# FEniCS/performance-test

Hardware: AMD Instinct MI355X
Metric: DoF/s for ZZZ Assemble + ZZZ Solve; CG-SpMV achieved HBM GB/s vs peak (higher is better)
Workload: dtype f64

## Files before the change

### performance-test_amd/csrc/zzz_api.hip

```cpp
#include "zzz_internal.h"
#include "zzz_sellp.h"

#include <algorithm>
#include <cstdlib>
#include <cstring>
#include <mutex>
#include <numeric>

namespace zzz
{
static std::mutex g_err_mutex;
static std::string g_err;

void set_global_error(const char* msg)
{
  std::lock_guard<std::mutex> lk(g_err_mutex);
  g_err = msg;
}

int fail(zzz_ctx* ctx, int code, const char* fmt, ...)
{
  char buf[1024];
  va_list ap;
  va_start(ap, fmt);
  vsnprintf(buf, sizeof(buf), fmt, ap);
  va_end(ap);
  if (ctx)
    ctx->err = buf;
  else
    set_global_error(buf);
  return code;
}

static int ndofs_cell(int order) { return order == 1 ? 4 : order == 2 ? 10 : order == 3 ? 20 : -1; }

template <typename T>
static int upload(zzz_ctx* ctx, DevBuf<T>& d, const T* h, size_t n, size_t pad = 0)
{
  ZZZ_HIP(ctx, d.alloc(n + pad));
  if (pad)
    ZZZ_HIP(ctx, hipMemsetAsync(d.p + n, 0, pad * sizeof(T), ctx->stream));
  if (n)
    ZZZ_HIP(ctx, hipMemcpyAsync(d.p, h, n * sizeof(T), hipMemcpyHostToDevice, ctx->stream));
  ZZZ_HIP(ctx, hipStreamSynchronize(ctx->stream));
  return ZZZ_OK;
}
int alloc_problem_vectors(zzz_ctx* ctx)
{
  const size_t nv = (size_t)ctx->nloc();
  ZZZ_HIP(ctx, ctx->bc.alloc(nv));
  ZZZ_HIP(ctx, hipMemsetAsync(ctx->bc.p, 0, nv, ctx->stream));
  DevBuf<double>* vecs[] = {&ctx->b, &ctx->u, &ctx->r, &ctx->z, &ctx->p, &ctx->w, &ctx->dinv, &ctx->coeff[0], &ctx->coeff[1]};
  for (DevBuf<double>* v : vecs)
  {
    ZZZ_HIP(ctx, v->alloc(nv));
    ZZZ_HIP(ctx, hipMemsetAsync(v->p, 0, nv * sizeof(double), ctx->stream));
  }
  ZZZ_HIP(ctx, ctx->part_a.alloc(3 * 4096));
  ZZZ_HIP(ctx, ctx->part_b.alloc(4096));
  ZZZ_HIP(ctx, hipStreamSynchronize(ctx->stream));
  return ZZZ_OK;
}
void bc_values_clear(zzz_ctx* ctx)
{
  ctx->have_bc_val = false;
  ++ctx->bc_version;
}
}

using namespace zzz;

extern "C" {

int zzz_device_count(void)
{
  int n = 0;
  if (hipGetDeviceCount(&n) != hipSuccess)
    return 0;
  return n;
}

int zzz_device_memory(int device, size_t* free_bytes, size_t* total_bytes)
{
  if (!free_bytes || !total_bytes)
    return fail(nullptr, ZZZ_ERR_ARG, "zzz_device_memory: NULL argument");
  int prev = 0;
  (void)hipGetDevice(&prev);
  if (hipSetDevice(device) != hipSuccess || hipMemGetInfo(free_bytes, total_bytes) != hipSuccess)
  {
    (void)hipGetLastError();
    (void)hipSetDevice(prev);
    return fail(nullptr, ZZZ_ERR_HIP, "hipMemGetInfo failed on device %d", device);
  }
  (void)hipSetDevice(prev);
  return ZZZ_OK;
}

int zzz_ctx_create(int device, zzz_ctx** out)
{
  if (!out)
    return fail(nullptr, ZZZ_ERR_ARG, "zzz_ctx_create: out is NULL");
  *out = nullptr;
  int n = 0;
  hipError_t e = hipGetDeviceCount(&n);
  if (e != hipSuccess || n <= 0)
    return fail(nullptr, ZZZ_ERR_NO_GPU, "no HIP device available (%s); libzzz_hip has no CPU fallback",
                e == hipSuccess ? "device count 0" : hipGetErrorString(e));
  if (device < 0 || device >= n)
    return fail(nullptr, ZZZ_ERR_ARG, "device %d out of range [0, %d)", device, n);
  e = hipSetDevice(device);
  if (e != hipSuccess)
    return fail(nullptr, ZZZ_ERR_HIP, "hipSetDevice(%d): %s", device, hipGetErrorString(e));
  zzz_ctx* ctx = new zzz_ctx();
  ctx->device = device;
  e = hipStreamCreateWithFlags(&ctx->stream, hipStreamNonBlocking);
  if (e != hipSuccess)
  {
    delete ctx;
    return fail(nullptr, ZZZ_ERR_HIP, "hipStreamCreate: %s", hipGetErrorString(e));
  }
  if (ctx->state.alloc(1) != hipSuccess || ctx->red.alloc(16) != hipSuccess
      || hipHostMalloc((void**)&ctx->h_state, 8 * sizeof(zzz::CgState), hipHostMallocDefault) != hipSuccess)
  {
    zzz_ctx_destroy(ctx);
    return fail(nullptr, ZZZ_ERR_HIP, "context allocation failed");
  }
  memset(ctx->h_state, 0, 8 * sizeof(zzz::CgState));
  {
    static bool loaded[64] = {};
    if (device < 64 && !loaded[device])
    {
      loaded[device] = true;
      zzz::preload_cubegen();
      zzz::preload_renumber();
      zzz::preload_pattern();
      zzz::preload_assemble();
      zzz::preload_sellp_pack();
      zzz::preload_sellp_dict();
      zzz::preload_sellp_pipe();
      zzz::preload_sellp_blk();
      zzz::preload_sellp_win();
      zzz::preload_sellp();
      zzz::preload_spmv();
      zzz::preload_cg();
      zzz::preload_cg_pipe();
      zzz::preload_cg_f32();
      zzz::preload_comm();
      zzz::preload_matfree();
      zzz::preload_mg();
      zzz::preload_pmg();
      zzz::preload_nullspace();
      (void)hipGetLastError();
    }
  }
  if (const char* e = getenv("ZZZ_SPMV_VARIANT"))
  {
    ctx->spmv_variant = atoi(e) & 27;
    ctx->spmv_auto = false;
  }
  if (const char* e = getenv("ZZZ_SELLP"))
  {
    const int v = atoi(e);
    ctx->sellp_mode = v >= 0 && v <= 4 ? v : 1;
    ctx->sellp_long_rows = v == 4;
    if (v == 4)
      ctx->sellp_mode = 2;
  }
  if (const char* e = getenv("ZZZ_SELLP_DROP"))
    ctx->sellp_drop = atoi(e) != 0;
  if (const char* e = getenv("ZZZ_SELLP_DICT"))
    ctx->sellp_dict = atoi(e);
  if (const char* e = getenv("ZZZ_SELLP_BWIN"))
    ctx->sellp_bwin = atoi(e);
  if (const char* e = getenv("ZZZ_SELLP_EARLY"))
    ctx->sellp_early = atoi(e) != 0;
  if (const char* e = getenv("ZZZ_ASM_NODE3"))
    ctx->asm_node3 = atoi(e) != 0;
  if (const char* e = getenv("ZZZ_SELLP_BLK"))
    ctx->sellp_blk = atoi(e);
  if (const char* e = getenv("ZZZ_SELLP_PIPE"))
    ctx->sellp_pipe = atoi(e);
  if (const char* e = getenv("ZZZ_CG_DINV_CODES"))
    ctx->cg_dinv_codes = atoi(e);
  if (const char* e = getenv("ZZZ_CG_XDEFER"))
    ctx->cg_xdefer = atoi(e);
  if (const char* e = getenv("ZZZ_CG_XDEFER_K"))
  {
    const int v = atoi(e);
    if (v == 2 || v == 4 || v == 8)
      ctx->cg_xdefer_k = v;
  }
  if (const char* e = getenv("ZZZ_SELLP_FORMS"))
  {
    const int v = atoi(e);
    if (!(v & 1))
      ctx->sellp_tail |= 2;
    ctx->sellp_align = (v & 2) != 0;
    ctx->sellp_periodic = (v & 4) != 0;
  }
  if (const char* e = getenv("ZZZ_SPMV_LPR"))
  {
    const int v = atoi(e);
    for (int sft = 0; sft <= 4; ++sft)
      if (v == (1 << sft))
        ctx->spmv_lpr_forced = sft;
  }
  if (const char* e = getenv("ZZZ_COLS16"))
  {
    const int v = atoi(e);
    ctx->cols16_enabled = v != 0;
    if (v >= 10 && v <= 13)
      ctx->cols16_offb_forced = v;
  }
  if (const char* e = getenv("ZZZ_OVERLAP"))
    ctx->overlap = atoi(e) != 0;
  if (const char* e = getenv("ZZZ_CG_PIPE_STREAM"))
    ctx->pipe_stream = atoi(e) != 0;
  *out = ctx;
  return ZZZ_OK;
}

void zzz_ctx_destroy(zzz_ctx* ctx)
{
  if (!ctx)
    return;
  (void)hipSetDevice(ctx->device);
  if (ctx->stream)
    (void)hipStreamSynchronize(ctx->stream);
  mg_destroy(ctx);
  comm_destroy(ctx);
  for (hipEvent_t ev : ctx->ev)
    (void)hipEventDestroy(ev);
  for (hipEvent_t ev : ctx->ev_halo)
    (void)hipEventDestroy(ev);
  if (ctx->sp_event)
    (void)hipEventDestroy(ctx->sp_event);
  if (ctx->h_state)
    (void)hipHostFree(ctx->h_state);
  if (ctx->adj_flag_host)
    (void)hipHostFree(ctx->adj_flag_host);
  if (ctx->stream && !ctx->stream_borrowed)
    (void)hipStreamDestroy(ctx->stream);
  for (void* q : ctx->retired)
    (void)hipFree(q);
  delete ctx;
}

const char* zzz_last_error(const zzz_ctx* ctx)
{
  if (ctx)
    return ctx->err.c_str();
  std::lock_guard<std::mutex> lk(g_err_mutex);
  static thread_local std::string copy;
  copy = g_err;
  return copy.c_str();
}

int zzz_sync(zzz_ctx* ctx)
{
  if (!ctx)
    return fail(nullptr, ZZZ_ERR_ARG, "NULL context");
  ZZZ_HIP(ctx, hipSetDevice(ctx->device));
  ZZZ_HIP(ctx, hipStreamSynchronize(ctx->stream));
  return ZZZ_OK;
}

#define ZZZ_ENTER(ctx)                                          \
  do                                                            \
  {                                                             \
    if (!(ctx))                                                 \
      return fail(nullptr, ZZZ_ERR_ARG, "NULL context");        \
    ZZZ_HIP(ctx, hipSetDevice((ctx)->device));                  \
  } while (0)

int zzz_mesh_upload(zzz_ctx* ctx, int64_t nverts, const double* x, int64_t ncells, const int32_t* cell_verts)
{
  ZZZ_ENTER(ctx);
  ctx->cube_feed = false;
  ++ctx->feed_version;
  if (nverts <= 0 || ncells <= 0 || !x || !cell_verts)
    return fail(ctx, ZZZ_ERR_ARG, "zzz_mesh_upload: empty mesh or NULL array");
  if (nverts > INT32_MAX / 4 || ncells > (INT32_MAX - 8) / 20)
    return fail(ctx, ZZZ_ERR_LIMIT, "mesh too large for int32 indexing (%lld vertices, %lld cells)", (long long)nverts,
                (long long)ncells);
  for (int64_t i = 0; i < 4 * ncells; ++i)
    if (cell_verts[i] < 0 || cell_verts[i] >= nverts)
      return fail(ctx, ZZZ_ERR_ARG, "cell_verts[%lld] = %d out of range", (long long)i, cell_verts[i]);
  ctx->nverts = nverts;
  ctx->ncells = ncells;
  ctx->h_cell_verts.assign(cell_verts, cell_verts + 4 * ncells);
  int rc = upload(ctx, ctx->x, x, (size_t)(3 * nverts));
  if (rc)
    return rc;
  rc = upload(ctx, ctx->cell_verts, cell_verts, (size_t)(4 * ncells));
  ctx->have_pattern = ctx->have_matrix = false;
  ctx->xq_valid = false;
  ctx->mf.valid = ctx->mf.failed = false;
  return rc;
}

int zzz_dofmap_upload(zzz_ctx* ctx, int order, int bs, const int32_t* cell_dofs, int64_t n_owned, int64_t n_ghost)
{
  ZZZ_ENTER(ctx);
  ctx->cube_feed = false;
  ++ctx->feed_version;
  const int nd = ndofs_cell(order);
  if (nd < 0)
    return fail(ctx, ZZZ_ERR_ARG, "order %d not supported (1..3)", order);
  if (bs != 1 && bs != 3)
    return fail(ctx, ZZZ_ERR_ARG, "block size %d not supported (1 or 3)", bs);
  if (ctx->ncells == 0)
    return fail(ctx, ZZZ_ERR_ARG, "zzz_dofmap_upload before zzz_mesh_upload");
  if (n_owned <= 0 || n_ghost < 0 || !cell_dofs)
    return fail(ctx, ZZZ_ERR_ARG, "zzz_dofmap_upload: bad sizes");
  const int64_t nloc = n_owned + n_ghost;
  if (nloc * bs > INT32_MAX - 8)
    return fail(ctx, ZZZ_ERR_LIMIT, "%lld local scalar dofs exceed int32", (long long)(nloc * bs));
  for (int64_t i = 0; i < ctx->ncells * nd; ++i)
    if (cell_dofs[i] < 0 || cell_dofs[i] >= nloc)
      return fail(ctx, ZZZ_ERR_ARG, "cell_dofs[%lld] = %d out of range", (long long)i, cell_dofs[i]);
  ctx->order = order;
  ctx->bs = bs;
  ctx->nd = nd;
  ctx->n_owned = n_owned;
  ctx->n_ghost = n_ghost;
  ctx->h_cell_dofs.assign(cell_dofs, cell_dofs + ctx->ncells * nd);
  int rc = upload(ctx, ctx->cell_dofs, cell_dofs, (size_t)(ctx->ncells * nd));
  if (rc)
    return rc;
  ZZZ_HIP(ctx, ctx->facet_mask.alloc((size_t)ctx->ncells));
  ZZZ_HIP(ctx, hipMemsetAsync(ctx->facet_mask.p, 0, (size_t)ctx->ncells, ctx->stream));
  ctx->nfacets = 0;
  rc = alloc_problem_vectors(ctx);
  if (rc)
    return rc;
  ctx->have_bc = false;
  bc_values_clear(ctx);
  ctx->have_coeff[0] = ctx->have_coeff[1] = false;
  ctx->have_pattern = ctx->have_matrix = false;
  ctx->xq_valid = false;
  ctx->mf.valid = ctx->mf.failed = false;
  ctx->near_null_ld = 0;
  rc = renumber_build(ctx);
  if (rc)
    return rc;
  ctx->adj_runs_n = -1;
  pattern_reserve(ctx);
  return ensure_p1_coords(ctx);
}

int zzz_bc_upload(zzz_ctx* ctx, int64_t nbc, const int32_t* bc_dofs)
{
  ZZZ_ENTER(ctx);
  ctx->cube_feed = false;
  ++ctx->feed_version;
  bc_values_clear(ctx);
  if (ctx->order == 0)
    return fail(ctx, ZZZ_ERR_ARG, "zzz_bc_upload before zzz_dofmap_upload");
  if (nbc < 0 || (nbc > 0 && !bc_dofs))
    return fail(ctx, ZZZ_ERR_ARG, "zzz_bc_upload: bad arguments");
  std::vector<uint8_t> m((size_t)ctx->nloc(), 0);
  for (int64_t i = 0; i < nbc; ++i)
  {
    if (bc_dofs[i] < 0 || bc_dofs[i] >= ctx->nloc())
      return fail(ctx, ZZZ_ERR_ARG, "bc_dofs[%lld] = %d out of range", (long long)i, bc_dofs[i]);
    int64_t d = bc_dofs[i];
    if (ctx->renumbered && d / ctx->bs < ctx->n_owned)
      d = (int64_t)ctx->h_iperm[(size_t)(d / ctx->bs)] * ctx->bs + d % ctx->bs;
    m[(size_t)d] = 1;
  }
  ZZZ_HIP(ctx, hipMemcpyAsync(ctx->bc.p, m.data(), m.size(), hipMemcpyHostToDevice, ctx->stream));
  ZZZ_HIP(ctx, hipStreamSynchronize(ctx->stream));
  ctx->have_bc = true;
  ctx->mf.valid = ctx->mf.failed = false;
  return ZZZ_OK;
}

int zzz_bc_values_upload(zzz_ctx* ctx, const double* values)
{
  ZZZ_ENTER(ctx);
  if (!values)
  {
    ctx->have_bc_val = false;
    return ZZZ_OK;
  }
  if (ctx->order == 0)
    return fail(ctx, ZZZ_ERR_ARG, "zzz_bc_values_upload before zzz_dofmap_upload / zzz_cube_generate: the values are indexed by local dof");
  if (!ctx->have_bc)
    return fail(ctx, ZZZ_ERR_ARG, "zzz_bc_values_upload before a Dirichlet set exists (zzz_bc_upload / zzz_cube_generate): the values "
                                  "belong to its dofs");
  const size_t nv = (size_t)ctx->nloc();
  std::vector<double> tmp;
  if (ctx->renumbered)
  {
    tmp.resize(nv);
    to_internal(ctx, values, tmp.data(), false);
    values = tmp.data();
  }
  ZZZ_HIP(ctx, ctx->bc_val.alloc(nv));
  ZZZ_HIP(ctx, hipMemcpyAsync(ctx->bc_val.p, values, nv * sizeof(double), hipMemcpyHostToDevice, ctx->stream));
  ZZZ_HIP(ctx, hipStreamSynchronize(ctx->stream));
  ctx->have_bc_val = true;
  return ZZZ_OK;
}

int zzz_facets_upload(zzz_ctx* ctx, int64_t nfacets, const int32_t* pairs)
{
  ZZZ_ENTER(ctx);
  ctx->cube_feed = false;
  ++ctx->feed_version;
  if (ctx->order == 0)
    return fail(ctx, ZZZ_ERR_ARG, "zzz_facets_upload before zzz_dofmap_upload");
  if (nfacets < 0 || (nfacets > 0 && !pairs))
    return fail(ctx, ZZZ_ERR_ARG, "zzz_facets_upload: bad arguments");
  std::vector<uint8_t> m((size_t)ctx->ncells, 0);
  for (int64_t i = 0; i < nfacets; ++i)
  {
    const int32_t c = pairs[2 * i], f = pairs[2 * i + 1];
    if (c < 0 || c >= ctx->ncells || f < 0 || f > 3)
      return fail(ctx, ZZZ_ERR_ARG, "facet %lld = (%d, %d) out of range", (long long)i, c, f);
    m[c] |= (uint8_t)(1u << f);
  }
  if (ctx->cells_renumbered)
  {
    std::vector<uint8_t> mi(m.size());
    for (size_t i = 0; i < m.size(); ++i)
      mi[i] = m[(size_t)ctx->h_cperm[i]];
    m.swap(mi);
  }
  ZZZ_HIP(ctx, hipMemcpyAsync(ctx->facet_mask.p, m.data(), m.size(), hipMemcpyHostToDevice, ctx->stream));
  ZZZ_HIP(ctx, hipStreamSynchronize(ctx->stream));
  ctx->nfacets = nfacets;
  return ZZZ_OK;
}

int zzz_coeff_upload(zzz_ctx* ctx, int which, const double* values)
{
  ZZZ_ENTER(ctx);
  if (ctx->order == 0)
    return fail(ctx, ZZZ_ERR_ARG, "zzz_coeff_upload before zzz_dofmap_upload");
  if ((which != ZZZ_COEFF_F && which != ZZZ_COEFF_G) || !values)
    return fail(ctx, ZZZ_ERR_ARG, "zzz_coeff_upload: bad arguments");
  std::vector<double> tmp;
  if (ctx->renumbered)
  {
    tmp.resize((size_t)ctx->nloc());
    to_internal(ctx, values, tmp.data(), false);
    values = tmp.data();
  }
  ZZZ_HIP(ctx, hipMemcpyAsync(ctx->coeff[which].p, values, (size_t)ctx->nloc() * sizeof(double), hipMemcpyHostToDevice,
                              ctx->stream));
  ZZZ_HIP(ctx, hipStreamSynchronize(ctx->stream));
  ctx->have_coeff[which] = true;
  return ZZZ_OK;
}

static int pattern_build_host(zzz_ctx* ctx);

int zzz_csr_pattern_build(zzz_ctx* ctx)
{
  ZZZ_ENTER(ctx);
  if (ctx->order == 0)
    return fail(ctx, ZZZ_ERR_ARG, "zzz_csr_pattern_build before zzz_dofmap_upload");
  ctx->have_pattern = ctx->have_matrix = false;
  ++ctx->pattern_version;
  ctx->bw_on = false;
  ctx->have_adj_li = false;
  ctx->have_asm_pos = false;
  ++ctx->mat_version;
  const char* mode = getenv("ZZZ_PATTERN");
  int rc;
  if (mode && strcmp(mode, "host") == 0)
    rc = pattern_build_host(ctx);
  else
  {
    bool fallback = false;
    rc = pattern_build_device(ctx, &fallback);
    if (rc && fallback)
      rc = pattern_build_host(ctx);
  }
  if (rc)
    return rc;
  rc = build_adjT(ctx);
  if (!rc)
// ... 358 lines not shown
    ctx->spmv_variant = variant & 27;
    ctx->spmv_auto = false;
  }
  hipEvent_t e0, e1;
  ZZZ_HIP(ctx, hipEventCreate(&e0));
  ZZZ_HIP(ctx, hipEventCreate(&e1));
  ZZZ_HIP(ctx, hipMemsetAsync(ctx->state.p, 0, sizeof(zzz::CgState), ctx->stream));
  int np = 0;
  int rc = launch_spmv(ctx, ctx->p.p, ctx->w.p, ctx->part_a.p, &np);
  ZZZ_HIP(ctx, hipEventRecord(e0, ctx->stream));
  for (int i = 0; i < reps && !rc; ++i)
    rc = launch_spmv(ctx, ctx->p.p, ctx->w.p, ctx->part_a.p, &np);
  ZZZ_HIP(ctx, hipEventRecord(e1, ctx->stream));
  ZZZ_HIP(ctx, hipEventSynchronize(e1));
  float ms = 0;
  ZZZ_HIP(ctx, hipEventElapsedTime(&ms, e0, e1));
  (void)hipEventDestroy(e0);
  (void)hipEventDestroy(e1);
  ctx->spmv_variant = saved;
  ctx->spmv_auto = saved_auto;
  *avg_ms = ms / reps;
  return rc;
}

int zzz_action(zzz_ctx* ctx, const double* x, double* y)
{
  ZZZ_ENTER(ctx);
  if (ctx->order == 0 || !x || !y)
    return fail(ctx, ZZZ_ERR_ARG, "zzz_action: no dofmap or NULL vector");
  const size_t n = (size_t)(ctx->n_owned * ctx->bs);
  std::vector<double> xin;
  if (ctx->renumbered)
  {
    xin.resize(n);
    to_internal(ctx, x, xin.data(), true);
    x = xin.data();
  }
  ZZZ_HIP(ctx, hipMemsetAsync(ctx->p.p, 0, ctx->p.n * sizeof(double), ctx->stream));
  ZZZ_HIP(ctx, hipMemcpyAsync(ctx->p.p, x, n * sizeof(double), hipMemcpyHostToDevice, ctx->stream));
  ZZZ_HIP(ctx, hipStreamSynchronize(ctx->stream));
  if (ctx->comm)
  {
    int rc = comm_halo_forward(ctx, ctx->p.p);
    if (rc)
      return rc;
  }
  int rc = launch_matfree_action(ctx, ctx->p.p, ctx->w.p, nullptr, nullptr);
  if (rc)
    return rc;
  if (ctx->renumbered)
  {
    ZZZ_HIP(ctx, hipMemcpyAsync(xin.data(), ctx->w.p, n * sizeof(double), hipMemcpyDeviceToHost, ctx->stream));
    ZZZ_HIP(ctx, hipStreamSynchronize(ctx->stream));
    to_caller(ctx, xin.data(), y, true);
    return ctx->comm ? comm_p2p_check(ctx) : ZZZ_OK;
  }
  ZZZ_HIP(ctx, hipMemcpyAsync(y, ctx->w.p, n * sizeof(double), hipMemcpyDeviceToHost, ctx->stream));
  ZZZ_HIP(ctx, hipStreamSynchronize(ctx->stream));
  return ctx->comm ? comm_p2p_check(ctx) : ZZZ_OK;
}

int zzz_matfree_setup(zzz_ctx* ctx)
{
  ZZZ_ENTER(ctx);
  return mf_plan_build(ctx);
}

int zzz_matfree_diagonal(zzz_ctx* ctx, double* diag)
{
  ZZZ_ENTER(ctx);
  if (ctx->order == 0 || !diag)
    return fail(ctx, ZZZ_ERR_ARG, "zzz_matfree_diagonal: no dofmap or NULL vector");
  if (int rc = launch_matfree_diagonal(ctx, ctx->w.p))
    return rc;
  const size_t n = (size_t)(ctx->n_owned * ctx->bs);
  std::vector<double> tmp(ctx->renumbered ? n : 0);
  double* dst = ctx->renumbered ? tmp.data() : diag;
  ZZZ_HIP(ctx, hipMemcpyAsync(dst, ctx->w.p, n * sizeof(double), hipMemcpyDeviceToHost, ctx->stream));
  ZZZ_HIP(ctx, hipStreamSynchronize(ctx->stream));
  if (ctx->renumbered)
    to_caller(ctx, tmp.data(), diag, true);
  return ZZZ_OK;
}

int zzz_matfree_info(zzz_ctx* ctx, int64_t info[8])
{
  if (!ctx || !info)
    return fail(ctx, ZZZ_ERR_ARG, "zzz_matfree_info: bad arguments");
  const zzz::MfPlan& M = ctx->mf;
  info[0] = M.valid ? 1 : 0;
  info[1] = M.nblocks;
  info[2] = M.nc;
  info[3] = M.threads;
  info[4] = M.nloc_max;
  info[5] = M.nshared;
  info[6] = M.nslots;
  info[7] = M.bytes_per_action;
  return ZZZ_OK;
}

int zzz_action_time(zzz_ctx* ctx, int reps, double* avg_ms)
{
  ZZZ_ENTER(ctx);
  if (reps <= 0 || !avg_ms || ctx->order == 0)
    return fail(ctx, ZZZ_ERR_ARG, "zzz_action_time: bad arguments");
  hipEvent_t e0, e1;
  ZZZ_HIP(ctx, hipEventCreate(&e0));
  ZZZ_HIP(ctx, hipEventCreate(&e1));
  ZZZ_HIP(ctx, hipMemsetAsync(ctx->state.p, 0, sizeof(zzz::CgState), ctx->stream));
  int np = 0;
  int rc = launch_matfree_action(ctx, ctx->p.p, ctx->w.p, ctx->part_a.p, &np);
  ZZZ_HIP(ctx, hipEventRecord(e0, ctx->stream));
  for (int i = 0; i < reps && !rc; ++i)
    rc = launch_matfree_action(ctx, ctx->p.p, ctx->w.p, ctx->part_a.p, &np);
  ZZZ_HIP(ctx, hipEventRecord(e1, ctx->stream));
  ZZZ_HIP(ctx, hipEventSynchronize(e1));
  float ms = 0;
  ZZZ_HIP(ctx, hipEventElapsedTime(&ms, e0, e1));
  (void)hipEventDestroy(e0);
  (void)hipEventDestroy(e1);
  *avg_ms = ms / reps;
  return rc;
}

int zzz_cg_solve(zzz_ctx* ctx, const zzz_solver_opts* o, int* iters, double* rnorm)
{
  ZZZ_ENTER(ctx);
  if (!o)
    return fail(ctx, ZZZ_ERR_ARG, "zzz_cg_solve: NULL options");
  if (o->op == ZZZ_OP_CSR && !ctx->have_matrix)
    return fail(ctx, ZZZ_ERR_ARG, "zzz_cg_solve: matrix not assembled");
  if (o->op != ZZZ_OP_CSR && o->op != ZZZ_OP_MATFREE)
    return fail(ctx, ZZZ_ERR_ARG, "unknown operator kind %d", o->op);
  if (o->variant != ZZZ_CG_PETSC && o->variant != ZZZ_CG_CGH && o->variant != ZZZ_CG_PIPE)
    return fail(ctx, ZZZ_ERR_ARG, "unknown CG variant %d", o->variant);
  if (o->variant == ZZZ_CG_PIPE && (o->op != ZZZ_OP_CSR || o->single_reduction || (o->pc != ZZZ_PC_NONE && o->pc != ZZZ_PC_JACOBI)))
    return fail(ctx, ZZZ_ERR_ARG, "-ksp_type pipecg applies to the assembled operator with -pc_type jacobi or none, and not with "
                                  "-ksp_cg_single_reduction");
  if (o->variant == ZZZ_CG_CGH && o->pc != ZZZ_PC_NONE)
    return fail(ctx, ZZZ_ERR_ARG, "src/cg.h has no preconditioner: use pc = ZZZ_PC_NONE");
  if (o->pc != ZZZ_PC_NONE && o->pc != ZZZ_PC_JACOBI && o->pc != ZZZ_PC_CHEBYSHEV_JACOBI && o->pc != ZZZ_PC_MG && o->pc != ZZZ_PC_PMG)
    return fail(ctx, ZZZ_ERR_ARG, "unsupported preconditioner %d (none, jacobi, chebyshev-jacobi, mg, pmg)", o->pc);
  if (o->pc == ZZZ_PC_MG || o->pc == ZZZ_PC_PMG)
    if (int rc = mg_check(ctx, o))
      return rc;
  if (o->pc == ZZZ_PC_CHEBYSHEV_JACOBI && o->op != ZZZ_OP_CSR)
    return fail(ctx, ZZZ_ERR_ARG, "the Chebyshev-Jacobi preconditioner needs the assembled operator");
  if (o->pc == ZZZ_PC_CHEBYSHEV_JACOBI && (o->variant != ZZZ_CG_PETSC || o->pc_degree < 0 || o->pc_degree > 64 || o->pc_esteig_its > 64))
    return fail(ctx, ZZZ_ERR_ARG, "the Chebyshev-Jacobi preconditioner applies to KSPCG (either form), degree 1..64, estimate <= 64 steps");
  if (o->norm < 0 || o->norm > 2)
    return fail(ctx, ZZZ_ERR_ARG, "unknown norm type %d", o->norm);
  if (o->single_reduction && (o->variant != ZZZ_CG_PETSC || o->op != ZZZ_OP_CSR))
    return fail(ctx, ZZZ_ERR_ARG, "-ksp_cg_single_reduction applies to KSPCG on the assembled operator only");
  if (o->max_it < 0 || o->max_it > (1 << 24))
    return fail(ctx, ZZZ_ERR_ARG, "max_it %d out of range", o->max_it);
  return cg_solve(ctx, o, iters, rnorm);
}

static const char* f32_declined(const zzz_ctx* ctx)
{
  if (ctx->order == 0)
    return "no dofmap";
  if (ctx->bs != 1)
    return "block size 3: the float32 path exists for the Poisson form M only (src/Poisson.py:33), not for elasticity";
  if (ctx->comm)
    return "a communicator is attached: the float32 path has no halo exchange or all-reduce yet (one rank only)";
  return nullptr;
}

int zzz_action_f32(zzz_ctx* ctx, const float* x, float* y)
{
  ZZZ_ENTER(ctx);
  if (!x || !y)
    return fail(ctx, ZZZ_ERR_ARG, "zzz_action_f32: NULL vector");
  if (const char* why = f32_declined(ctx))
    return fail(ctx, ZZZ_ERR_ARG, "zzz_action_f32: %s", why);
  const size_t n = (size_t)ctx->n_owned, nl = (size_t)ctx->nloc();
  std::vector<float> tmp;
  if (ctx->renumbered)
  {
    tmp.resize(n);
    for (size_t i = 0; i < n; ++i)
      tmp[i] = x[ctx->h_perm[i]];
    x = tmp.data();
  }
  ZZZ_HIP(ctx, ctx->f32_p.reserve(nl));
  ZZZ_HIP(ctx, ctx->f32_y.reserve(nl));
  ZZZ_HIP(ctx, hipMemsetAsync(ctx->f32_p.p, 0, nl * sizeof(float), ctx->stream));
  ZZZ_HIP(ctx, hipMemcpyAsync(ctx->f32_p.p, x, n * sizeof(float), hipMemcpyHostToDevice, ctx->stream));
  ZZZ_HIP(ctx, hipStreamSynchronize(ctx->stream));
  if (int rc = mf_action_f32(ctx, ctx->f32_p.p, ctx->f32_y.p, nullptr, nullptr))
    return rc;
  float* dst = ctx->renumbered ? tmp.data() : y;
  ZZZ_HIP(ctx, hipMemcpyAsync(dst, ctx->f32_y.p, n * sizeof(float), hipMemcpyDeviceToHost, ctx->stream));
  ZZZ_HIP(ctx, hipStreamSynchronize(ctx->stream));
  if (ctx->renumbered)
    for (size_t i = 0; i < n; ++i)
      y[ctx->h_perm[i]] = tmp[i];
  return ZZZ_OK;
}

int zzz_action_time_f32(zzz_ctx* ctx, int reps, double* avg_ms)
{
  ZZZ_ENTER(ctx);
  if (reps <= 0 || !avg_ms)
    return fail(ctx, ZZZ_ERR_ARG, "zzz_action_time_f32: bad arguments");
  if (const char* why = f32_declined(ctx))
    return fail(ctx, ZZZ_ERR_ARG, "zzz_action_time_f32: %s", why);
  const size_t nl = (size_t)ctx->nloc();
  const float* before = ctx->f32_p.p;
  ZZZ_HIP(ctx, ctx->f32_p.reserve(nl));
  ZZZ_HIP(ctx, ctx->f32_y.reserve(nl));
  if (ctx->f32_p.p != before)
    ZZZ_HIP(ctx, hipMemsetAsync(ctx->f32_p.p, 0, nl * sizeof(float), ctx->stream));
  hipEvent_t e0, e1;
  ZZZ_HIP(ctx, hipEventCreate(&e0));
  ZZZ_HIP(ctx, hipEventCreate(&e1));
  ZZZ_HIP(ctx, hipMemsetAsync(ctx->state.p, 0, sizeof(zzz::CgState), ctx->stream));
  int np = 0;
  int rc = mf_action_f32(ctx, ctx->f32_p.p, ctx->f32_y.p, ctx->part_a.p, &np);
  ZZZ_HIP(ctx, hipEventRecord(e0, ctx->stream));
  for (int i = 0; i < reps && !rc; ++i)
    rc = mf_action_f32(ctx, ctx->f32_p.p, ctx->f32_y.p, ctx->part_a.p, &np);
  ZZZ_HIP(ctx, hipEventRecord(e1, ctx->stream));
  ZZZ_HIP(ctx, hipEventSynchronize(e1));
  float ms = 0;
  ZZZ_HIP(ctx, hipEventElapsedTime(&ms, e0, e1));
  (void)hipEventDestroy(e0);
  (void)hipEventDestroy(e1);
  *avg_ms = ms / reps;
  return rc;
}

int zzz_matfree_info_f32(zzz_ctx* ctx, int64_t info[4])
{
  if (!ctx || !info)
    return fail(ctx, ZZZ_ERR_ARG, "zzz_matfree_info_f32: bad arguments");
  return mf_f32_info(ctx, info);
}

int zzz_cg_solve_f32(zzz_ctx* ctx, const zzz_solver_opts* o, int* iters, double* rnorm)
{
  ZZZ_ENTER(ctx);
  if (!o)
    return fail(ctx, ZZZ_ERR_ARG, "zzz_cg_solve_f32: NULL options");
  if (o->variant != ZZZ_CG_CGH)
    return fail(ctx, ZZZ_ERR_ARG, "zzz_cg_solve_f32: variant %d: float32 runs linalg::cg (src/cg.h, ZZZ_CG_CGH) only", o->variant);
  if (o->pc != ZZZ_PC_NONE)
    return fail(ctx, ZZZ_ERR_ARG, "zzz_cg_solve_f32: preconditioner %d: src/cg.h has none, use pc = ZZZ_PC_NONE", o->pc);
  if (o->op != ZZZ_OP_MATFREE)
    return fail(ctx, ZZZ_ERR_ARG, "zzz_cg_solve_f32: operator %d: float32 exists for the matrix-free operator (ZZZ_OP_MATFREE) only", o->op);
  if (o->single_reduction)
    return fail(ctx, ZZZ_ERR_ARG, "zzz_cg_solve_f32: -ksp_cg_single_reduction (single_reduction) applies to KSPCG on the assembled operator only");
  if (const char* why = f32_declined(ctx))
    return fail(ctx, ZZZ_ERR_ARG, "zzz_cg_solve_f32: %s", why);
  if (ctx->have_bc_val)
    return fail(ctx, ZZZ_ERR_ARG, "zzz_cg_solve_f32: Dirichlet values were uploaded (zzz_bc_values_upload): the lifted right-hand side is "
                                  "not formed in float32 yet");
  if (o->max_it < 0 || o->max_it > (1 << 24))
    return fail(ctx, ZZZ_ERR_ARG, "max_it %d out of range", o->max_it);
  if (ctx->b.n < (size_t)ctx->nloc() || ctx->u.n < (size_t)ctx->nloc())
    return fail(ctx, ZZZ_ERR_ARG, "zzz_cg_solve_f32: no problem vectors");
  return cg_solve_f32(ctx, o, iters, rnorm);
}

int zzz_cg_history(zzz_ctx* ctx, int n, double* out)
{
  if (!ctx || !out || n < 0)
    return fail(ctx, ZZZ_ERR_ARG, "zzz_cg_history: bad arguments");
  const size_t m = std::min((size_t)n, ctx->history.size());
  std::copy(ctx->history.begin(), ctx->history.begin() + (long)m, out);
  return ZZZ_OK;
}

int zzz_spmv_info(zzz_ctx* ctx, int64_t info[8])
{
  ZZZ_ENTER(ctx);
  if (!info || !ctx->have_pattern)
    return fail(ctx, ZZZ_ERR_ARG, "zzz_spmv_info: no pattern");
  if (!sellp_active(ctx))
    if (int rc = ensure_cols16(ctx))
      return rc;
  info[0] = ctx->have_cols16 ? 1 : 0;
  info[1] = ctx->cols16_offb;
  info[2] = ctx->have_cols16 ? ctx->cols16_fallback_tiles : ctx->ntiles;
  info[3] = ctx->ntiles;
  if (sellp_active(ctx) && ctx->sp_win_max > 0)
  {
    info[2] = ctx->sp_win_bytes;
    info[3] = -(int64_t)ctx->sp_win_max;
  }
  info[4] = sellp_active(ctx) ? 1 : (int64_t)1 << ctx->spmv_lpr_shift;
  info[5] = sellp_active(ctx) ? (ctx->sp_sorted ? 2 : 1) : 0;
  info[6] = sellp_active(ctx) ? sellp_stream_bytes(ctx) : 0;
  info[7] = sellp_active(ctx) ? ctx->sp_chunks * 512 : 0;
  return ZZZ_OK;
}

int zzz_spmv_values_info2(zzz_ctx* ctx, int n, int64_t* out)
{
  ZZZ_ENTER(ctx);
  if (!out || n < 0 || !ctx->have_pattern)
    return fail(ctx, ZZZ_ERR_ARG, "zzz_spmv_values_info: no pattern");
  int64_t info[10] = {0, 0, 0, 0, 0, 0, 0, 0, 0, 0};
  if (sellp_active(ctx))
  {
    const bool blk = zzz::sellp_blk_serves(ctx);
    info[4] = !blk && zzz::sellp_pipe_wgs(ctx, false) ? 1 : 0;
    info[5] = blk ? 1 : (info[4] ? zzz::sellp_pipe_wgs(ctx, false) : 8);
    info[0] = ctx->sp_sd_on ? 3 : (ctx->sp_dict_on ? (ctx->sp_dict_n <= zzz::SP_DICT_LDS_ENTRIES ? 2 : 1) : 0);
    info[1] = ctx->sp_dict_on ? ctx->sp_dict_n : 0;
    info[2] = sellp_stream_bytes(ctx);
    info[3] = ctx->sp_bytes + ctx->nslices * 8;
    const bool win = zzz::sellp_win_serves(ctx);
    info[6] = blk ? 1 : (win ? 2 : 0);
    info[7] = blk ? ctx->bk_entries : (win ? ctx->bw_window_entries : 0);
    info[8] = blk ? ctx->bk_chunks : (win ? ctx->bw_chunks : 0);
    info[9] = blk ? ctx->bk_form : (win ? ctx->bw_nblk : 0);
    if (win)
      info[4] = 0, info[5] = 1;
  }
  for (int i = 0; i < std::min(n, 10); ++i)
    out[i] = info[i];
  return ZZZ_OK;
}

int zzz_spmv_values_info(zzz_ctx* ctx, int64_t info[4]) { return zzz_spmv_values_info2(ctx, 4, info); }

int zzz_abi_version(void) { return ZZZ_ABI_VERSION; }

int zzz_internal_order_download(zzz_ctx* ctx, int32_t* perm, int32_t* kind)
{
  if (!ctx || ctx->order == 0)
    return fail(ctx, ZZZ_ERR_ARG, "zzz_internal_order_download: no dofmap yet");
  if (perm)
    for (int64_t i = 0; i < ctx->n_owned; ++i)
      perm[i] = ctx->renumbered ? ctx->h_perm[(size_t)i] : (int32_t)i;
  if (kind)
    *kind = (ctx->renumbered ? ctx->renumber_kind : 0) | (ctx->cells_renumbered ? 16 : 0);
  return ZZZ_OK;
}

int zzz_cg_info(zzz_ctx* ctx, int64_t info[4])
{
  if (!ctx || !info)
    return fail(ctx, ZZZ_ERR_ARG, "zzz_cg_info: bad arguments");
  info[0] = (ctx->last_solve_dinv_codes > 0 ? 2 : 0) | (ctx->last_solve_red_overlapped ? 4 : 0) | (ctx->last_solve_xdefer_k > 1 ? 8 : 0) |
            ((int64_t)(ctx->last_solve_xdefer_k & 15) << 4) | ((int64_t)ctx->last_solve_dinv_codes << 8);
  info[1] = ctx->last_iters;
  info[2] = ctx->last_reason;
  info[3] = (int64_t)(ctx->last_pc_bound * 1.0e6);
  return ZZZ_OK;
}

int zzz_profile_get(zzz_ctx* ctx, double* spmv_avg_ms, int64_t* spmv_count)
{
  if (!ctx)
    return fail(nullptr, ZZZ_ERR_ARG, "NULL context");
  if (spmv_avg_ms)
    *spmv_avg_ms = ctx->prof_spmv_ms;
  if (spmv_count)
    *spmv_count = ctx->prof_spmv_n;
  return ZZZ_OK;
}

}
```

### performance-test_amd/csrc/zzz_cg.hip

```cpp
#include "zzz_device.h"
#include "zzz_internal.h"
#include "zzz_cg.h"

#include <cmath>
#include <cstdlib>

namespace zzz
{
__device__ inline double reduce_parts_bcast(const double* __restrict__ parts, int np, double* sh)
{
  double s = 0;
  for (int i = threadIdx.x; i < np; i += blockDim.x)
    s += parts[i];
  const double t = block_reduce_sum(s, sh);
  __shared__ double bc;
  __syncthreads();
  if (threadIdx.x == 0)
    bc = t;
  __syncthreads();
  return bc;
}

struct DirScalars
{
// ... 493 lines not shown
  const double alpha = beta_it / pw;
  if (variant != ZZZ_CG_CGH && !isfinite(alpha))
  {
    if (blockIdx.x == 0 && threadIdx.x == 0)
    {
      st->iters = it;
      st->converged = 2;
      __atomic_store_n(&st->conv_it1, it + 1, __ATOMIC_RELAXED);
    }
    return;
  }
  if (blockIdx.x == 0 && threadIdx.x == 0)
    alpha_hist[it] = alpha;
  double sa = 0, sb = 0;
  for (int64_t i = i0; i < n2; i += stride)
  {
    dbl2 wi, di, ri, zi;
    if (i == i0)
    {
      wi = wi0;
      di = di0;
      ri = ri0;
    }
    else
    {
      wi = vload<NT>(w2 + i);
      if (!DZ)
        di = vload<NT>(d2 + i);
      ri = vload<NT>(r2 + i);
    }
    if (DZ)
    {
      const uint32_t dc = i == i0 ? dc0 : dz.codes[i];
      di.x = dtab[dc & 0xffffu];
      di.y = dtab[dc >> 16];
    }
    ri.x = -alpha * wi.x + ri.x;
    ri.y = -alpha * wi.y + ri.y;
    zi.x = di.x * ri.x;
    zi.y = di.y * ri.y;
    if (DZ)
      r2[i] = ri;
    else
    {
      vstore<NT>(ri, r2 + i);
      z2[i] = zi;
    }
    sa += ri.x * zi.x;
    sa += ri.y * zi.y;
    if (norm == ZZZ_NORM_UNPRECONDITIONED)
    {
      sb += ri.x * ri.x;
      sb += ri.y * ri.y;
    }
    else
    {
      sb += zi.x * zi.x;
      sb += zi.y * zi.y;
    }
  }
  if ((n & 1) && blockIdx.x == 0 && threadIdx.x == 0)
  {
    const int64_t i = n - 1;
    const double ri = -alpha * w[i] + r[i];
    const double zi = (DZ ? dtab[reinterpret_cast<const uint16_t*>(dz.codes)[i]] : dinv[i]) * ri;
    r[i] = ri;
    if (!DZ)
      z[i] = zi;
    sa += ri * zi;
    sb += (norm == ZZZ_NORM_UNPRECONDITIONED) ? ri * ri : zi * zi;
  }
  const double ta = block_reduce_sum(sa, sh);
  const double tb = block_reduce_sum(sb, sh);
  if (threadIdx.x == 0)
  {
    pa[blockIdx.x] = ta;
    pb[blockIdx.x] = tb;
  }
}

template <bool NT, bool CHEB = false, bool DZ = false>
__global__ __launch_bounds__(VB) void k_sr_update(CgState* __restrict__ st, double* __restrict__ beta_hist,
                                                  double* __restrict__ dpi_hist, double* __restrict__ dp_hist, int it,
                                                  CgParams P, const double* __restrict__ pa, const double* __restrict__ pb,
                                                  const double* __restrict__ pc, int np, const double* __restrict__ dinv,
                                                  const double* __restrict__ s, double* __restrict__ z, double* __restrict__ p,
                                                  double* __restrict__ w, double* __restrict__ x, double* __restrict__ r,
                                                  int64_t n, int scalars_only, double theta = 0.0, double* __restrict__ chg = nullptr,
                                                  double* __restrict__ chd = nullptr, DinvCodes dz = DinvCodes())
{
  static_assert(!(CHEB && DZ), "the polynomial's first term is not D^-1 r alone");
  __shared__ double dtab[DZ ? DZ_MAX : 1];
  if (DZ)
  {
    for (int k = threadIdx.x; k < dz.ndict; k += VB)
      dtab[k] = dz.dict[k];
    __syncthreads();
  }
  const int64_t n2 = n >> 1, stride = (int64_t)gridDim.x * VB;
  const int64_t i0 = blockIdx.x * (int64_t)VB + threadIdx.x;
  const dbl2* __restrict__ s2 = reinterpret_cast<const dbl2*>(s);
  const dbl2* __restrict__ d2 = reinterpret_cast<const dbl2*>(dinv);
  dbl2 *__restrict__ z2 = reinterpret_cast<dbl2*>(z), *__restrict__ p2 = reinterpret_cast<dbl2*>(p),
                     *__restrict__ w2 = reinterpret_cast<dbl2*>(w), *__restrict__ x2 = reinterpret_cast<dbl2*>(x),
                     *__restrict__ r2 = reinterpret_cast<dbl2*>(r);
  const int64_t c0 = (i0 < n2) ? i0 : 0;
  dbl2 zi0 = {0, 0}, si0 = {0, 0}, di0 = {0, 0}, xi0 = {0, 0}, ri0 = {0, 0}, po0 = {0, 0}, wo0 = {0, 0};
  uint32_t dc0 = 0;
  if (n2 > 0 && !scalars_only)
  {
    if (DZ)
      dc0 = dz.codes[c0];
    else
    {
      zi0 = z2[c0];
      di0 = vload<NT>(d2 + c0);
    }
    si0 = vload<NT>(s2 + c0);
    xi0 = vload<NT>(x2 + c0);
    ri0 = vload<NT>(r2 + c0);
    po0 = vload<NT>(p2 + c0);
    wo0 = vload<NT>(w2 + c0);
  }
  const int f0 = st->converged;
  const double ttol_st = st->ttol, dp0_st = st->dp0;
  const double bo_h = it > 0 ? beta_hist[it - 1] : 1.0, dpi_h = it > 0 ? dpi_hist[it - 1] : 0.0;
  double rz = pa[0], nn = pb[0], zs = pc[0];
  if (np == 1)
  {
    if (f0)
      return;
  }
  else
  {
    if (block_flag(f0))
      return;
    reduce_parts3_bcast(pa, pb, pc, np, rz, nn, zs);
  }
  const double dp = (P.norm == ZZZ_NORM_NATURAL) ? sqrt(fabs(rz)) : sqrt(nn);
  double ttol = ttol_st;
  if (it == 0)
    ttol = fmax(P.rtol * dp, P.atol);
  int conv = 0;
  if (!isfinite(dp))
    conv = 2;
  else if (dp <= ttol)
    conv = 1;
  else if (dp >= P.dtol * (it == 0 ? dp : dp0_st))
    conv = 3;
  double b = 0.0, dpi = zs;
  if (it > 0)
  {
    const double bo = bo_h;
    b = rz / bo;
    dpi = zs - rz * rz * dpi_h / (bo * bo);
  }
  const double a = rz / dpi;
  if (!conv && !scalars_only && !isfinite(a))
    conv = 2;
  if (blockIdx.x == 0 && threadIdx.x == 0)
  {
    beta_hist[it] = rz;
    dpi_hist[it] = dpi;
    dp_hist[it] = dp;
    st->dp = dp;
    if (it == 0)
    {
      st->dp0 = dp;
      st->ttol = ttol;
    }
    if (conv)
    {
      st->iters = it;
      st->converged = conv;
    }
  }
  if (conv || scalars_only)
    return;
  auto one = [&](int64_t i) {
    const double dv = DZ ? dtab[reinterpret_cast<const uint16_t*>(dz.codes)[i]] : dinv[i];
    const double zo = DZ ? dv * r[i] : z[i];
    const double pn = (it == 0) ? zo : b * p[i] + zo;
    const double wn = (it == 0) ? s[i] : b * w[i] + s[i];
    p[i] = pn;
    w[i] = wn;
    x[i] = a * pn + x[i];
    const double ri = -a * wn + r[i];
    r[i] = ri;
    const double zi = dv * ri;
    if (CHEB)
    {
      chg[i] = zi;
      chd[i] = zi / theta;
      z[i] = zi / theta;
    }
    else
      z[i] = zi;
  };
  for (int64_t i = i0; i < n2; i += stride)
  {
    dbl2 zi, si, di, xi, ri, po, wo;
    uint32_t dc = dc0;
    if (i == i0)
    {
      zi = zi0, si = si0, di = di0, xi = xi0, ri = ri0, po = po0, wo = wo0;
    }
    else
    {
      if (DZ)
        dc = dz.codes[i];
      else
        zi = z2[i], di = vload<NT>(d2 + i);
      si = vload<NT>(s2 + i), xi = vload<NT>(x2 + i), ri = vload<NT>(r2 + i);
      if (it != 0)
        po = vload<NT>(p2 + i), wo = vload<NT>(w2 + i);
    }
    if (DZ)
    {
      di.x = dtab[dc & 0xffffu];
      di.y = dtab[dc >> 16];
      zi.x = di.x * ri.x;
      zi.y = di.y * ri.y;
    }
    dbl2 pn = zi, wn = si, zn;
    if (it != 0)
    {
      pn.x = b * po.x + zi.x;
      pn.y = b * po.y + zi.y;
      wn.x = b * wo.x + si.x;
      wn.y = b * wo.y + si.y;
    }
    xi.x = a * pn.x + xi.x;
    xi.y = a * pn.y + xi.y;
    ri.x = -a * wn.x + ri.x;
    ri.y = -a * wn.y + ri.y;
    zn.x = di.x * ri.x;
    zn.y = di.y * ri.y;
    vstore<NT>(pn, p2 + i);
    vstore<NT>(wn, w2 + i);
    vstore<NT>(xi, x2 + i);
    vstore<NT>(ri, r2 + i);
    if (CHEB)
    {
      dbl2 dn;
      dn.x = zn.x / theta;
      dn.y = zn.y / theta;
      reinterpret_cast<dbl2*>(chg)[i] = zn;
      reinterpret_cast<dbl2*>(chd)[i] = dn;
      z2[i] = dn;
    }
    else
      z2[i] = zn;
  }
  if ((n & 1) && blockIdx.x == 0 && threadIdx.x == 0)
    one(n - 1);
}

__device__ inline double reduce_parts(const double* __restrict__ parts, int np, double* sh)
{
  double s = 0;
  for (int i = threadIdx.x; i < np; i += blockDim.x)
    s += parts[i];
  return block_reduce_sum(s, sh);
}

__global__ __launch_bounds__(VB) void k_sqnorm(const double* __restrict__ v, int64_t n, double* __restrict__ parts)
{
  __shared__ double sh[VB / 64];
  double s = 0;
  for (int64_t i = blockIdx.x * (int64_t)VB + threadIdx.x; i < n; i += (int64_t)gridDim.x * VB)
    s += v[i] * v[i];
  const double t = block_reduce_sum(s, sh);
  if (threadIdx.x == 0)
    parts[blockIdx.x] = t;
}
__global__ __launch_bounds__(1024) void k_reduce_plain(const double* __restrict__ parts, int np, double* out)
{
  __shared__ double sh[16];
  const double s = reduce_parts(parts, np, sh);
  if (threadIdx.x == 0)
    out[0] = s;
}

int dinv_codes_build(zzz_ctx* ctx, int64_t n, DinvCodes& dzc)
{
  hipStream_t s = ctx->stream;
  const int64_t npad = (n + 1) & ~(int64_t)1;
  ValSet<DD_BITS, 0>& vs = ctx->dd_set;
  ZZZ_HIP(ctx, vs.begin(DZ_MAX, s, ctx->retired));
  ZZZ_HIP(ctx, ctx->dd_codes.reserve((size_t)npad));
  const unsigned gd = (unsigned)std::min<int64_t>((n + 255) / 256, 4096);
  hipLaunchKernelGGL(k_dd_insert, dim3(gd), dim3(256), 0, s, ctx->dinv.p, n, vs.table.p, vs.info.p, DZ_MAX);
  vs.number(s);
  hipLaunchKernelGGL(k_dd_encode, dim3(gd), dim3(256), 0, s, ctx->dinv.p, n, npad, vs.table.p, vs.slot.p, ctx->dd_codes.p, vs.info.p);
  int nd = 0;
  ZZZ_HIP(ctx, vs.finish(s, nd));
  if (nd)
    dzc = DinvCodes{reinterpret_cast<const uint32_t*>(ctx->dd_codes.p), vs.dict.p, ctx->r.p, nd};
  return ZZZ_OK;
}

bool loop_exceeds_cache(zzz_ctx* ctx, int nvec)
{
  const double op = sellp_active(ctx) ? (double)sellp_stream_bytes(ctx) : 10.0 * (double)ctx->nnz;
  return op + 8.0 * nvec * (double)ctx->nloc() > 200.0e6;
}

int vgrid(int64_t n)
{
  constexpr int per = 8;
  int64_t g = (n + VB * per - 1) / (VB * per);
  if (g > VGRID_MAX)
    g = VGRID_MAX;
  if (g < 1)
    g = 1;
  return (int)g;
}

void cg_launch_extract_dinv(zzz_ctx* ctx, int64_t n, int jacobi)
{
  hipLaunchKernelGGL(k_extract_dinv, dim3(vgrid(n)), dim3(VB), 0, ctx->stream, ctx->rowptr.p, ctx->cols.p, ctx->vals.p, ctx->dinv.p, n,
                     jacobi);
}
void cg_launch_init_residual(zzz_ctx* ctx, double* z, int64_t n, int norm, double* pa, double* pb)
{
  hipLaunchKernelGGL(k_init_residual, dim3(vgrid(n)), dim3(VB), 0, ctx->stream, ctx->b.p, (const double*)nullptr, ctx->dinv.p, ctx->r.p,
                     z, n, norm, pa, pb);
}

int vec_norm_local(zzz_ctx* ctx, const double* v, int64_t n, double* out)
{
  const int g = vgrid(n);
  hipLaunchKernelGGL(k_sqnorm, dim3(g), dim3(VB), 0, ctx->stream, v, n, ctx->part_b.p);
  if (ctx->comm)
  {
    int rc = comm_reduce_allreduce(ctx, nullptr, ctx->part_b.p, nullptr, nullptr, g, 1, ctx->red.p);
    if (rc)
      return rc;
  }
  else
    hipLaunchKernelGGL(k_reduce_plain, dim3(1), dim3(1024), 0, ctx->stream, ctx->part_b.p, g, ctx->red.p);
  ZZZ_HIP(ctx, hipGetLastError());
  double s = 0;
  ZZZ_HIP(ctx, hipMemcpyAsync(&s, ctx->red.p, sizeof(double), hipMemcpyDeviceToHost, ctx->stream));
  ZZZ_HIP(ctx, hipStreamSynchronize(ctx->stream));
  *out = std::sqrt(s);
  return comm_p2p_check(ctx);
}

static int cg_solve_single_reduction(zzz_ctx* ctx, const zzz_solver_opts* o, int* iters, double* rnorm);

static int finish_reason(zzz_ctx* ctx, const zzz_solver_opts* o, const CgState& fin, int its)
{
  int reason;
  if (fin.converged == 1)
    reason = (o->variant != ZZZ_CG_CGH && fin.dp < o->atol) ? 3  : 2 ;
  else if (fin.converged == 2)
    reason = -9;
  else if (fin.converged == 3)
    reason = -4;
  else
    reason = -3;
  ctx->last_reason = reason;
  if (o->error_if_not_converged && reason < 0)
  {
    if (reason == -9)
      return fail(ctx, ZZZ_ERR_DIVERGED, "KSP_DIVERGED_NANORINF: CG broke down, non-finite scalar at iteration %d", its);
    if (reason == -4)
      return fail(ctx, ZZZ_ERR_DIVERGED, "KSP_DIVERGED_DTOL: norm %g >= divtol x initial norm %g at iteration %d", fin.dp,
                  fin.dp0, its);
    return fail(ctx, ZZZ_ERR_DIVERGED, "KSP_DIVERGED_ITS: %d iterations without reaching the tolerance (norm %g)", its, fin.dp);
  }
  return ZZZ_OK;
}

void cg_report_reset(zzz_ctx* ctx)
{
  ctx->last_pc_bound = 0.0;
  ctx->last_solve_red_overlapped = false;
  ctx->last_solve_xdefer_k = 1;
  ctx->last_solve_dinv_codes = 0;
}

int CgSolve::begin(zzz_ctx* c, const zzz_solver_opts* opts, int prof_stride)
{
  ctx = c;
  o = opts;
  stride = prof_stride;
  ZZZ_HIP(ctx, ctx->beta_hist.reserve((size_t)o->max_it + 2));
  ZZZ_HIP(ctx, ctx->dp_hist.reserve((size_t)o->max_it + 2));
  ZZZ_HIP(ctx, hipMemsetAsync(ctx->state.p, 0, sizeof(CgState), ctx->stream));
  max_prof = o->profile ? 512 : 0;
  if ((int)ctx->ev.size() < 2 * max_prof)
  {
    size_t old = ctx->ev.size();
    ctx->ev.resize(2 * max_prof);
    for (size_t i = old; i < ctx->ev.size(); ++i)
      ZZZ_HIP(ctx, hipEventCreate(&ctx->ev[i]));
  }
  ctx->prof_halo_n = 0;
  ctx->prof_halo_wait_ms = 0.0;
  ZZZ_HIP(ctx, chk_ev.create());
  return ZZZ_OK;
}

void CgSolve::product_begin(int it)
{
  timed = nprof < max_prof && it % stride == 0;
  ctx->prof_now = timed;
  if (timed)
    (void)hipEventRecord(ctx->ev[2 * nprof], ctx->stream);
}

int CgSolve::product_end(int rc)
{
  ctx->prof_now = false;
  if (rc)
    return rc;
  if (timed)
  {
    (void)hipEventRecord(ctx->ev[2 * nprof + 1], ctx->stream);
    ++nprof;
  }
  return ZZZ_OK;
}

int CgSolve::poll(int done)
{
  if (done % CHECK != 0)
    return ZZZ_OK;
  const int slot = nchk % NSLOT;
  if (nchk >= NSLOT - 1)
  {
    const int old = (nchk - (NSLOT - 1)) % NSLOT;
    ZZZ_HIP(ctx, hipEventSynchronize(chk_ev[old]));
    if (ctx->h_state[old].converged)
      stop = true;
  }
  ZZZ_HIP(ctx, hipMemcpyAsync(&ctx->h_state[slot], ctx->state.p, sizeof(CgState), hipMemcpyDeviceToHost, ctx->stream));
  ZZZ_HIP(ctx, hipEventRecord(chk_ev[slot], ctx->stream));
  ++nchk;
  return ZZZ_OK;
}

int CgSolve::finish(int* iters, double* rnorm)
{
  hipStream_t s = ctx->stream;
  ZZZ_HIP(ctx, hipGetLastError());
  CgState fin;
  ZZZ_HIP(ctx, hipMemcpyAsync(&fin, ctx->state.p, sizeof(CgState), hipMemcpyDeviceToHost, s));
  ZZZ_HIP(ctx, hipStreamSynchronize(s));
  if (int rc = comm_p2p_check(ctx))
    return rc;

  const int its = fin.converged ? fin.iters : o->max_it;
  ctx->last_iters = its;
  if (iters)
    *iters = its;
  if (rnorm)
  {
    rnorm[0] = fin.dp;
    rnorm[1] = fin.dp0;
  }
  ctx->history.resize((size_t)its + 1);
  ZZZ_HIP(ctx, hipMemcpy(ctx->history.data(), ctx->dp_hist.p, sizeof(double) * ((size_t)its + 1), hipMemcpyDeviceToHost));

  ctx->prof_spmv_ms = 0.0;
  ctx->prof_spmv_n = 0;
  const int used = std::min(nprof, (its + stride - 1) / stride);
  for (int i = 0; i < used; ++i)
  {
    float ms = 0;
    if (hipEventElapsedTime(&ms, ctx->ev[2 * i], ctx->ev[2 * i + 1]) == hipSuccess)
    {
      ctx->prof_spmv_ms += ms;
      ctx->prof_spmv_n++;
    }
  }
  if (ctx->prof_spmv_n)
    ctx->prof_spmv_ms /= (double)ctx->prof_spmv_n;
  int cnt = 0;
  for (int i = 0; i < ctx->prof_halo_n; ++i)
  {
    float ms = 0;
    if (hipEventElapsedTime(&ms, ctx->ev_halo[(size_t)(2 * i)], ctx->ev_halo[(size_t)(2 * i + 1)]) == hipSuccess)
    {
      ctx->prof_halo_wait_ms += ms;
      ++cnt;
    }
  }
  if (cnt)
    ctx->prof_halo_wait_ms /= cnt;
  (void)hipGetLastError();
  return finish_reason(ctx, o, fin, its);
}

static int cg_solve_chebyshev(zzz_ctx* ctx, const zzz_solver_opts* o, int* iters, double* rnorm);

int cg_solve(zzz_ctx* ctx, const zzz_solver_opts* o, int* iters, double* rnorm)
{
  cg_report_reset(ctx);
  if (o->variant == ZZZ_CG_PIPE)
    return cg_solve_pipe(ctx, o, iters, rnorm);
  if (o->pc == ZZZ_PC_CHEBYSHEV_JACOBI && !o->single_reduction)
    return cg_solve_chebyshev(ctx, o, iters, rnorm);
  if (o->pc == ZZZ_PC_MG || o->pc == ZZZ_PC_PMG)
    return cg_solve_mg(ctx, o, iters, rnorm);
  if (o->single_reduction)
    return cg_solve_single_reduction(ctx, o, iters, rnorm);
  const int64_t n = ctx->n_owned * ctx->bs;
  const int max_it = o->max_it;
  CgParams P{o->variant, o->pc, o->norm, o->rtol, o->atol, o->dtol > 0.0 ? o->dtol : 1.0e4};
  const bool multi = ctx->comm != nullptr;
  const int g = vgrid(n);
  hipStream_t s = ctx->stream;
  const bool nt = loop_exceeds_cache(ctx, 6);
  auto pick_update_p = [&](bool dzf) { return dzf ? (nt ? k_update_p<true, true> : k_update_p<false, true>) : (nt ? k_update_p<true, false> : k_update_p<false, false>); };
  auto pick_update_xr = [&](bool dzf) { return dzf ? (nt ? k_update_xr<true, true> : k_update_xr<false, true>) : (nt ? k_update_xr<true, false> : k_update_xr<false, false>); };

  CgSolve S;
  if (int rc = S.begin(ctx, o))
    return rc;
  ZZZ_HIP(ctx, ctx->alpha_hist.reserve((size_t)max_it + 2));
  ZZZ_HIP(ctx, hipMemsetAsync(ctx->p.p, 0, sizeof(double) * ctx->p.n, s));

  if (o->op == ZZZ_OP_CSR)
    hipLaunchKernelGGL(k_extract_dinv, dim3(g), dim3(VB), 0, s, ctx->rowptr.p, ctx->cols.p, ctx->vals.p, ctx->dinv.p, n,
                       o->pc == ZZZ_PC_JACOBI ? 1 : 0);
  else if (o->pc == ZZZ_PC_JACOBI)
  {
    if (int rc = launch_matfree_diagonal(ctx, ctx->dinv.p))
      return rc;
    hipLaunchKernelGGL(k_invert, dim3(g), dim3(VB), 0, s, ctx->dinv.p, n);
  }
  else
    hipLaunchKernelGGL(k_extract_dinv, dim3(g), dim3(VB), 0, s, (const rp_t*)nullptr, (const int32_t*)nullptr,
                       (const double*)nullptr, ctx->dinv.p, n, 0);

  DinvCodes dzc{nullptr, nullptr, nullptr, 0};
  if (o->variant == ZZZ_CG_PETSC && o->pc == ZZZ_PC_JACOBI && ctx->cg_dinv_codes != 0 && (ctx->cg_dinv_codes == 2 || nt))
    if (int rc = dinv_codes_build(ctx, n, dzc))
      return rc;
  ctx->last_solve_dinv_codes = dzc.codes ? dzc.ndict : 0;
  const bool dz = dzc.codes != nullptr;
  auto kern_update_p = pick_update_p(dz);
  auto kern_update_xr = pick_update_xr(dz);

  int K = (ctx->cg_xdefer != 0 && (ctx->cg_xdefer == 2 || nt)) ? ctx->cg_xdefer_k : 1;
  PRing ring{};
  ring.slot[0] = ctx->p.p;
  for (int j = 1; j < K; ++j)
  {
    DevBuf<double>& rb = ctx->p_ring[j - 1];
    const double* before = rb.p;
    if (rb.reserve(ctx->p.n) != hipSuccess)
    {
      (void)hipGetLastError();
      for (DevBuf<double>& b : ctx->p_ring)
        b.release();
      fprintf(stderr, "zzz: no memory for %d more direction vectors of %zu entries: CG updates the solution in every iteration (K = 1)\n",
              K - 1, ctx->p.n);
      K = 1;
      break;
    }
    if (rb.p != before)
      ZZZ_HIP(ctx, hipMemsetAsync(rb.p, 0, sizeof(double) * rb.cap, s));
    else if (ctx->p.n > (size_t)n)
      ZZZ_HIP(ctx, hipMemsetAsync(rb.p + n, 0, sizeof(double) * (ctx->p.n - (size_t)n), s));
    ring.slot[j] = rb.p;
  }
  ctx->last_solve_xdefer_k = K;
  update_p_ring_fn kern_light = nullptr, kern_flush = nullptr;
  if (K > 1)
  {
    kern_light = dz ? (nt ? k_update_p_light<true, true> : k_update_p_light<false, true>)
                    : (nt ? k_update_p_light<true, false> : k_update_p_light<false, false>);
    kern_flush = dz ? (nt ? pick_update_p_flush<true, true>(K) : pick_update_p_flush<false, true>(K))
                    : (nt ? pick_update_p_flush<true, false>(K) : pick_update_p_flush<false, false>(K));
  }
  auto dir_of = [&](int k) { return ring.slot[k % K]; };
  auto launch_update_p = [&](int k, int update_dir, const double* rz_src, const double* nn_src, int n_rz) {
    if (K == 1)
      hipLaunchKernelGGL(kern_update_p, dim3(g), dim3(VB), 0, s, ctx->state.p, ctx->beta_hist.p, ctx->dp_hist.p, ctx->alpha_hist.p, k,
                         P, rz_src, nn_src, n_rz, ctx->z.p, ctx->p.p, ctx->u.p, n, update_dir, dzc);
    else
      hipLaunchKernelGGL((k > 0 && k % K == 0) ? kern_flush : kern_light, dim3(g), dim3(VB), 0, s, ctx->state.p, ctx->beta_hist.p,
                         ctx->dp_hist.p, ctx->alpha_hist.p, k, P, rz_src, nn_src, n_rz, ctx->z.p, (const double*)dir_of(k + K - 1),
                         dir_of(k), ring, ctx->u.p, n, update_dir, dzc);
  };

  auto apply = [&](double* x, double* y, double* parts, int* np) -> int {
    if (o->op == ZZZ_OP_CSR)
      return launch_product(ctx, x, y, parts, np);
    if (multi)
      if (int rc = comm_halo_forward(ctx, x))
        return rc;
    return launch_matfree_action(ctx, x, y, parts, np);
  };

  const double* w0 = nullptr;
  if (o->variant == ZZZ_CG_CGH)
  {
    int rc = apply(ctx->u.p, ctx->w.p, nullptr, nullptr);
    if (rc)
      return rc;
    w0 = ctx->w.p;
  }
// ... 678 lines not shown
```

### performance-test_amd/csrc/zzz_internal.h

```cpp
#pragma once

#include <hip/hip_runtime.h>

#include <cstdarg>
#include <cstdint>
#include <cstdio>
#include <string>
#include <vector>

#include "../../include/zzz_abi.h"

struct ChebEpi
{
  const double* dinv = nullptr;
  double* g = nullptr;
  double* z = nullptr;
  const double* r = nullptr;
  double c1 = 0.0, c2 = 0.0;
};

namespace zzz
{
template <typename T>
struct DevBuf
{
  T* p = nullptr;
  size_t n = 0;
  size_t cap = 0;
  DevBuf() = default;
  DevBuf(const DevBuf&) = delete;
  DevBuf& operator=(const DevBuf&) = delete;
  ~DevBuf() { release(); }
  void release()
  {
    if (p)
      (void)hipFree(p);
    p = nullptr;
    n = cap = 0;
  }
  hipError_t reserve(size_t count)
  {
    if (p && cap >= count)
    {
      n = count ? count : 1;
      return hipSuccess;
    }
    return alloc(count);
  }
  hipError_t grow_keep(size_t count, std::vector<void*>& retired)
  {
    if (count == 0)
      count = 1;
    if (p && cap >= count)
    {
      n = count;
      return hipSuccess;
    }
    if (p)
      retired.push_back(p);
    p = nullptr;
    n = cap = 0;
    hipError_t e = hipMalloc((void**)&p, count * sizeof(T));
    if (e == hipSuccess)
      n = cap = count;
    return e;
  }
  hipError_t alloc(size_t count)
  {
    if (count == 0)
      count = 1;
    if (p && cap >= count && cap <= 2 * count + 1024)
    {
      n = count;
      return hipSuccess;
    }
    release();
    hipError_t e = hipMalloc((void**)&p, count * sizeof(T));
    if (e == hipSuccess)
      n = cap = count;
    return e;
  }
};

struct Comm;
struct MgHier;

typedef int64_t rp_t;

constexpr int SPMV_PSTRIDE = 4096;
constexpr int SPMV_TILE_NNZ = 2048;

struct CgState
{
  int converged;
  int iters;
  double dp0;
  double ttol;
  double dp;
  int conv_it1;
  int pad;
};

struct CgParams
{
  int variant, pc, norm;
  double rtol, atol, dtol;
};

struct MfPlan
{
  bool valid = false, failed = false;
  int nd = 0, nc = 0, threads = 0, nsb = 0;
  int ndw = 0, nrw = 0;
  int64_t nblocks = 0, nshared = 0, nslots = 0;
  int nloc_max = 0;
  int64_t bytes_per_action = 0;
  DevBuf<int32_t> hdr;
  DevBuf<int32_t> dof_ids;
  DevBuf<uint8_t> dof_flag;
  DevBuf<double> xyz;
  DevBuf<uint32_t> idxw, rnkw;
  DevBuf<uint8_t> rmax;
  DevBuf<double> geom;
  DevBuf<int32_t> gid;
  DevBuf<double> dtab;
  DevBuf<double> ypart;
  DevBuf<int32_t> sh_dof, sh_off, sh_slot;
  DevBuf<uint8_t> sh_flag;
  DevBuf<int32_t> mf_cell;
  bool f32_built = false;
  int64_t nu = 0;
  int64_t bytes_per_action_f32 = 0;
  DevBuf<float> xyz32;
  DevBuf<float> geom32, dtab32;
  DevBuf<float> ypart32;
};
}

#include "zzz_valset.h"

struct zzz_ctx
{
  int device = 0;
  hipStream_t stream = nullptr;
  std::string err;

  int64_t nverts = 0, ncells = 0;
  zzz::DevBuf<double> x;
  zzz::DevBuf<double> xdof;
  const double* xq = nullptr;
  bool xq_valid = false;
  zzz::DevBuf<int32_t> cell_verts;
  std::vector<int32_t> h_cell_verts;

  int order = 0, bs = 0, nd = 0;
  int64_t n_owned = 0, n_ghost = 0;
  zzz::DevBuf<int32_t> cell_dofs;
  std::vector<int32_t> h_cell_dofs;
  std::vector<int64_t> h_dof_global, h_vert_global;
  int64_t owned_cells = 0;
  bool renumbered = false;
  int renumber_kind = 0;
  zzz::DevBuf<int32_t> perm, iperm;
  std::vector<int32_t> h_perm, h_iperm;
  std::vector<uint16_t> csr_slot;
  bool cells_renumbered = false;
  std::vector<int32_t> h_cperm;

  zzz::DevBuf<uint8_t> bc;
  bool have_bc = false;
  zzz::DevBuf<double> bc_val;
  bool have_bc_val = false;
  uint64_t bc_version = 0;
  zzz::DevBuf<int32_t> lift_rows;
  zzz::DevBuf<uint8_t> lift_flag;
  int64_t n_lift_rows = 0;
  uint64_t lift_pattern_version = ~0ull, lift_bc_version = ~0ull;
  zzz::DevBuf<double> b_masked;

  zzz::DevBuf<uint8_t> facet_mask;
  int64_t nfacets = 0;

  zzz::DevBuf<double> tables;
  int tables_order = 0;
  unsigned lds_attr_set = 0;

  zzz::DevBuf<double> coeff[2];
  bool have_coeff[2] = {false, false};

  int64_t nrows = 0, ncols = 0, nnz = 0;
  zzz::DevBuf<zzz::rp_t> rowptr;
  zzz::DevBuf<int32_t> cols;
  zzz::DevBuf<double> vals;
  zzz::DevBuf<int32_t> scr_keys_out, scr_vals_in, scr_cnt, scr_stage;
  int64_t scr_cell_of_n = -1;
  int scr_cell_of_nd = 0;
  zzz::DevBuf<int64_t> scr_bptr;
  zzz::DevBuf<int32_t> adj_runs, adj_run_lo, adj_win_base;
  int adj_runs_n = -1;
  int32_t* adj_flag_host = nullptr;
  zzz::DevBuf<unsigned char> scr_tmp;
  std::vector<void*> retired;
  zzz::DevBuf<int32_t> adj_off, adj_cells;
  zzz::DevBuf<int32_t> adjT_off, adjT_cells;
  zzz::DevBuf<uint8_t> adj_li;
  zzz::DevBuf<double> cell_w;
  bool have_adj_li = false;
  zzz::DevBuf<uint16_t> asm_pos;
  bool have_asm_pos = false;
  zzz::DevBuf<double> cell_geom;
  int max_row_nnz = 0;
  zzz::DevBuf<double> alpha_hist;
  zzz::DevBuf<int32_t> tile_row;
  zzz::DevBuf<uint16_t> cols16;
  zzz::DevBuf<int32_t> tile_base;
  zzz::DevBuf<int32_t> scr_c16;
  bool have_cols16 = false, cols16_enabled = true, cols16_pending = false;
  int cols16_offb = 12, cols16_offb_forced = 0;
  int64_t cols16_fallback_tiles = 0;
  int64_t ntiles = 0;
  zzz::DevBuf<int32_t> tiles_interior, tiles_boundary;
  int64_t n_tiles_interior = 0, n_tiles_boundary = 0;
  bool have_tile_split = false;
  int spmv_lpr_shift = 0, spmv_lpr_forced = -1;
  bool spmv_auto = true;
  int spmv_variant = 1;
  zzz::DevBuf<int32_t> sp_rownnz, sp_nch, sp_chunk_off, sp_perm, sp_codes32, sp_meta, sp_desc, sp_counter;
  zzz::DevBuf<int64_t> sp_crow;
  zzz::DevBuf<double> sp_cvals;
  zzz::DevBuf<int32_t> sp_ccols;
  zzz::DevBuf<uint8_t> sp_gflag;
  hipEvent_t sp_event = nullptr;
  bool sp_pending = false, sp_forced = false, sp_bounds_ok = false, sp_lds_attr = false;
  bool sp_rownnz_fresh = false;
  bool sp_compact_fresh = false;
  bool sp_crow_is_cap = false;
  int sp_max_range = 0;
  int64_t sp_chunk_bound = 0;
  zzz::DevBuf<uint16_t> sp_codes16;
  zzz::DevBuf<double> sp_vals;
  zzz::DevBuf<unsigned long long> sp_smode;
  bool sp_pipe_ok = false;
  bool sp_one_chunk = false;
  zzz::DevBuf<uint8_t> sp_pairs;
  bool sp_pairs_ok = false;
  int sellp_pipe = 1;
  int64_t nslices = 0, sp_chunks = 0, sp_kept = 0, sp_bytes = 0;
  zzz::DevBuf<uint8_t> sp_wlast;
  zzz::DevBuf<uint16_t> sp_vcode;
  zzz::ValSet<18, 1> sp_dset;
  zzz::DevBuf<int32_t> sp_dict_info;
  zzz::DevBuf<uint16_t> sp_vcode8;
  zzz::DevBuf<double> sp_sd_vals;
  zzz::DevBuf<int32_t> sp_sd_info;
  zzz::DevBuf<int64_t> sp_sd_off;
  bool sp_sd_on = false;
  bool sp_sd_all = false;
  int64_t sp_sd_bytes = 0;
  bool sp_dict_done = false, sp_dict_on = false;
  bool sp_generic = false;
  bool sp_special_tried = false;
  bool sellp_early = true;
  int sellp_dict = 1;
  zzz::ValSet<14, 0> dd_set;
  zzz::DevBuf<uint16_t> dd_codes;
  int cg_dinv_codes = 1;
  int last_solve_dinv_codes = 0;
  zzz::DevBuf<double> p_ring[7];
  int cg_xdefer = 1;
  int cg_xdefer_k = 4;
  int last_solve_xdefer_k = 1;
  int sp_dict_n = 0;
  int64_t sp_dict_bytes = 0;
  bool sp_sorted = false;
  int sellp_mode = 1;
  bool sellp_long_rows = false;
  bool sellp_align = true;
  bool sellp_periodic = true;
  int sellp_tail = 1;
  bool sellp_drop = true;
  bool have_sell = false;
  bool sell_current = false;
  zzz::DevBuf<int32_t> groups_interior, groups_boundary;
  zzz::DevBuf<int32_t> bw_order, bw_perm, bw_desc, bw_wlist, bw_blk_chunks, bw_blk_wn, bw_dnum, bw_info, bw_list_interior, bw_list_boundary;
  zzz::DevBuf<int64_t> bw_chunk0, bw_woff;
  zzz::DevBuf<uint16_t> bw_ccode, bw_vcode, bw_hcode;
  zzz::DevBuf<uint32_t> bw_cpack, bw_vpack;
  zzz::DevBuf<uint8_t> bw_cflag, bw_vflag;
  int64_t bw_packed_planes = 0;
  zzz::DevBuf<uint32_t> bw_key, bw_key2, bw_skey;
  zzz::DevBuf<int32_t> bw_val, bw_hid, bw_first;
  zzz::DevBuf<double> bw_dofx, bw_bbox;
  zzz::DevBuf<double> bw_dict;
  zzz::DevBuf<uint8_t> bw_gflag;
  bool bw_on = false, bw_struct_ok = false, bw_have_split = false, bw_lds_attr = false;
  int sellp_bwin = 1;
  bool asm_node3 = true;
  int32_t bw_nblk = 0;
  int64_t bw_chunks = 0, bw_window_entries = 0, bw_dict_entries = 0, bw_bytes = 0, bw_n_interior = 0, bw_n_boundary = 0;
  uint64_t pattern_version = 0, bw_struct_version = ~0ull;
  zzz::DevBuf<int32_t> bk_desc, bk_meta, bk_flags, bk_nch, bk_c0, bk_slot_code, bk_info, bk_list_interior, bk_list_boundary;
  zzz::DevBuf<uint16_t> bk_code, bk_ccode, bk_rows16;
  zzz::ValSet<13, 1> bk_vset;
  int bk_form = 1, bk_ndict = 0;
  zzz::DevBuf<double> bk_tab;
  zzz::DevBuf<unsigned long long> bk_hash_tag, bk_hash_tag2, bk_hash_owner;
  zzz::DevBuf<int32_t> bk_park;
  zzz::DevBuf<uint8_t> bk_gflag;
  bool bk_on = false, bk_have_split = false, bk_lds_attr = false;
  int sellp_blk = 1;
  int bk_entries = 0;
  int64_t bk_chunks = 0, bk_slices = 0, bk_bytes = 0, bk_n_interior = 0, bk_n_boundary = 0;
  int64_t n_groups_interior = 0, n_groups_boundary = 0;
  bool have_group_split = false;
  zzz::DevBuf<int32_t> asm_tile;
  int64_t n_asm_tiles = 0;
  bool have_pattern = false, have_matrix = false;
  bool tiles_ok = true;

  zzz::DevBuf<double> b, u, r, z, p, w, dinv;
  zzz::DevBuf<double> part_a, part_b, red;
  zzz::DevBuf<double> beta_hist, dp_hist, dpi_hist;
  zzz::DevBuf<double> sr_s;
  zzz::DevBuf<double> pipe_m, pipe_n, pipe_parts;
  zzz::DevBuf<double> cheb_d, cheb_d2, cheb_g;
  zzz::DevBuf<double> cheb_noise;
  zzz::DevBuf<zzz::CgState> state;
  zzz::CgState* h_state = nullptr;
  std::vector<double> history;
  int last_iters = 0;
  int last_reason = 0;
  zzz::DevBuf<int32_t> sp_win_info;
  zzz::DevBuf<int32_t> sp_win_seg;
  int sp_win_max = 0;
  int64_t sp_win_bytes = 0;
  bool halo_pending = false;
  zzz::MfPlan mf;
  zzz::DevBuf<float> f32_x, f32_r, f32_p, f32_y;
  zzz::DevBuf<double> near_null;
  int64_t near_null_ld = 0;
  uint64_t mat_version = 0, cheb_version = ~0ull;
  int cheb_est_its = 0;
  double cheb_hi = 0.0;
  double last_pc_bound = 0.0;

  std::vector<hipEvent_t> ev;
  double prof_spmv_ms = 0.0;
  int64_t prof_spmv_n = 0;
  std::vector<hipEvent_t> ev_halo;
  bool prof_now = false;
  int prof_halo_n = 0;
  double prof_halo_wait_ms = 0.0;

  zzz::Comm* comm = nullptr;
  int nneigh = 0;
  std::vector<int32_t> neigh_rank;
  std::vector<int64_t> send_off, recv_cnt;
  zzz::DevBuf<int32_t> send_idx;
  zzz::DevBuf<double> send_buf;
  std::vector<int64_t> send_contig;
  hipStream_t comm_stream = nullptr;
  hipEvent_t ev_x_ready = nullptr, ev_halo_done = nullptr;
  hipStream_t red_stream = nullptr;
  hipEvent_t ev_parts_ready = nullptr, ev_red_done = nullptr;
  bool red_pending = false;
  bool pipe_stream = true;
  bool last_solve_red_overlapped = false;
  bool overlap = true;

  bool cube_feed = false;
  int cube_problem = 0, cube_nparts = 0;
  int64_t cube_n[3] = {0, 0, 0};
  uint64_t feed_version = 0;
  zzz::MgHier* mg = nullptr;
  bool stream_borrowed = false;

  int64_t nloc() const { return (n_owned + n_ghost) * bs; }
};

namespace zzz
{
int fail(zzz_ctx* ctx, int code, const char* fmt, ...);
void set_global_error(const char* msg);

#define ZZZ_HIP(ctx, call)                                                                                            \
  do                                                                                                                  \
  {                                                                                                                   \
    hipError_t e_ = (call);                                                                                           \
    if (e_ != hipSuccess)                                                                                             \
      return zzz::fail(ctx, ZZZ_ERR_HIP, "%s failed: %s (%s:%d)", #call, hipGetErrorString(e_), __FILE__, __LINE__); \
  } while (0)

#define ZZZ_PRELOAD_TU(name)                                                                                          \
  __global__ void k_preload_##name() {}                                                                               \
  void preload_##name()                                                                                               \
  {                                                                                                                   \
    hipFuncAttributes a;                                                                                              \
    (void)hipFuncGetAttributes(&a, reinterpret_cast<const void*>(&k_preload_##name));                                 \
  }
void preload_assemble();
void preload_cg();
void preload_cg_pipe();
void preload_cg_f32();
void preload_comm();
void preload_cubegen();
void preload_matfree();
void preload_mg();
void preload_nullspace();
void preload_pmg();
void preload_pattern();
void preload_renumber();
void preload_sellp();
void preload_sellp_dict();
void preload_sellp_pack();
void preload_sellp_pipe();
void preload_sellp_blk();
void preload_sellp_win();
void preload_spmv();

int alloc_problem_vectors(zzz_ctx* ctx);
int pattern_build_device(zzz_ctx* ctx, bool* fallback);
void pattern_reserve(zzz_ctx* ctx);
int build_tiles_device(zzz_ctx* ctx, int max_block_cols);
int ensure_cols16(zzz_ctx* ctx);
int asm_tile_nnz(const zzz_ctx* ctx);
int build_adjT(zzz_ctx* ctx);
int dof_coords_device(zzz_ctx* ctx, DevBuf<double>& dofx, DevBuf<int32_t>& first);
int build_adjT_offsets(zzz_ctx* ctx);
int ensure_tables(zzz_ctx* ctx);
int ensure_p1_coords(zzz_ctx* ctx);
int renumber_build(zzz_ctx* ctx);
void renumber_clear(zzz_ctx* ctx);
void to_internal(const zzz_ctx* ctx, const double* in, double* out, bool owned_only);
void to_caller(const zzz_ctx* ctx, const double* in, double* out, bool owned_only);
int csr_to_caller(zzz_ctx* ctx, std::vector<zzz::rp_t>& rowptr_c, int32_t* cols_c, double* vals_c, bool need_cols);
int csr_values_to_internal(zzz_ctx* ctx, const double* vals_c, std::vector<double>& vals_i);
enum ProductMode { PM_DOT_SR, PM_DOT, PM_PLAIN, PM_CHEB_DOT, PM_CHEB, PM_COUNT };
enum ProductLoad { LOAD_NT, LOAD_PLAIN };
struct ProductCall
{
  const double* x = nullptr;
  double* y = nullptr;
  double* partials = nullptr;
  const int* stop = nullptr;
  const int32_t* list = nullptr;
  int64_t nlist = 0;
  const double* rvec = nullptr;
  int nn_is_rr = 0;
  const ChebEpi* epi = nullptr;
  ProductMode mode = PM_PLAIN;
  ProductLoad load = LOAD_PLAIN;
  int special = 0;
};
inline ProductCall product_call(const zzz_ctx* ctx, const double* x, double* y, double* partials, const double* rvec, int nn_is_rr,
                                const ChebEpi* epi)
{
  ProductCall c;
  c.x = x;
  c.y = y;
  c.epi = epi;
  if (partials)
  {
    c.partials = partials;
    c.stop = reinterpret_cast<const int*>(ctx->state.p);
    c.rvec = rvec;
    c.nn_is_rr = nn_is_rr;
  }
  c.mode = epi ? (partials ? PM_CHEB_DOT : PM_CHEB) : partials ? (rvec ? PM_DOT_SR : PM_DOT) : PM_PLAIN;
  return c;
}
typedef void (*ProductLauncher)(zzz_ctx* ctx, int grid, const ProductCall& c);
struct ProductPart
{
  int64_t n;
  const int32_t* list;
  int grid;
};
int launch_spmv(zzz_ctx* ctx, const double* x, double* y, double* partials, int* npartials, const double* rvec = nullptr,
                int nn_is_rr = 0, const ChebEpi* epi = nullptr);
int launch_product(zzz_ctx* ctx, double* x, double* y, double* partials, int* npartials, const double* rvec = nullptr,
                   int nn_is_rr = 0, const ChebEpi* epi = nullptr);
int launch_overlapped(zzz_ctx* ctx, double* x, ProductCall c, const ProductPart& in, const ProductPart& bd, ProductLauncher launch,
                      int* npartials);
int sell_update(zzz_ctx* ctx, bool structure);
bool sellp_active(zzz_ctx* ctx);
int sellp_resolve(zzz_ctx* ctx);
int sellp_pattern_bounds(zzz_ctx* ctx);
int sellp_capacity_rows(zzz_ctx* ctx);
int64_t sellp_stream_bytes(const zzz_ctx* ctx);
constexpr int SP_DICT_LDS_ENTRIES = 2048;
int launch_sellp(zzz_ctx* ctx, ProductCall c, int* npartials);
int launch_sellp_overlapped(zzz_ctx* ctx, double* x, ProductCall c, int* npartials);

int launch_assemble_matrix(zzz_ctx* ctx, int form);
int launch_assemble_vector(zzz_ctx* ctx, int form);
int launch_lift(zzz_ctx* ctx);
void bc_values_clear(zzz_ctx* ctx);
int launch_matfree_action(zzz_ctx* ctx, const double* x, double* y, double* partials, int* npartials);
int launch_matfree_legacy(zzz_ctx* ctx, const double* x, double* y, double* partials, int* npartials);
int launch_matfree_diagonal(zzz_ctx* ctx, double* d);
int mf_plan_build(zzz_ctx* ctx);
int mf_action(zzz_ctx* ctx, const double* x, double* y, double* partials, int* npartials);
int mf_diagonal(zzz_ctx* ctx, double* y);
int mf_action_f32(zzz_ctx* ctx, const float* x, float* y, double* partials, int* npartials);
int mf_f32_prepare(zzz_ctx* ctx);
int mf_f32_info(zzz_ctx* ctx, int64_t info[4]);
int cg_solve_f32(zzz_ctx* ctx, const zzz_solver_opts* o, int* iters, double* rnorm);

int cg_solve(zzz_ctx* ctx, const zzz_solver_opts* o, int* iters, double* rnorm);
int vec_norm_local(zzz_ctx* ctx, const double* v, int64_t n, double* out);

int mg_check(zzz_ctx* ctx, const zzz_solver_opts* o);
int mg_setup(zzz_ctx* ctx, const zzz_solver_opts* o);
int mg_vcycle(zzz_ctx* ctx, const double* r, double* z, bool timed);
void mg_profile_begin(zzz_ctx* ctx);
void mg_profile_end(zzz_ctx* ctx, int cycles);
int mg_level0_products(const zzz_ctx* ctx);
double mg_level0_bound(const zzz_ctx* ctx);
void mg_destroy(zzz_ctx* ctx);
int pmg_prolong(zzz_ctx* ctx, const int* stop, int order, int bs, const int64_t n[3], const uint8_t* bcf, const uint8_t* bcc,
                const double* ec, double* xf, int accumulate);
int pmg_restrict(zzz_ctx* ctx, const int* stop, int order, int bs, const int64_t n[3], const uint8_t* bcf, const uint8_t* bcc,
                 const double* rf, const double* sub, double* rc);
int chebyshev_bound(zzz_ctx* ctx, const zzz_solver_opts* o, double* hi);
int cg_solve_mg(zzz_ctx* ctx, const zzz_solver_opts* o, int* iters, double* rnorm);

int comm_allreduce_sum(zzz_ctx* ctx, double* dev, int n);
int comm_reduce_allreduce(zzz_ctx* ctx, const int* stop, const double* pa, const double* pb, const double* pc, int np, int nv,
                          double* out, hipStream_t st = nullptr);
int comm_reduce_begin(zzz_ctx* ctx, const int* stop, const double* pa, const double* pb, const double* pc, int np, int nv,
                      double* out);
int comm_reduce_end(zzz_ctx* ctx);
bool comm_p2p_enabled(const zzz_ctx* ctx);
int comm_p2p_check(zzz_ctx* ctx);
int comm_halo_forward(zzz_ctx* ctx, double* vec);
int comm_halo_begin(zzz_ctx* ctx, double* vec);
int comm_halo_end(zzz_ctx* ctx);
int build_tile_split(zzz_ctx* ctx);
void comm_destroy(zzz_ctx* ctx);
}
```

### performance-test_amd/csrc/zzz_sellp.hip

```cpp
#include <climits>
#include <cstring>
#include <cstdlib>
#include <vector>

#include "zzz_sellp.h"

namespace zzz
{
template <bool NT, typename T>
__device__ inline T sp_load(const T* p)
{
  return NT ? __builtin_nontemporal_load(p) : *p;
}

template <bool NT, bool FULL, int DICT = 0, bool FOLD = false>
__device__ inline void read_chunk(int c, int w, int lane, const double* __restrict__ svals, const uint16_t* __restrict__ c16,
                                  const int32_t* __restrict__ c32, const int32_t* __restrict__ meta, dbl2 (&v)[4], int (&cl)[8],
                                  const uint16_t* __restrict__ vcode = nullptr, const double* __restrict__ dict = nullptr,
                                  int* __restrict__ loff = nullptr)
{
  if (FOLD)
    *loff = 0;
  const double* __restrict__ sp = svals + (size_t)c * 512;
  if (DICT == 1 || DICT == 2 || (DICT == 3 && dict != nullptr))
// ... 74 lines not shown
    cl[2] = mp[2] + (int)((q.x >> 16) & 0xffu);
    cl[3] = mp[3] + (int)(q.x >> 24);
    cl[4] = mp[4] + (int)(q.y & 0xffu);
    cl[5] = mp[5] + (int)((q.y >> 8) & 0xffu);
    cl[6] = mp[6] + (int)((q.y >> 16) & 0xffu);
    cl[7] = mp[7] + (int)(q.y >> 24);
  }
  else
  {
    const uint4v q = sp_load<NT>(reinterpret_cast<const uint4v*>(c16 + (size_t)c * 512) + lane);
    cl[0] = m0 + (int)(q.x & 0xffffu);
    cl[1] = mp[1] + (int)(q.x >> 16);
    cl[2] = mp[2] + (int)(q.y & 0xffffu);
    cl[3] = mp[3] + (int)(q.y >> 16);
    cl[4] = mp[4] + (int)(q.z & 0xffffu);
    cl[5] = mp[5] + (int)(q.z >> 16);
    cl[6] = mp[6] + (int)(q.w & 0xffffu);
    cl[7] = mp[7] + (int)(q.w >> 16);
  }
}

template <bool NT, bool FULL, bool LDS = false, int DICT = 0>
__device__ inline void chunk_product(int c, int w, int lane, const double* __restrict__ svals, const uint16_t* __restrict__ c16,
                                     const int32_t* __restrict__ c32, const int32_t* __restrict__ meta,
                                     const double* __restrict__ x, double& sum, const uint16_t* __restrict__ vcode = nullptr,
                                     const double* __restrict__ dict = nullptr)
{
  dbl2 v[4];
  int cl[8];
  int loff = 0;
  read_chunk<NT, FULL, DICT, LDS>(c, w, lane, svals, c16, c32, meta, v, cl, vcode, dict, &loff);
  const double* __restrict__ xl = LDS ? x + loff : x;
  double xv[8];
#pragma unroll
  for (int e = 0; e < 8; ++e)
    xv[e] = (FULL || e < w) ? (LDS ? xl[cl[e]] : gather(x, cl[e])) : 0.0;
#pragma unroll
  for (int e = 0; e < 8; ++e)
    if (FULL || e < w)
      sum += ((e & 1) ? v[e >> 1].y : v[e >> 1].x) * xv[e];
}

template <bool DOT, bool NT, bool PERM, bool CHEB = false, bool WIN = false, int DICT = 0>
__global__ __launch_bounds__(SP_BLOCK, 8) void spmv_sellp_kernel(const int2* __restrict__ desc,
                                                              const double* __restrict__ svals,
                                                              const uint16_t* __restrict__ c16,
                                                              const int32_t* __restrict__ c32,
                                                              const int32_t* __restrict__ meta,
                                                              const int32_t* __restrict__ perm,
                                                              const double* __restrict__ x, double* __restrict__ y,
                                                              int nrows, int64_t nslices, double* __restrict__ partials,
                                                              const int* __restrict__ stop_flag,
                                                              const int32_t* __restrict__ group_list, int64_t nlist,
                                                              const double* __restrict__ rvec, int pstride, int nn_is_rr,
                                                              ChebEpi epi, const int2* __restrict__ win_info,
                                                              const int2* __restrict__ win_seg, const uint16_t* __restrict__ vcode,
                                                              const double* __restrict__ dict_g, int dict_n,
                                                              const int32_t* __restrict__ sd_info,
                                                              const int64_t* __restrict__ sd_off)
{
  extern __shared__ __attribute__((aligned(16))) double sp_lds[];
  double* const xwin = sp_lds + (DICT == 2 ? ((dict_n + 1) & ~1) : 0);
  double* const sdl = sp_lds + (threadIdx.x >> 6) * SD_MAX;
  const double* dict = DICT == 2 ? sp_lds : dict_g;
  __shared__ double red[SP_BLOCK / 64];
  const int lane = threadIdx.x & 63, wv = threadIdx.x >> 6;
  const int64_t ngroups = group_list ? nlist : (nslices + 3) / 4;
  double dot = 0.0, dot_rx = 0.0, dot_nn = 0.0;
  auto next_slice = [&](int i, int& s_out, int2& ds_out) -> int {
    const int64_t gi = sp_xcd_item(ngroups, blockIdx.x, gridDim.x, i);
    if (gi < 0)
      return -1;
    const int64_t g = group_list ? group_list[gi] : gi;
    const int s = __builtin_amdgcn_readfirstlane((int)(4 * g + wv));
    s_out = s;
    if (s >= nslices)
      return 0;
    ds_out = desc[s];
    return 1;
  };
  int s_n = 0;
  int2 ds_n = make_int2(0, 0);
  int st_n = next_slice(0, s_n, ds_n);
  if (stop_flag && *stop_flag)
    return;
  if (DICT == 2)
  {
    double t[SP_DICT_LDS_ENTRIES / SP_BLOCK];
#pragma unroll
    for (int i = 0; i < SP_DICT_LDS_ENTRIES / SP_BLOCK; ++i)
    {
      const int k = (int)threadIdx.x + i * SP_BLOCK;
      t[i] = k < dict_n ? dict_g[k] : 0.0;
    }
#pragma unroll
    for (int i = 0; i < SP_DICT_LDS_ENTRIES / SP_BLOCK; ++i)
    {
      const int k = (int)threadIdx.x + i * SP_BLOCK;
      if (k < dict_n)
        sp_lds[k] = t[i];
    }
    __syncthreads();
  }
  for (int i = 0; st_n >= 0; ++i)
  {
    const int st = st_n, s = s_n;
    const int2 ds = ds_n;
    st_n = next_slice(i + 1, s_n, ds_n);
    int nwin = 0;
    if (WIN)
    {
      const int2 wi = win_info[s >> 2];
      nwin = __builtin_amdgcn_readfirstlane(wi.x);
      if (nwin > 0)
      {
        const int2* __restrict__ sg = win_seg + (int64_t)(s >> 2) * SP_WIN_NSEG;
        __syncthreads();
        constexpr int WIN_BLOCKS = 12;
        int q = 0, seg_first = 0, off = 0;
        int2 sq = sg[0];
        int c0s = __builtin_amdgcn_readfirstlane(sq.x), len = __builtin_amdgcn_readfirstlane(sq.y);
        for (int b0 = 0; q < nwin; b0 += WIN_BLOCKS)
        {
          double t[WIN_BLOCKS];
          int at[WIN_BLOCKS];
#pragma unroll
          for (int i = 0; i < WIN_BLOCKS; ++i)
          {
            at[i] = -1;
            t[i] = 0.0;
            while (q < nwin && (b0 + i - seg_first) * SP_BLOCK >= len)
            {
              off += len;
              seg_first = b0 + i;
              ++q;
              if (q < nwin)
              {
                sq = sg[q];
                c0s = __builtin_amdgcn_readfirstlane(sq.x);
                len = __builtin_amdgcn_readfirstlane(sq.y);
              }
            }
            if (q < nwin)
            {
              const int k = (b0 + i - seg_first) * SP_BLOCK + (int)threadIdx.x;
              if (k < len)
              {
                t[i] = x[c0s + k];
                at[i] = off + k;
              }
            }
          }
#pragma unroll
          for (int i = 0; i < WIN_BLOCKS; ++i)
            if (at[i] >= 0)
              xwin[at[i]] = t[i];
        }
        __syncthreads();
      }
    }
    if (st == 0)
      continue;
    if (DICT == 3)
    {
      const int n_sd = __builtin_amdgcn_readfirstlane(sd_info[s]);
      const int64_t sd_tab = sd_off[s];
      if (n_sd > 0)
      {
        __builtin_amdgcn_wave_barrier();
        const dbl2* __restrict__ tsrc = reinterpret_cast<const dbl2*>(dict_g + sd_tab);
        const int n2 = (n_sd + 1) >> 1;
        for (int b0 = 0; b0 * 64 < n2; b0 += 4)
        {
          dbl2 t[4];
#pragma unroll
          for (int i = 0; i < 4; ++i)
            t[i] = lane + 64 * (b0 + i) < n2 ? tsrc[lane + 64 * (b0 + i)] : dbl2{0.0, 0.0};
#pragma unroll
          for (int i = 0; i < 4; ++i)
            if (lane + 64 * (b0 + i) < n2)
              reinterpret_cast<dbl2*>(sdl)[lane + 64 * (b0 + i)] = t[i];
        }
        __builtin_amdgcn_wave_barrier();
        dict = sdl;
      }
      else
        dict = nullptr;
    }
    const int c0 = ds.x, nch = ds.y & 0xffffff, wl = ds.y >> 24;
    int r = PERM ? perm[(int64_t)s * 64 + lane] : s * 64 + lane;
    if (!PERM && r >= nrows)
      r = -1;
    const double xr = ((DOT || CHEB) && r >= 0) ? x[r] : 0.0;
    double sum = 0.0;
    if (WIN && nwin > 0)
    {
      for (int j = 0; j + 1 < nch; ++j)
        chunk_product<NT, true, true, DICT>(c0 + j, 8, lane, svals, c16, c32, meta, xwin, sum, vcode, dict);
      if (nch)
      {
        if (wl == 8)
          chunk_product<NT, true, true, DICT>(c0 + nch - 1, 8, lane, svals, c16, c32, meta, xwin, sum, vcode, dict);
        else
          chunk_product<NT, false, true, DICT>(c0 + nch - 1, wl, lane, svals, c16, c32, meta, xwin, sum, vcode, dict);
      }
    }
    else
    {
      for (int j = 0; j + 1 < nch; ++j)
        chunk_product<NT, true, false, DICT>(c0 + j, 8, lane, svals, c16, c32, meta, x, sum, vcode, dict);
      if (nch)
      {
        if (wl == 8)
          chunk_product<NT, true, false, DICT>(c0 + nch - 1, 8, lane, svals, c16, c32, meta, x, sum, vcode, dict);
        else
          chunk_product<NT, false, false, DICT>(c0 + nch - 1, wl, lane, svals, c16, c32, meta, x, sum, vcode, dict);
      }
    }
    if (CHEB)
    {
      if (r >= 0)
      {
        const double gi = -1.0 * (epi.dinv[r] * sum) + epi.g[r];
        const double dn = epi.c1 * xr + epi.c2 * gi;
        const double zi = epi.z[r] + dn;
        epi.z[r] = zi;
        if (DOT)
        {
          const double ri = epi.r[r];
          dot_rx += ri * zi;
          dot_nn += nn_is_rr ? ri * ri : zi * zi;
        }
        else
        {
          epi.g[r] = gi;
          y[r] = dn;
        }
      }
    }
    else if (r >= 0)
    {
      y[r] = sum;
      if (DOT)
      {
        dot += sum * xr;
        if (rvec)
        {
          const double rr_ = rvec[r];
          dot_rx += rr_ * xr;
          dot_nn += nn_is_rr ? rr_ * rr_ : xr * xr;
        }
      }
    }
  }
  if (DOT)
  {
    const double sres = CHEB ? 0.0 : block_reduce_sum(dot, red);
    double s1 = 0.0, s2 = 0.0;
    if (rvec || CHEB)
    {
      s1 = block_reduce_sum(dot_rx, red);
      s2 = block_reduce_sum(dot_nn, red);
    }
    if (threadIdx.x == 0)
    {
      if (!CHEB)
        partials[blockIdx.x] = sres;
      if (rvec || CHEB)
      {
        partials[pstride + blockIdx.x] = s1;
        partials[2 * pstride + blockIdx.x] = s2;
      }
    }
  }
}


bool sellp_special_build(zzz_ctx* ctx)
{
  if (sellp_blk_build(ctx) != ZZZ_OK)
  {
    ctx->bk_on = false;
    (void)hipGetLastError();
  }
  if (sellp_win_build(ctx) != ZZZ_OK)
  {
    ctx->bw_on = false;
    (void)hipGetLastError();
  }
  return sellp_blk_serves(ctx) || sellp_win_serves(ctx);
}

bool sellp_active(zzz_ctx* ctx)
{
  if (ctx->sp_pending)
    (void)sellp_resolve(ctx);
  if (!ctx->have_sell || !ctx->sell_current)
    return false;
  if (!(ctx->spmv_auto || (ctx->spmv_variant & 8) != 0))
    return false;
  if (!ctx->sp_dict_done)
  {
    ctx->sp_dict_done = true;
    ctx->sp_dict_on = ctx->sp_sd_on = ctx->sp_sd_all = false;
    ctx->sp_dict_n = 0;
    if (!ctx->sp_special_tried)
    {
      (void)sellp_special_build(ctx);
      ctx->sp_special_tried = true;
    }
    if (!sellp_blk_serves(ctx) && !sellp_win_serves(ctx))
    {
      if (sp_dict_build(ctx) != ZZZ_OK)
      {
        ctx->sp_dict_on = false;
        (void)hipGetLastError();
        ctx->sp_vcode.release();
      }
      if (sp_sd_build(ctx) != ZZZ_OK)
      {
        ctx->sp_sd_on = ctx->sp_sd_all = false;
        (void)hipGetLastError();
        ctx->sp_vcode8.release();
        ctx->sp_sd_vals.release();
        ctx->sp_sd_info.release();
        ctx->sp_sd_off.release();
      }
    }
    ctx->sp_pairs_ok = false;
    if (ctx->sp_one_chunk && ctx->sp_dict_on && ctx->bs == 1 && !ctx->sp_sorted)
      ctx->sp_pairs_ok = sellp_pairs_build(ctx) == ZZZ_OK;
  }
  return true;
}

int64_t sellp_stream_bytes(const zzz_ctx* ctx)
{
  if (sellp_blk_serves(ctx))
    return ctx->bk_bytes;
  if (sellp_win_serves(ctx))
    return ctx->bw_bytes;
  return (ctx->sp_sd_on ? ctx->sp_sd_bytes : (ctx->sp_dict_on ? ctx->sp_dict_bytes : ctx->sp_bytes)) + ctx->nslices * 8;
}

static bool sp_stream_nt(const zzz_ctx* ctx)
{
  return (double)sellp_stream_bytes(ctx) + 48.0 * (double)(ctx->n_owned + ctx->n_ghost) * ctx->bs > 200.0e6;
}

static int sp_grid(const zzz_ctx* ctx, int64_t ngroups, bool sr, bool plain)
{
  const int pw = plain ? sellp_pipe_wgs(ctx, sr) : 0;
  int64_t gs = 256 * (pw ? pw : 8);
  const int64_t need = (ngroups + 7) / 8 * 8;
  if (gs > need)
    gs = need;
  if (gs < 8)
    gs = 8;
  return (int)gs;
}

enum SpLayout { SP_PLAIN, SP_SORTED, SP_WINDOWED, SP_LAYOUTS };
using SpKernel = decltype(&spmv_sellp_kernel<false, false, false>);
struct SpVariants
{
  SpKernel k[SP_LAYOUTS][4];
};
template <bool DOT, bool CHEB, bool NT>
constexpr SpVariants sp_variants()
{
  return {{{spmv_sellp_kernel<DOT, NT, false, CHEB, false, 0>, spmv_sellp_kernel<DOT, NT, false, CHEB, false, 1>,
            spmv_sellp_kernel<DOT, NT, false, CHEB, false, 2>, spmv_sellp_kernel<DOT, NT, false, CHEB, false, 3>},
           {spmv_sellp_kernel<DOT, NT, true, CHEB, false, 0>, spmv_sellp_kernel<DOT, NT, true, CHEB, false, 1>,
            spmv_sellp_kernel<DOT, NT, true, CHEB, false, 2>, spmv_sellp_kernel<DOT, NT, true, CHEB, false, 3>},
           {spmv_sellp_kernel<DOT, NT, false, CHEB, true, 0>, spmv_sellp_kernel<DOT, NT, false, CHEB, true, 1>,
            spmv_sellp_kernel<DOT, NT, false, CHEB, true, 2>, nullptr}}};
}
static const SpVariants sp_kernels[PM_COUNT][2] = {{sp_variants<true, false, true>(), sp_variants<true, false, false>()},
                                                   {sp_variants<true, false, true>(), sp_variants<true, false, false>()},
                                                   {sp_variants<false, false, true>(), sp_variants<false, false, false>()},
                                                   {sp_variants<true, true, true>(), sp_variants<true, true, false>()},
                                                   {sp_variants<false, true, true>(), sp_variants<false, true, false>()}};

static void launch_one(zzz_ctx* ctx, int grid, const ProductCall& c)
{
  if (c.special == 1 && launch_sellp_blk(ctx, grid, c))
    return;
  if (c.special == 2 && launch_sellp_win(ctx, grid, c))
    return;
  if (launch_sellp_pipe(ctx, grid, c))
    return;
  const SpLayout layout = ctx->sp_sorted ? SP_SORTED : ctx->sp_win_max > 0 ? SP_WINDOWED : SP_PLAIN;
  size_t lds = layout == SP_WINDOWED ? (size_t)ctx->sp_win_max * sizeof(double) : 0;
  int dict = 0;
  if (ctx->sp_sd_on && layout != SP_WINDOWED)
  {
    dict = 3;
    lds = (size_t)4 * SD_MAX * sizeof(double);
  }
  else if (ctx->sp_dict_on && ctx->sp_dict_n <= SP_DICT_LDS_ENTRIES)
  {
    dict = 2;
    lds += (size_t)((ctx->sp_dict_n + 1) & ~1) * sizeof(double);
  }
  else if (ctx->sp_dict_on)
    dict = 1;
  hipLaunchKernelGGL(sp_kernels[c.mode][c.load].k[layout][dict], dim3(grid), dim3(SP_BLOCK), lds, ctx->stream,
                     reinterpret_cast<const int2*>(ctx->sp_desc.p), ctx->sp_vals.p, ctx->sp_codes16.p, ctx->sp_codes32.p,
                     ctx->sp_meta.p, ctx->sp_perm.p, c.x, c.y, (int)ctx->nrows, ctx->nslices, c.partials, c.stop, c.list, c.nlist,
                     c.rvec, SPMV_PSTRIDE, c.nn_is_rr, c.epi ? *c.epi : ChebEpi(), reinterpret_cast<const int2*>(ctx->sp_win_info.p),
                     reinterpret_cast<const int2*>(ctx->sp_win_seg.p), dict == 3 ? ctx->sp_vcode8.p : ctx->sp_vcode.p,
                     dict == 3 ? ctx->sp_sd_vals.p : ctx->sp_dset.dict.p, ctx->sp_dict_n, ctx->sp_sd_info.p, ctx->sp_sd_off.p);
}

static int sp_prepare(zzz_ctx* ctx, ProductCall& c, bool split)
{
  c.special = (sellp_blk_serves(ctx) && (!split || ctx->bk_have_split)) ? 1
              : (sellp_win_serves(ctx) && (!split || ctx->bw_have_split)) ? 2 : 0;
  bool nt = sp_stream_nt(ctx);
  if (!ctx->spmv_auto)
    nt = (ctx->spmv_variant & 1) != 0;
  c.load = nt ? LOAD_NT : LOAD_PLAIN;
  return c.special ? ZZZ_OK : sellp_need_generic(ctx);
}

int launch_sellp(zzz_ctx* ctx, ProductCall c, int* npartials)
{
  if (int rc = sp_prepare(ctx, c, false))
    return rc;
  const int gs = c.special == 1 ? sellp_blk_grid(ctx, ctx->bk_slices) : c.special == 2 ? sellp_win_grid(ctx, ctx->bw_nblk)
                 : sp_grid(ctx, (ctx->nslices + 3) / 4, c.mode == PM_DOT_SR, !c.epi);
  launch_one(ctx, gs, c);
  if (c.partials && npartials)
    *npartials = gs;
  ZZZ_HIP(ctx, hipGetLastError());
  return ZZZ_OK;
}

int launch_sellp_overlapped(zzz_ctx* ctx, double* x, ProductCall c, int* npartials)
{
  if (int rc = sp_prepare(ctx, c, true))
    return rc;
  const int blk = c.special;
  const bool plain = !c.epi, sr = c.mode == PM_DOT_SR;
  const int64_t gi = blk == 1 ? ctx->bk_n_interior : blk == 2 ? ctx->bw_n_interior : ctx->n_groups_interior;
  const int64_t gb = blk == 1 ? ctx->bk_n_boundary : blk == 2 ? ctx->bw_n_boundary : ctx->n_groups_boundary;
  const int32_t* list_in = blk == 1 ? ctx->bk_list_interior.p : blk == 2 ? ctx->bw_list_interior.p : ctx->groups_interior.p;
  const int32_t* list_bd = blk == 1 ? ctx->bk_list_boundary.p : blk == 2 ? ctx->bw_list_boundary.p : ctx->groups_boundary.p;
  auto grid = [&](int64_t items) {
    return !items ? 0 : blk == 1 ? sellp_blk_grid(ctx, items) : blk == 2 ? sellp_win_grid(ctx, items) : sp_grid(ctx, items, sr, plain);
  };
  int g_in = grid(gi);
  const int pw = plain ? sellp_pipe_wgs(ctx, sr) : 0;
  const int room = 256 * ((pw ? pw : 8) - 1);
  if (!blk && g_in > room && ctx->nneigh > 0)
    g_in = room;
  const int g_bd = grid(gb);
  if (c.partials && (size_t)(g_in + g_bd) > (size_t)SPMV_PSTRIDE)
    return fail(ctx, ZZZ_ERR_ARG, "partials buffer too small");
  return launch_overlapped(ctx, x, c, {gi, list_in, g_in}, {gb, list_bd, g_bd}, launch_one, npartials);
}
ZZZ_PRELOAD_TU(sellp)
}
```

### performance-test_amd/csrc/zzz_sellp_dict.hip

```cpp
#include <climits>
#include <cstring>
#include <cstdlib>

#include "zzz_sellp.h"

#include <rocprim/rocprim.hpp>

namespace zzz
{
struct Even2
{
  __host__ __device__ int64_t operator()(int32_t n) const { return ((int64_t)n + 1) & ~(int64_t)1; }
};
constexpr int SP_DICT_BITS = decltype(zzz_ctx::sp_dset)::bits;
constexpr int SP_DICT_MAX = 65535;

__device__ inline unsigned long long sp_value_bits(const double* __restrict__ svals, int64_t c, int w, int lane, int e)
{
  const int64_t at = ((w & 1) && e == w - 1) ? 128 * (e >> 1) + lane : 128 * (e >> 1) + 2 * lane + (e & 1);
  return reinterpret_cast<const unsigned long long*>(svals)[c * 512 + at];
}

template <bool PERM>
__global__ __launch_bounds__(256) void k_sp_dict_insert(const int2* __restrict__ desc, const int32_t* __restrict__ perm,
                                                         const double* __restrict__ svals, int nrows, int64_t nslices,
                                                         unsigned long long* __restrict__ table, int* __restrict__ info, int limit)
{
  const int lane = threadIdx.x & 63;
  for (int64_t s = blockIdx.x * 4ll + (threadIdx.x >> 6); s < nslices; s += gridDim.x * 4ll)
  {
    const int r = PERM ? perm[s * 64 + lane] : (int)(s * 64 + lane);
    const bool row = r >= 0 && r < nrows;
    const int2 ds = desc[s];
    const int c0 = ds.x, nch = ds.y & 0xffffff, wl = ds.y >> 24;
    unsigned long long last = 0ull;
    for (int j = 0; j < nch; ++j)
    {
      const int w = j + 1 < nch ? 8 : wl;
      for (int e = 0; e < w; ++e)
      {
        const unsigned long long b = row ? sp_value_bits(svals, c0 + j, w, lane, e) : 0ull;
        const bool need = b != last && b != 0ull;
        last = b;
        if (!valset_insert_wave<SP_DICT_BITS>(table, info, limit, b, need))
          return;
      }
    }
  }
}

template <bool PERM>
__global__ __launch_bounds__(256) void k_sp_dict_encode(const int2* __restrict__ desc, const int32_t* __restrict__ perm,
                                                         const double* __restrict__ svals, const int32_t* __restrict__ meta,
                                                         int nrows, int64_t nslices, const unsigned long long* __restrict__ table,
                                                         const int32_t* __restrict__ slot_code, const int* __restrict__ info,
                                                         uint16_t* __restrict__ vcode, unsigned long long* __restrict__ bytes_out)
{
  if (info[1])
    return;
  const int lane = threadIdx.x & 63;
  unsigned long long bytes = 0;
  for (int64_t s = blockIdx.x * 4ll + (threadIdx.x >> 6); s < nslices; s += gridDim.x * 4ll)
  {
    const int r = PERM ? perm[s * 64 + lane] : (int)(s * 64 + lane);
    const bool row = r >= 0 && r < nrows;
    const int2 ds = desc[s];
    const int c0 = ds.x, nch = ds.y & 0xffffff, wl = ds.y >> 24;
    unsigned long long last = 0ull;
    unsigned last_code = 0;
    for (int j = 0; j < nch; ++j)
    {
      const int w = j + 1 < nch ? 8 : wl;
      unsigned code[8];
#pragma unroll
      for (int e = 0; e < 8; ++e)
      {
        code[e] = 0;
        if (row && e < w)
        {
          const unsigned long long b = sp_value_bits(svals, c0 + j, w, lane, e);
          if (b == 0ull)
            continue;
          if (b != last)
          {
            last = b;
            last_code = (unsigned)valset_find<SP_DICT_BITS>(table, slot_code, b);
          }
          code[e] = last_code;
        }
      }
      uint4v q;
      q.x = code[0] | (code[1] << 16);
      q.y = code[2] | (code[3] << 16);
      q.z = code[4] | (code[5] << 16);
      q.w = code[6] | (code[7] << 16);
      reinterpret_cast<uint4v*>(vcode + (size_t)(c0 + j) * 512)[lane] = q;
      if (lane == 0)
      {
        const int m0 = meta[(size_t)(c0 + j) * 8];
        unsigned cb = 0;
        if (m0 < 0 && (m0 & 0x40000000))
          cb = 100;
        else if (m0 < 0)
          cb = 2048;
        else if ((m0 & 0x60000000) == 0x20000000)
          cb = 0;
        else if (m0 & 0x40000000)
          cb = 512;
        else
          cb = 1024;
        bytes += 1024 + 32 + cb;
      }
    }
  }
  if (lane == 0 && bytes)
    atomicAdd(bytes_out, bytes);
}

template <bool PERM, bool COUNT>
__global__ __launch_bounds__(128) void k_sp_sd_build(const int2* __restrict__ desc, const int32_t* __restrict__ perm,
                                                      const double* __restrict__ svals, const int32_t* __restrict__ meta,
                                                      int nrows, int64_t nslices, uint16_t* __restrict__ vcode8,
                                                      double* __restrict__ sd_vals, const int64_t* __restrict__ sd_off,
                                                      int32_t* __restrict__ sd_info, unsigned long long* __restrict__ bytes_out)
{
  __shared__ unsigned long long keys_s[2][SD_SLOTS];
  __shared__ uint16_t code_s[2][SD_SLOTS];
  __shared__ int cnt_s[2];
  const int lane = threadIdx.x & 63, wv = threadIdx.x >> 6;
  unsigned long long* const keys = keys_s[wv];
  uint16_t* const codes = code_s[wv];
  unsigned long long bytes = 0;
  for (int64_t s = blockIdx.x * 2ll + wv; s < nslices; s += gridDim.x * 2ll)
  {
    for (int k = lane; k < SD_SLOTS; k += 64)
      keys[k] = ~0ull;
    if (lane == 0)
      cnt_s[wv] = 1;
    __builtin_amdgcn_wave_barrier();
    const int r = PERM ? perm[s * 64 + lane] : (int)(s * 64 + lane);
    const bool row = r >= 0 && r < nrows;
    const int2 ds = desc[s];
    const int c0 = ds.x, nch = ds.y & 0xffffff, wl = ds.y >> 24;
    if (!COUNT && sd_info[s] == 0)
    {
      if (lane == 0)
      {
        for (int j = 0; j < nch; ++j)
        {
          const int w = j + 1 < nch ? 8 : wl;
          const int m0 = meta[(size_t)(c0 + j) * 8];
          const unsigned cb = (m0 < 0 && (m0 & 0x40000000)) ? 100u : (m0 < 0 ? 2048u : ((m0 & 0x60000000) == 0x20000000 ? 0u : ((m0 & 0x40000000) ? 512u : 1024u)));
          bytes += 32 + cb + (unsigned)((w >> 1) * 1024 + (w & 1) * 512);
        }
        bytes += 4;
        atomicAdd(reinterpret_cast<int*>(bytes_out) + 2, 1);
      }
      continue;
    }
    double* const tab = COUNT ? nullptr : sd_vals + sd_off[s];
    if (!COUNT && lane == 0)
      tab[0] = 0.0;
    unsigned long long last = 0ull;
    for (int j = 0; j < nch; ++j)
    {
      if (cnt_s[wv] > SD_MAX)
        break;
      const int w = j + 1 < nch ? 8 : wl;
      for (int e = 0; e < w; ++e)
      {
        const unsigned long long b = row ? sp_value_bits(svals, c0 + j, w, lane, e) : 0ull;
        if (b != 0ull && b != last && b != ~0ull)
        {
          unsigned h = valset_hash<SD_BITS>(b);
          for (int probe = 0; probe < SD_SLOTS; ++probe)
          {
            const unsigned long long cur = keys[h];
            if (cur == b)
              break;
            if (cur == ~0ull)
            {
              const unsigned long long old = atomicCAS(&keys[h], ~0ull, b);
              if (old == ~0ull)
              {
                const int c = atomicAdd(&cnt_s[wv], 1);
                codes[h] = (uint16_t)c;
                if (!COUNT && c < SD_MAX)
                  tab[c] = __longlong_as_double((long long)b);
                break;
              }
              if (old == b)
                break;
            }
            h = (h + 1) & (SD_SLOTS - 1);
            if (cnt_s[wv] > SD_MAX)
              break;
          }
        }
        if (b == ~0ull)
          cnt_s[wv] = SD_MAX + 1;
        last = b;
      }
    }
    __builtin_amdgcn_wave_barrier();
    const int n = cnt_s[wv];
    const bool ok = n <= SD_MAX;
    if (COUNT)
    {
      if (lane == 0)
        sd_info[s] = ok ? n : 0;
      __builtin_amdgcn_wave_barrier();
      continue;
    }
    if (ok)
    {
      last = 0ull;
      unsigned last_code = 0;
      for (int j = 0; j < nch; ++j)
      {
        const int w = j + 1 < nch ? 8 : wl;
        unsigned code[8];
#pragma unroll
        for (int e = 0; e < 8; ++e)
        {
          code[e] = 0;
          if (row && e < w)
          {
            const unsigned long long b = sp_value_bits(svals, c0 + j, w, lane, e);
            if (b == 0ull)
              continue;
            if (b != last)
            {
              unsigned h = valset_hash<SD_BITS>(b);
              while (keys[h] != b)
                h = (h + 1) & (SD_SLOTS - 1);
              last = b;
              last_code = codes[h];
            }
            code[e] = last_code;
          }
        }
        uint4v q;
        q.x = code[0] | (code[1] << 16);
        q.y = code[2] | (code[3] << 16);
        q.z = code[4] | (code[5] << 16);
        q.w = code[6] | (code[7] << 16);
        reinterpret_cast<uint4v*>(vcode8 + (size_t)(c0 + j) * 512)[lane] = q;
      }
    }
    if (lane == 0)
    {
      for (int j = 0; j < nch; ++j)
      {
        const int w = j + 1 < nch ? 8 : wl;
        const int m0 = meta[(size_t)(c0 + j) * 8];
        unsigned cb = 0;
        if (m0 < 0 && (m0 & 0x40000000))
          cb = 100;
        else if (m0 < 0)
          cb = 2048;
        else if ((m0 & 0x60000000) == 0x20000000)
          cb = 0;
        else if (m0 & 0x40000000)
          cb = 512;
        else
          cb = 1024;
        bytes += 32 + cb + (ok ? 1024 : (unsigned)((w >> 1) * 1024 + (w & 1) * 512));
      }
      bytes += ok ? (unsigned)n * 8 + 4 : 4;
    }
    __builtin_amdgcn_wave_barrier();
  }
  if (lane == 0 && bytes)
    atomicAdd(bytes_out, bytes);
}

int sp_dict_build(zzz_ctx* ctx)
{
  ctx->sp_dict_done = true;
  ctx->sp_dict_on = false;
  ctx->sp_dict_n = 0;
  if (!ctx->sellp_dict || ctx->sp_chunks <= 0 || (ctx->sellp_dict == 1 && ctx->sp_bytes < 48ll << 20))
    return ZZZ_OK;
  hipStream_t s = ctx->stream;
  const int64_t nsl = ctx->nslices;
  ValSet<SP_DICT_BITS, 1>& vs = ctx->sp_dset;
  ZZZ_HIP(ctx, vs.begin(SP_DICT_MAX + 1, s, ctx->retired));
  ZZZ_HIP(ctx, ctx->sp_vcode.alloc((size_t)ctx->sp_chunks * 512));
  ZZZ_HIP(ctx, ctx->sp_dict_info.reserve(4));
  ZZZ_HIP(ctx, hipMemsetAsync(ctx->sp_dict_info.p, 0, 4 * sizeof(int32_t), s));
  unsigned long long* bytes = reinterpret_cast<unsigned long long*>(ctx->sp_dict_info.p);
  const int2* desc = reinterpret_cast<const int2*>(ctx->sp_desc.p);
  const unsigned grid = (unsigned)std::min<int64_t>((nsl + 3) / 4, 256 * 16);
  const int limit = ctx->sellp_dict == 2 ? SP_DICT_MAX - 1 : SP_DICT_LDS_ENTRIES - 2;
  if (ctx->sp_sorted)
    hipLaunchKernelGGL(k_sp_dict_insert<true>, dim3(grid), dim3(256), 0, s, desc, ctx->sp_perm.p, ctx->sp_vals.p, (int)ctx->nrows, nsl,
                       vs.table.p, vs.info.p, limit);
  else
    hipLaunchKernelGGL(k_sp_dict_insert<false>, dim3(grid), dim3(256), 0, s, desc, (const int32_t*)nullptr, ctx->sp_vals.p,
                       (int)ctx->nrows, nsl, vs.table.p, vs.info.p, limit);
  vs.number(s);
  if (ctx->sp_sorted)
    hipLaunchKernelGGL(k_sp_dict_encode<true>, dim3(grid), dim3(256), 0, s, desc, ctx->sp_perm.p, ctx->sp_vals.p, ctx->sp_meta.p,
                       (int)ctx->nrows, nsl, vs.table.p, vs.slot.p, vs.info.p, ctx->sp_vcode.p, bytes);
  else
    hipLaunchKernelGGL(k_sp_dict_encode<false>, dim3(grid), dim3(256), 0, s, desc, (const int32_t*)nullptr, ctx->sp_vals.p,
                       ctx->sp_meta.p, (int)ctx->nrows, nsl, vs.table.p, vs.slot.p, vs.info.p, ctx->sp_vcode.p, bytes);
  unsigned long long hb = 0;
  ZZZ_HIP(ctx, hipMemcpyAsync(&hb, bytes, sizeof(hb), hipMemcpyDeviceToHost, s));
  int n = 0;
  ZZZ_HIP(ctx, vs.finish(s, n));
  if (!n)
    return ZZZ_OK;
  ctx->sp_dict_n = n;
  ctx->sp_dict_bytes = (int64_t)hb + (int64_t)n * 8;
  ctx->sp_dict_on = true;
  return ZZZ_OK;
}

int sp_sd_build(zzz_ctx* ctx)
{
  ctx->sp_sd_on = ctx->sp_sd_all = false;
  if (!ctx->sellp_dict || ctx->sp_dict_on || ctx->sp_chunks <= 0 || ctx->sp_win_max > 0)
    return ZZZ_OK;
  if (ctx->sellp_dict != 3 && (ctx->sp_bytes < 48ll << 20 || ctx->sp_chunks < 4 * ctx->nslices))
    return ZZZ_OK;
  hipStream_t s = ctx->stream;
  const int64_t nsl = ctx->nslices;
  ZZZ_HIP(ctx, ctx->sp_vcode8.alloc((size_t)ctx->sp_chunks * 512));
  ZZZ_HIP(ctx, ctx->sp_sd_info.alloc((size_t)nsl + 1));
  ZZZ_HIP(ctx, ctx->sp_sd_off.alloc((size_t)nsl + 1));
  ZZZ_HIP(ctx, ctx->sp_dict_info.reserve(4));
  ZZZ_HIP(ctx, hipMemsetAsync(ctx->sp_dict_info.p, 0, 4 * sizeof(int32_t), s));
  ZZZ_HIP(ctx, hipMemsetAsync(ctx->sp_sd_info.p + nsl, 0, sizeof(int32_t), s));
  const int2* desc = reinterpret_cast<const int2*>(ctx->sp_desc.p);
  const unsigned grid = (unsigned)std::min<int64_t>((nsl + 1) / 2, 256 * 8);
  unsigned long long* bytes = reinterpret_cast<unsigned long long*>(ctx->sp_dict_info.p);
  if (ctx->sp_sorted)
    hipLaunchKernelGGL((k_sp_sd_build<true, true>), dim3(grid), dim3(128), 0, s, desc, ctx->sp_perm.p, ctx->sp_vals.p, ctx->sp_meta.p,
                       (int)ctx->nrows, nsl, (uint16_t*)nullptr, (double*)nullptr, (const int64_t*)nullptr, ctx->sp_sd_info.p, bytes);
  else
    hipLaunchKernelGGL((k_sp_sd_build<false, true>), dim3(grid), dim3(128), 0, s, desc, (const int32_t*)nullptr, ctx->sp_vals.p,
                       ctx->sp_meta.p, (int)ctx->nrows, nsl, (uint16_t*)nullptr, (double*)nullptr, (const int64_t*)nullptr,
                       ctx->sp_sd_info.p, bytes);
  {
    const auto even = rocprim::make_transform_iterator(ctx->sp_sd_info.p, Even2{});
    size_t tb = 0;
    ZZZ_HIP(ctx, rocprim::exclusive_scan(nullptr, tb, even, ctx->sp_sd_off.p, (int64_t)0, (size_t)nsl + 1, rocprim::plus<int64_t>(), s));
    ZZZ_HIP(ctx, ctx->scr_tmp.grow_keep(tb, ctx->retired));
    ZZZ_HIP(ctx, rocprim::exclusive_scan(ctx->scr_tmp.p, tb, even, ctx->sp_sd_off.p, (int64_t)0, (size_t)nsl + 1, rocprim::plus<int64_t>(), s));
  }
  int64_t total = 0;
  ZZZ_HIP(ctx, hipMemcpyAsync(&total, ctx->sp_sd_off.p + nsl, sizeof(total), hipMemcpyDeviceToHost, s));
  ZZZ_HIP(ctx, hipStreamSynchronize(s));
  ZZZ_HIP(ctx, ctx->sp_sd_vals.alloc((size_t)total + 2));
  if (ctx->sp_sorted)
    hipLaunchKernelGGL((k_sp_sd_build<true, false>), dim3(grid), dim3(128), 0, s, desc, ctx->sp_perm.p, ctx->sp_vals.p, ctx->sp_meta.p,
                       (int)ctx->nrows, nsl, ctx->sp_vcode8.p, ctx->sp_sd_vals.p, ctx->sp_sd_off.p, ctx->sp_sd_info.p, bytes);
  else
    hipLaunchKernelGGL((k_sp_sd_build<false, false>), dim3(grid), dim3(128), 0, s, desc, (const int32_t*)nullptr, ctx->sp_vals.p,
                       ctx->sp_meta.p, (int)ctx->nrows, nsl, ctx->sp_vcode8.p, ctx->sp_sd_vals.p, ctx->sp_sd_off.p, ctx->sp_sd_info.p,
                       bytes);
  ZZZ_HIP(ctx, hipGetLastError());
  int32_t h[4];
  ZZZ_HIP(ctx, hipMemcpyAsync(h, ctx->sp_dict_info.p, sizeof(h), hipMemcpyDeviceToHost, s));
  ZZZ_HIP(ctx, hipStreamSynchronize(s));
  unsigned long long b = 0;
  memcpy(&b, h, sizeof(b));
  if (ctx->sellp_dict != 3 && (double)b > 0.6 * (double)ctx->sp_bytes)
    return ZZZ_OK;
  if ((int64_t)h[2] >= nsl)
    return ZZZ_OK;
  ctx->sp_sd_bytes = (int64_t)b;
  ctx->sp_sd_on = true;
  ctx->sp_sd_all = h[2] == 0;
  return ZZZ_OK;
}
ZZZ_PRELOAD_TU(sellp_dict)
}
```

### performance-test_amd/csrc/zzz_sellp_pipe.hip

```cpp
#include <algorithm>
#include <cstdlib>
#include <type_traits>

#include "zzz_sellp.h"

namespace zzz
{
struct PipeArgs
{
  int dict_n;
  int nrows;
  int nslices;
  double* partials;
  const int* stop_flag;
  int64_t nlist;
  int pstride, nn_is_rr;
};

template <bool NT, typename T>
__device__ inline T pipe_load(const T* p)
{
  return NT ? __builtin_nontemporal_load(p) : *p;
}

typedef double dbl2u __attribute__((ext_vector_type(2), aligned(8)));

__global__ __launch_bounds__(256) void k_sp_pairs(const int2* __restrict__ desc, const unsigned long long* __restrict__ smode,
                                                  const int32_t* __restrict__ meta, int64_t nslices, uint8_t* __restrict__ pairs)
{
  const int64_t npairs = (nslices + 1) / 2;
  for (int64_t p = blockIdx.x * (int64_t)blockDim.x + threadIdx.x; p < npairs; p += (int64_t)gridDim.x * blockDim.x)
  {
    bool ok = 2 * p + 1 < nslices;
    if (ok)
    {
      const int2 da = desc[2 * p], db = desc[2 * p + 1];
      ok = (da.y & 0xffffff) == 1 && (db.y & 0xffffff) == 1 && (da.y >> 24) == (db.y >> 24) && (smode[2 * p] & 3ull) == 0ull
           && (smode[2 * p + 1] & 3ull) == 0ull;
      if (ok)
      {
        const int32_t* ma = meta + (int64_t)da.x * 8;
        const int32_t* mb = meta + (int64_t)db.x * 8;
        const int w = da.y >> 24;
        ok = ma[0] >= 0 && mb[0] >= 0 && (ma[0] & 0x60000000) == 0x20000000 && (mb[0] & 0x60000000) == 0x20000000;
        for (int e = 0; e < w && ok; ++e)
        {
          const int ba = e ? ma[e] : (ma[0] & 0x1fffffff), bb = e ? mb[e] : (mb[0] & 0x1fffffff);
          ok = bb - ba == 64;
        }
      }
    }
    pairs[p] = ok ? 1 : 0;
  }
}

template <bool DOT, bool SR, bool NT>
__global__ __launch_bounds__(SP_BLOCK, SR ? SP_ONE_WGS_SR : SP_ONE_WGS) void spmv_one_kernel(
    const int2* __restrict__ p_desc, const unsigned long long* __restrict__ p_smode, const uint8_t* __restrict__ p_pairs,
    const double* __restrict__ p_svals, const uint16_t* __restrict__ p_c16, const int32_t* __restrict__ p_meta,
    const uint16_t* __restrict__ p_vcode, const double* __restrict__ p_dict, const double* __restrict__ p_x, double* __restrict__ p_y,
    const double* __restrict__ p_rvec, const int32_t* __restrict__ p_list, PipeArgs a)
{
  extern __shared__ __attribute__((aligned(16))) double pp_lds[];
  __shared__ double red[SP_BLOCK / 64];
  const int lane = threadIdx.x & 63;
  const int wv = __builtin_amdgcn_readfirstlane((int)(threadIdx.x >> 6));
  const double* dict = pp_lds;

  const int64_t ngroups = p_list ? a.nlist : ((int64_t)a.nslices + 3) / 4;
  const int64_t nitems = (ngroups + 1) / 2;
  const int xcd = blockIdx.x & 7;
  const int64_t lo = nitems * xcd / 8, hi = nitems * (xcd + 1) / 8;
  const int n_in_xcd = ((int)gridDim.x + 7 - xcd) >> 3;
  const int64_t first_item = lo + (blockIdx.x >> 3);
  const int n_steps = first_item < hi ? (int)((hi - first_item + n_in_xcd - 1) / n_in_xcd) : 0;

  int r_ia = 0, r_ib = 0, r_s = 0;
  auto load_regs = [&](int base) {
    const int i = base + lane;
    const bool valid = i < n_steps;
    const int64_t t = first_item + (int64_t)(valid ? i : 0) * n_in_xcd;
    const int64_t gi = 2 * t + (wv >> 1);
    const bool have = valid && gi < ngroups;
    const int64_t g = (have && p_list) ? p_list[gi] : gi;
    const int64_t sa = 4 * g + 2 * (wv & 1);
    auto slice_info = [&](int64_t s64) -> int {
      if (!(have && s64 < a.nslices))
        return 0;
      const int2 d = p_desc[s64];
      const unsigned sm = (unsigned)p_smode[s64];
      const int nch = d.y & 0xffffff;
      return (nch ? d.x : 0) | ((nch ? (int)((unsigned)d.y >> 24) : 0) << 25) | ((nch ? (int)(sm & 3u) : 0) << 29) | (int)0x80000000;
    };
    r_ia = slice_info(sa);
    r_ib = slice_info(sa + 1);
    const bool pr = have && sa + 1 < a.nslices && p_pairs[sa >> 1] != 0;
    r_s = have ? ((int)sa | (pr ? 0x40000000 : 0)) : 0;
  };
  load_regs(0);
  if (a.stop_flag && *a.stop_flag)
    return;
  {
    double t[SP_DICT_LDS_ENTRIES / SP_BLOCK];
#pragma unroll
    for (int i = 0; i < SP_DICT_LDS_ENTRIES / SP_BLOCK; ++i)
    {
      const int k = (int)threadIdx.x + i * SP_BLOCK;
      t[i] = k < a.dict_n ? p_dict[k] : 0.0;
    }
#pragma unroll
    for (int i = 0; i < SP_DICT_LDS_ENTRIES / SP_BLOCK; ++i)
    {
      const int k = (int)threadIdx.x + i * SP_BLOCK;
      if (k < a.dict_n)
        pp_lds[k] = t[i];
    }
  }
  __syncthreads();

  const int nb8 = a.nrows * 8;
  const __amdgpu_buffer_rsrc_t rs_vq = __builtin_amdgcn_make_buffer_rsrc(const_cast<uint16_t*>(p_vcode), 0, a.nslices * 1024, 0x00020000);
  const __amdgpu_buffer_rsrc_t rs_x = __builtin_amdgcn_make_buffer_rsrc(const_cast<double*>(p_x), 0, nb8, 0x00020000);
  const __amdgpu_buffer_rsrc_t rs_y = __builtin_amdgcn_make_buffer_rsrc(p_y, 0, nb8, 0x00020000);
  const __amdgpu_buffer_rsrc_t rs_r = __builtin_amdgcn_make_buffer_rsrc(const_cast<double*>(SR ? p_rvec : p_x), 0, nb8, 0x00020000);
  const int lane8 = lane * 8, lane16 = lane * 16;
  const int aux = NT ? 2 : 0;

  struct Two
  {
    int ba[8];
    uint4v c0, c1;
  };
  auto prefetch = [&](Two& S, int ia, int ib, int sw) {
    const int ca = ia & 0x1ffffff, cb = ib & 0x1ffffff;
    const int32_t* __restrict__ ma = p_meta + (int64_t)ca * 8;
#pragma unroll
    for (int e = 0; e < 8; ++e)
      S.ba[e] = ma[e];
    int off0, off1;
    if (sw & 0x40000000)
    {
      off0 = ((lane < 32 ? ca : cb) << 10) + ((lane & 31) << 5);
      off1 = off0 + 16;
    }
    else
    {
      off0 = (ca << 10) + lane16;
      off1 = (cb << 10) + lane16;
    }
    const auto q0 = __builtin_amdgcn_raw_buffer_load_b128(rs_vq, off0, 0, aux);
    const auto q1 = __builtin_amdgcn_raw_buffer_load_b128(rs_vq, off1, 0, aux);
    S.c0.x = q0[0], S.c0.y = q0[1], S.c0.z = q0[2], S.c0.w = q0[3];
    S.c1.x = q1[0], S.c1.y = q1[1], S.c1.z = q1[2], S.c1.w = q1[3];
  };
  auto load_codes = [&](int info) -> uint4v {
    const int c = info & 0x1ffffff, cls = (info >> 29) & 3;
    uint4v q = {0u, 0u, 0u, 0u};
    if (cls == SP_CLS_C16)
      q = pipe_load<NT>(reinterpret_cast<const uint4v*>(p_c16 + (int64_t)c * 512) + lane);
    else if (cls != SP_CLS_NONE)
    {
      const char* cbase = cls == SP_CLS_C8T ? reinterpret_cast<const char*>(p_svals) + ((int64_t)c * 4096 + 3584)
                                            : reinterpret_cast<const char*>(p_c16) + (int64_t)c * 1024;
      const uint2v t = pipe_load<NT>(reinterpret_cast<const uint2v*>(cbase) + lane);
      q.x = t.x, q.y = t.y;
    }
    return q;
  };

  double dot = 0.0, dot_rx = 0.0, dot_nn = 0.0;
  int regs_base = 0;
  auto step_scalars = [&](int i, int& ia, int& ib, int& sw) {
    if (i >= n_steps)
    {
      ia = ib = sw = 0;
      return;
    }
    if (i - regs_base >= 64)
    {
      regs_base = i;
      load_regs(regs_base);
      __builtin_amdgcn_s_waitcnt(0x0F70);
    }
    ia = __builtin_amdgcn_readlane(r_ia, i - regs_base);
    ib = __builtin_amdgcn_readlane(r_ib, i - regs_base);
    sw = __builtin_amdgcn_readlane(r_s, i - regs_base);
  };

  auto slice = [&](auto wtag, const int (&b)[8], const uint4v vq, int info, int s, auto&& between) {
    constexpr int W = decltype(wtag)::value;
    const int w = (info >> 25) & 15, cls = (info >> 29) & 3;
    const uint4v cq = load_codes(info);
    unsigned cc[8];
    if (cls == SP_CLS_C16)
    {
      cc[0] = cq.x & 0xffffu, cc[1] = cq.x >> 16, cc[2] = cq.y & 0xffffu, cc[3] = cq.y >> 16;
      cc[4] = cq.z & 0xffffu, cc[5] = cq.z >> 16, cc[6] = cq.w & 0xffffu, cc[7] = cq.w >> 16;
    }
    else if (cls != SP_CLS_NONE)
    {
      cc[0] = cq.x & 0xffu, cc[1] = (cq.x >> 8) & 0xffu, cc[2] = (cq.x >> 16) & 0xffu, cc[3] = cq.x >> 24;
      cc[4] = cq.y & 0xffu, cc[5] = (cq.y >> 8) & 0xffu, cc[6] = (cq.y >> 16) & 0xffu, cc[7] = cq.y >> 24;
    }
    else
    {
#pragma unroll
      for (int e = 0; e < 8; ++e)
        cc[e] = lane;
    }
    const unsigned vc[8] = {vq.x & 0xffffu, vq.x >> 16, vq.y & 0xffffu, vq.y >> 16, vq.z & 0xffffu, vq.z >> 16, vq.w & 0xffffu, vq.w >> 16};
    double xv[W > 0 ? W : 1], v[W > 0 ? W : 1];
#pragma unroll
    for (int e = 0; e < W; ++e)
    {
      const unsigned base = e == 0 ? (unsigned)(b[0] & 0x1fffffff) : (unsigned)b[e];
      xv[e] = *reinterpret_cast<const double*>(reinterpret_cast<const char*>(p_x) + ((base + ((W == 8 && e >= w) ? 0u : cc[e])) << 3));
    }
    double xr = 0.0, rr = 0.0;
    if (DOT)
    {
      const auto u = __builtin_amdgcn_raw_buffer_load_b64(rs_x, lane8, s << 9, 0);
      xr = __hiloint2double((int)u[1], (int)u[0]);
      if (SR)
      {
        const auto t = __builtin_amdgcn_raw_buffer_load_b64(rs_r, lane8, s << 9, 0);
        rr = __hiloint2double((int)t[1], (int)t[0]);
      }
    }
#pragma unroll
    for (int e = 0; e < W; ++e)
      v[e] = dict[vc[e]];
    between();
    double sum = 0.0;
#pragma unroll
    for (int e = 0; e < W; ++e)
      if (W < 8 || e < w)
        sum += v[e] * xv[e];
    __builtin_amdgcn_raw_buffer_store_b64(__builtin_bit_cast(uint2v, sum), rs_y, lane8, s << 9, 0);
    if (DOT && (s << 6) + lane < a.nrows)
    {
      dot += sum * xr;
      if (SR)
      {
        dot_rx += rr * xr;
        dot_nn += a.nn_is_rr ? rr * rr : xr * xr;
      }
    }
  };
  auto slice_w = [&](const int (&b)[8], const uint4v vq, int info, int s, auto&& between) {
    if (info >= 0)
    {
      between();
      return;
    }
    const int w = (info >> 25) & 15;
    if (w == 7)
      slice(std::integral_constant<int, 7>(), b, vq, info, s, between);
    else
      slice(std::integral_constant<int, 8>(), b, vq, info, s, between);
  };

  auto body = [&](Two& S, int ia, int ib, int sw, Two& N, int ia_n, int ib_n, int sw_n) {
    const int sa = sw & 0x3fffffff;
    auto request_next = [&]() {
      __builtin_amdgcn_sched_barrier(0);
      __builtin_amdgcn_s_waitcnt(0xC07F);
      prefetch(N, ia_n, ib_n, sw_n);
      __builtin_amdgcn_sched_barrier(0);
    };
    if (sw & 0x40000000)
    {
      const int w = (ia >> 25) & 15;
      auto pair = [&](auto wtag, auto dtag) {
        constexpr int W = decltype(wtag)::value;
        constexpr int D = decltype(dtag)::value;
        dbl2u xq[W];
#pragma unroll
        for (int e = 0; e < W; ++e)
        {
          if (e == D)
            continue;
          const unsigned base = e == 0 ? (unsigned)(S.ba[0] & 0x1fffffff) : ((W == 8 && e >= w) ? 0u : (unsigned)S.ba[e]);
          xq[e] = *reinterpret_cast<const dbl2u*>(reinterpret_cast<const char*>(p_x) + ((base << 3) + lane16));
        }
        if (D >= 1)
        {
          xq[D >= 1 ? D : 1].x = xq[D >= 1 ? D - 1 : 0].y;
          xq[D >= 1 ? D : 1].y = xq[D >= 1 ? D + 1 : 2].x;
        }
        double xr0 = 0.0, xr1 = 0.0, rr0 = 0.0, rr1 = 0.0;
        if (DOT)
        {
          if (D >= 1)
          {
            xr0 = xq[D >= 1 ? D : 1].x;
            xr1 = xq[D >= 1 ? D : 1].y;
          }
          else
          {
            const auto u = __builtin_amdgcn_raw_buffer_load_b128(rs_x, lane16, sa << 9, 0);
            xr0 = __hiloint2double((int)u[1], (int)u[0]);
            xr1 = __hiloint2double((int)u[3], (int)u[2]);
          }
          if (SR)
          {
            const auto t = __builtin_amdgcn_raw_buffer_load_b128(rs_r, lane16, sa << 9, 0);
            rr0 = __hiloint2double((int)t[1], (int)t[0]);
            rr1 = __hiloint2double((int)t[3], (int)t[2]);
          }
        }
        const uint4v c0 = S.c0, c1 = S.c1;
        __builtin_amdgcn_sched_barrier(0);
        prefetch(N, ia_n, ib_n, sw_n);
        __builtin_amdgcn_sched_barrier(0);
        auto code = [](const uint4v& c, int e) -> unsigned {
          const unsigned wd = e < 2 ? c.x : (e < 4 ? c.y : (e < 6 ? c.z : c.w));
          return (e & 1) ? wd >> 16 : wd & 0xffffu;
        };
        double s0 = 0.0, s1 = 0.0;
#pragma unroll
        for (int e = 0; e < W; ++e)
          if (W < 8 || e < w)
          {
            s0 += dict[code(c0, e)] * xq[e].x;
            s1 += dict[code(c1, e)] * xq[e].y;
          }
        uint4v out;
        out.x = (unsigned)__double2loint(s0), out.y = (unsigned)__double2hiint(s0);
        out.z = (unsigned)__double2loint(s1), out.w = (unsigned)__double2hiint(s1);
        __builtin_amdgcn_raw_buffer_store_b128(out, rs_y, lane16, sa << 9, 0);
        if (DOT)
        {
          const int r0 = (sa << 6) + 2 * lane;
          if (r0 < a.nrows)
          {
            dot += s0 * xr0;
            if (SR)
            {
              dot_rx += rr0 * xr0;
              dot_nn += a.nn_is_rr ? rr0 * rr0 : xr0 * xr0;
            }
          }
          if (r0 + 1 < a.nrows)
          {
            dot += s1 * xr1;
            if (SR)
            {
              dot_rx += rr1 * xr1;
              dot_nn += a.nn_is_rr ? rr1 * rr1 : xr1 * xr1;
            }
          }
        }
      };
      const unsigned rb = (unsigned)sa << 6;
      auto tri = [&](int d) {
        const unsigned bl = d - 1 == 0 ? (unsigned)(S.ba[0] & 0x1fffffff) : (unsigned)S.ba[d - 1];
        return d + 1 < w && (unsigned)S.ba[d] == rb && bl + 1u == rb && (unsigned)S.ba[d + 1] == rb + 1u;
      };
      const int dsel = tri(3) ? 3 : (tri(4) ? 4 : -1);
      if (w == 7)
      {
        if (dsel == 3)
          pair(std::integral_constant<int, 7>(), std::integral_constant<int, 3>());
        else if (dsel == 4)
          pair(std::integral_constant<int, 7>(), std::integral_constant<int, 4>());
        else
          pair(std::integral_constant<int, 7>(), std::integral_constant<int, -1>());
      }
      else
      {
        if (dsel == 3)
          pair(std::integral_constant<int, 8>(), std::integral_constant<int, 3>());
        else if (dsel == 4)
          pair(std::integral_constant<int, 8>(), std::integral_constant<int, 4>());
        else
          pair(std::integral_constant<int, 8>(), std::integral_constant<int, -1>());
      }
    }
    else
    {
      slice_w(S.ba, S.c0, ia, sa, request_next);
      int bb[8];
      const int32_t* __restrict__ mb = p_meta + (int64_t)(ib & 0x1ffffff) * 8;
#pragma unroll
      for (int e = 0; e < 8; ++e)
        bb[e] = mb[e];
      slice_w(bb, S.c1, ib, sa + 1, []() {});
    }
  };

  Two A, B;
  int ia_a, ib_a, sw_a, ia_b, ib_b, sw_b;
  step_scalars(0, ia_a, ib_a, sw_a);
  prefetch(A, ia_a, ib_a, sw_a);
  for (int i = 0; i < n_steps;)
  {
    step_scalars(i + 1, ia_b, ib_b, sw_b);
    body(A, ia_a, ib_a, sw_a, B, ia_b, ib_b, sw_b);
    if (++i >= n_steps)
      break;
    step_scalars(i + 1, ia_a, ib_a, sw_a);
    body(B, ia_b, ib_b, sw_b, A, ia_a, ib_a, sw_a);
    ++i;
  }

  if (DOT)
  {
    const double sres = block_reduce_sum(dot, red);
    double s1 = 0.0, s2 = 0.0;
    if (SR)
    {
      s1 = block_reduce_sum(dot_rx, red);
      s2 = block_reduce_sum(dot_nn, red);
    }
    if (threadIdx.x == 0)
    {
      a.partials[blockIdx.x] = sres;
      if (SR)
      {
        a.partials[a.pstride + blockIdx.x] = s1;
        a.partials[2 * a.pstride + blockIdx.x] = s2;
      }
    }
  }
}

int sellp_pairs_build(zzz_ctx* ctx)
{
  const int64_t npairs = (ctx->nslices + 1) / 2;
  ZZZ_HIP(ctx, ctx->sp_pairs.alloc((size_t)npairs + 1));
  hipLaunchKernelGGL(k_sp_pairs, dim3((unsigned)std::min<int64_t>((npairs + 255) / 256, 4096)), dim3(256), 0, ctx->stream,
                     reinterpret_cast<const int2*>(ctx->sp_desc.p), ctx->sp_smode.p, ctx->sp_meta.p, ctx->nslices, ctx->sp_pairs.p);
  ZZZ_HIP(ctx, hipGetLastError());
  return ZZZ_OK;
}

int sellp_pipe_wgs(const zzz_ctx* ctx, bool sr)
{
  if (!ctx->sellp_pipe || !ctx->sp_pipe_ok || ctx->sp_sorted || ctx->sp_chunks <= 0)
    return 0;
  if (!(ctx->sp_dict_on && ctx->sp_dict_n <= SP_DICT_LDS_ENTRIES && !ctx->sp_sd_on))
    return 0;
  if (!(ctx->sp_one_chunk && ctx->sp_pairs_ok && ctx->bs == 1 && ctx->sp_win_max == 0 && ctx->nslices < (1 << 21)))
    return 0;
  return sr ? SP_ONE_WGS_SR : SP_ONE_WGS;
}

using OneKernel = decltype(&spmv_one_kernel<false, false, false>);
static const OneKernel one_kernels[PM_PLAIN + 1][2] = {{spmv_one_kernel<true, true, true>, spmv_one_kernel<true, true, false>},
                                                       {spmv_one_kernel<true, false, true>, spmv_one_kernel<true, false, false>},
                                                       {spmv_one_kernel<false, false, true>, spmv_one_kernel<false, false, false>}};

bool launch_sellp_pipe(zzz_ctx* ctx, int grid, const ProductCall& c)
{
  if (c.epi || !sellp_pipe_wgs(ctx, c.mode == PM_DOT_SR))
    return false;
  PipeArgs a;
  a.dict_n = ctx->sp_dict_n;
  a.nrows = (int)ctx->nrows;
  a.nslices = (int)ctx->nslices;
  product_args_tail(a, c);
  const size_t lds = (size_t)((ctx->sp_dict_n + 1) & ~1) * sizeof(double);
  hipLaunchKernelGGL(one_kernels[c.mode][c.load], dim3(grid), dim3(SP_BLOCK), lds, ctx->stream,
                     reinterpret_cast<const int2*>(ctx->sp_desc.p), ctx->sp_smode.p, ctx->sp_pairs.p, ctx->sp_vals.p, ctx->sp_codes16.p,
                     ctx->sp_meta.p, ctx->sp_vcode.p, ctx->sp_dset.dict.p, c.x, c.y, c.rvec, c.list, a);
  return true;
}
ZZZ_PRELOAD_TU(sellp_pipe)
}
```

### performance-test_amd/zzz/__init__.py

```python
import ctypes as C
import os
import subprocess

import numpy as np

PKG = os.path.dirname(os.path.dirname(os.path.abspath(__file__)))
ROOT = os.path.dirname(PKG)

FORM_POISSON, FORM_ELASTICITY = 0, 1
COEFF_F, COEFF_G = 0, 1
VEC_B, VEC_U = 0, 1
PC_NONE, PC_JACOBI, PC_CHEBYSHEV_JACOBI, PC_MG, PC_PMG = 0, 1, 2, 3, 4
NORM_PRECONDITIONED, NORM_UNPRECONDITIONED, NORM_NATURAL = 0, 1, 2
CG_PETSC, CG_CGH, CG_PIPE = 0, 1, 2
OP_CSR, OP_MATFREE = 0, 1
ERR_NO_GPU = 4

ABI_SYMBOLS = [
    "zzz_device_count", "zzz_device_memory", "zzz_ctx_create", "zzz_ctx_destroy", "zzz_last_error", "zzz_sync", "zzz_mesh_upload",
    "zzz_dofmap_upload", "zzz_bc_upload", "zzz_bc_values_upload", "zzz_facets_upload", "zzz_coeff_upload", "zzz_cube_generate",
    "zzz_csr_pattern_build",
    "zzz_csr_sizes", "zzz_csr_download", "zzz_csr_rowptr64_download", "zzz_csr_upload_values", "zzz_assemble_matrix", "zzz_assemble_vector",
    "zzz_vec_download", "zzz_vec_upload", "zzz_vec_norm", "zzz_spmv", "zzz_spmv_time", "zzz_spmv_values_info", "zzz_spmv_values_info2", "zzz_abi_version", "zzz_action", "zzz_matfree_setup", "zzz_matfree_info", "zzz_matfree_diagonal", "zzz_action_time", "zzz_near_nullspace_build", "zzz_near_nullspace_download", "zzz_cg_solve", "zzz_cg_history",
    "zzz_profile_get", "zzz_cg_info", "zzz_internal_order_download", "zzz_global_ids_upload", "zzz_global_ids_download", "zzz_ghost_layer_build", "zzz_local_sizes", "zzz_spmv_info", "zzz_comm_load", "zzz_comm_library_path", "zzz_comm_info", "zzz_comm_unique_id", "zzz_comm_init", "zzz_halo_upload", "zzz_local_group_create",
# ... 287 lines not shown

        def blocks(v, width):
            out = np.empty_like(v)
            out.reshape(self.nloc, width)[full] = v.reshape(self.nloc, width)
            return out

        Q.cell_dofs = full[self.cell_dofs][c_order].astype(np.int32)
        Q.cells = v_new_of_old[self.cells][c_order].astype(np.int32)
        Q.x = np.empty_like(self.x)
        Q.x[v_new_of_old] = self.x
        Q.global_verts = np.empty_like(self.global_verts)
        Q.global_verts[v_new_of_old] = self.global_verts
        c_new_of_old = np.empty(nc, np.int64)
        c_new_of_old[c_order] = np.arange(nc)
        Q.facets = self.facets.copy()
        if Q.facets.size:
            Q.facets[:, 0] = c_new_of_old[self.facets[:, 0]]
        Q.bc_dofs = np.sort(full[self.bc_dofs // bs] * bs + self.bc_dofs % bs).astype(np.int32)
        Q.f = blocks(self.f, bs)
        Q.g = blocks(self.g, 1) if self.g is not None else None
        Q.dof_x = blocks(self.dof_x.reshape(-1), 3).reshape(-1, 3)
        Q.global_dofs = blocks(self.global_dofs, 1)
        Q.send_idx = full[self.send_idx].astype(np.int32)
        return Q


class Context:

    def __init__(self, device=0):
        self.L = hip()
        h = C.c_void_p()
        rc = self.L.zzz_ctx_create(int(device), C.byref(h))
        if rc:
            raise ZzzError(rc, self.L.zzz_last_error(None).decode())
        self.h = h
        self.bs = 1
        self.n_owned = 0
        self.n_ghost = 0

    def close(self):
        if getattr(self, "h", None):
            self.L.zzz_ctx_destroy(self.h)
            self.h = None

    def __del__(self):
        self.close()

    def __enter__(self):
        return self

    def __exit__(self, *a):
        self.close()

    def _ck(self, rc):
        if rc:
            raise ZzzError(rc, self.L.zzz_last_error(self.h).decode())

    def sync(self):
        self._ck(self.L.zzz_sync(self.h))

    def upload_mesh(self, x, cells):
        x = np.ascontiguousarray(x, np.float64)
        cells = np.ascontiguousarray(cells, np.int32)
        self._ck(self.L.zzz_mesh_upload(self.h, x.shape[0], x, cells.shape[0], cells))

    def upload_dofmap(self, order, bs, cell_dofs, n_owned, n_ghost=0):
        cd = np.ascontiguousarray(cell_dofs, np.int32)
        self._ck(self.L.zzz_dofmap_upload(self.h, order, bs, cd, n_owned, n_ghost))
        self.bs, self.n_owned, self.n_ghost = bs, n_owned, n_ghost

    def upload_bc(self, bc_dofs):
        b = np.ascontiguousarray(bc_dofs, np.int32)
        self._ck(self.L.zzz_bc_upload(self.h, b.shape[0], b if b.size else np.zeros(1, np.int32)))

    def upload_bc_values(self, values):
        if values is None:
            self._ck(self.L.zzz_bc_values_upload(self.h, None))
            return
        v = np.ascontiguousarray(values, np.float64)
        if self.n_owned and v.shape != ((self.n_owned + self.n_ghost) * self.bs,):
            raise ValueError(f"upload_bc_values: {v.shape} values for {(self.n_owned + self.n_ghost) * self.bs} local dofs")
        self._ck(self.L.zzz_bc_values_upload(self.h, v.ctypes.data_as(C.c_void_p)))

    def upload_facets(self, facets):
        f = np.ascontiguousarray(facets, np.int32).reshape(-1)
        self._ck(self.L.zzz_facets_upload(self.h, f.shape[0] // 2, f if f.size else np.zeros(2, np.int32)))

    def upload_coeff(self, which, values):
        self._ck(self.L.zzz_coeff_upload(self.h, which, np.ascontiguousarray(values, np.float64)))

    def upload_global_ids(self, dof_global, vert_global):
        d = np.ascontiguousarray(dof_global, np.int64)
        v = np.ascontiguousarray(vert_global, np.int64)
        self._ck(self.L.zzz_global_ids_upload(self.h, d.ctypes.data_as(C.c_void_p), v.ctypes.data_as(C.c_void_p)))

    def ghost_layer_build(self):
        self._ck(self.L.zzz_ghost_layer_build(self.h))
        s = self.local_sizes()
        self.n_ghost = s[3]
        return s

    def local_sizes(self):
        s = (C.c_int64 * 6)()
        self._ck(self.L.zzz_local_sizes(self.h, s))
        return [int(v) for v in s]

    def global_ids(self):
        s = self.local_sizes()
        out = np.zeros(s[2] + s[3], np.int64)
        self._ck(self.L.zzz_global_ids_download(self.h, out.ctypes.data_as(C.c_void_p)))
        return out

    def upload_part(self, P):
        self.upload_mesh(P.x, P.cells)
        self.upload_dofmap(P.order, P.bs, P.cell_dofs, P.n_owned, P.n_ghost)
        self.upload_bc(P.bc_dofs)
        self.upload_facets(P.facets)
        self.upload_coeff(COEFF_F, P.f)
        if P.g is not None:
            self.upload_coeff(COEFF_G, P.g)

    def cube_generate(self, problem, order, nx, ny, nz, nparts=1, part=0):
        info = np.zeros(6, np.int64)
        pid = FORM_ELASTICITY if problem == "elasticity" else FORM_POISSON
        self._ck(self.L.zzz_cube_generate(self.h, pid, order, nx, ny, nz, nparts, part, info))
        self.bs = 3 if pid == FORM_ELASTICITY else 1
        self.n_owned, self.n_ghost = int(info[2]), int(info[3])
        return info

    def pattern_build(self):
        self._ck(self.L.zzz_csr_pattern_build(self.h))

    def csr_sizes(self):
        a, b, c = C.c_int64(), C.c_int64(), C.c_int64()
        self._ck(self.L.zzz_csr_sizes(self.h, C.byref(a), C.byref(b), C.byref(c)))
        return a.value, b.value, c.value

    def csr_download(self, values=True):
        nrows, _, nnz = self.csr_sizes()
        rowptr = np.zeros(nrows + 1, np.int32)
        cols = np.zeros(nnz, np.int32)
        vals = np.zeros(nnz) if values else None
        self._ck(self.L.zzz_csr_download(self.h, rowptr.ctypes.data, cols.ctypes.data,
                                         vals.ctypes.data if values else None))
        return rowptr, cols, vals

    def csr_rowptr64(self):
        nrows, _, _ = self.csr_sizes()
        out = np.zeros(nrows + 1, np.int64)
        self._ck(self.L.zzz_csr_rowptr64_download(self.h, out.ctypes.data_as(C.c_void_p)))
        return out

    def csr_upload_values(self, vals):
        self._ck(self.L.zzz_csr_upload_values(self.h, np.ascontiguousarray(vals, np.float64)))

    def assemble_matrix(self, form):
        self._ck(self.L.zzz_assemble_matrix(self.h, form))

    def assemble_vector(self, form):
        self._ck(self.L.zzz_assemble_vector(self.h, form))

    def vec_download(self, which):
        out = np.zeros(self.n_owned * self.bs)
        self._ck(self.L.zzz_vec_download(self.h, which, out))
        return out

    def vec_upload(self, which, v):
        v = np.ascontiguousarray(v, np.float64)
        assert v.shape[0] == self.n_owned * self.bs
        self._ck(self.L.zzz_vec_upload(self.h, which, v))

    def vec_norm(self, which):
        out = C.c_double()
        self._ck(self.L.zzz_vec_norm(self.h, which, C.byref(out)))
        return out.value

    def spmv(self, x):
        x = np.ascontiguousarray(x, np.float64)
        y = np.zeros_like(x)
        self._ck(self.L.zzz_spmv(self.h, x, y))
        return y

    def spmv_time(self, reps=20, variant=-1):
        ms = C.c_double()
        self._ck(self.L.zzz_spmv_time(self.h, reps, variant, C.byref(ms)))
        return ms.value

    def action(self, x):
        x = np.ascontiguousarray(x, np.float64)
        y = np.zeros_like(x)
        self._ck(self.L.zzz_action(self.h, x, y))
        return y

    def near_nullspace(self):
        dev = C.c_double()
        self._ck(self.L.zzz_near_nullspace_build(self.h, C.byref(dev)))
        B = np.zeros((6, 3 * self.n_owned))
        for k in range(6):
            self._ck(self.L.zzz_near_nullspace_download(self.h, k, B[k]))
        return B, dev.value

    def matfree_setup(self):
        self._ck(self.L.zzz_matfree_setup(self.h))

    def matfree_diagonal(self):
        d = np.zeros(self.n_owned * self.bs)
        self._ck(self.L.zzz_matfree_diagonal(self.h, d))
        return d

    def matfree_info(self):
        a = (C.c_int64 * 8)()
        self._ck(self.L.zzz_matfree_info(self.h, a))
        return dict(zip(("valid", "blocks", "cells_per_block", "threads", "nloc_max", "shared_dofs", "partial_slots",
                         "bytes_per_action"), [int(v) for v in a]))

    def action_time(self, reps=20):
        ms = C.c_double()
        self._ck(self.L.zzz_action_time(self.h, reps, C.byref(ms)))
        return ms.value

    def action_f32(self, x):
        x = np.ascontiguousarray(x, np.float32)
        y = np.zeros_like(x)
        self._ck(self.L.zzz_action_f32(self.h, x, y))
        return y

    def action_time_f32(self, reps=20):
        ms = C.c_double()
        self._ck(self.L.zzz_action_time_f32(self.h, reps, C.byref(ms)))
        return ms.value

    def matfree_info_f32(self):
        a = (C.c_int64 * 4)()
        self._ck(self.L.zzz_matfree_info_f32(self.h, a))
        return dict(zip(("built", "bytes_per_action", "lds_bytes", "workgroups_per_cu"), [int(v) for v in a]))

    def cg_solve_f32(self, variant=CG_CGH, pc=PC_NONE, op=OP_MATFREE, rtol=1e-6, max_it=100, single_reduction=False,
                     error_if_not_converged=False):
        o = SolverOpts(variant, pc, NORM_PRECONDITIONED, op, max_it, 0, 1 if single_reduction else 0,
                       1 if error_if_not_converged else 0, rtol, 1e-50, 0.0, 0, 0, 0.0, 0, 0)
        it = C.c_int()
        rn = (C.c_double * 2)()
        self._ck(self.L.zzz_cg_solve_f32(self.h, C.byref(o), C.byref(it), rn))
        return it.value, rn[0], rn[1]

    def cg_solve(self, variant=CG_PETSC, pc=PC_JACOBI, norm=NORM_PRECONDITIONED, op=OP_CSR, rtol=1e-8, atol=1e-50,
                 max_it=10000, profile=False, single_reduction=False, dtol=0.0, error_if_not_converged=False,
                 pc_degree=0, pc_ratio=0.0, pc_esteig_its=0, pc_mg_levels=0, pc_mg_coarse_eq_limit=0):
        o = SolverOpts(variant, pc, norm, op, max_it, 1 if profile else 0, 1 if single_reduction else 0,
                       1 if error_if_not_converged else 0, rtol, atol, dtol, pc_degree, pc_esteig_its, pc_ratio,
                       pc_mg_levels, pc_mg_coarse_eq_limit)
        it = C.c_int()
        rn = (C.c_double * 2)()
        self._ck(self.L.zzz_cg_solve(self.h, C.byref(o), C.byref(it), rn))
        return it.value, rn[0], rn[1]

    def mg_setup(self, pc_degree=0, pc_ratio=0.0, pc_esteig_its=0, pc_mg_levels=0, pc_mg_coarse_eq_limit=0, pc=PC_MG):
        o = SolverOpts(CG_PETSC, pc, NORM_PRECONDITIONED, OP_CSR, 10000, 0, 0, 0, 1e-8, 1e-50, 0.0, pc_degree, pc_esteig_its,
                       pc_ratio, pc_mg_levels, pc_mg_coarse_eq_limit)
        self._ck(self.L.zzz_mg_setup(self.h, C.byref(o)))

    def mg_info(self, level=-1):
        out = np.zeros(8)
        self._ck(self.L.zzz_mg_info(self.h, level, out))
        if level < 0:
            return dict(levels=int(out[0]), coarse_dofs=int(out[1]), setups=int(out[2]), products_per_cycle=int(out[3]),
                        coarse_bytes=int(out[4]), cycle_ms=float(out[5]), setup_ms=float(out[6]), high_order_levels=int(out[7]))
        return dict(cells=(int(out[0]), int(out[1]), int(out[2])), dofs=int(out[3]), nnz=int(out[4]), hi=float(out[5]),
                    lo=float(out[6]), degree=int(out[7]))

    def mg_apply(self, r):
        r = np.ascontiguousarray(r, np.float64)
        z = np.zeros_like(r)
        self._ck(self.L.zzz_mg_apply(self.h, r, z))
        return z

    def mg_transfer(self, level, direction, v):
        v = np.ascontiguousarray(v, np.float64)
        a, b = self.mg_info(level)["dofs"], self.mg_info(level + 1)["dofs"]
        assert v.shape[0] == (b if direction == 0 else a)
        out = np.zeros(a if direction == 0 else b)
        self._ck(self.L.zzz_mg_transfer(self.h, level, direction, v, out))
        return out

    def cg_history(self, n):
        out = np.zeros(n)
        self._ck(self.L.zzz_cg_history(self.h, n, out))
        return out

    def spmv_info(self):
        info = (C.c_int64 * 8)()
        self._ck(self.L.zzz_spmv_info(self.h, info))
        return tuple(int(v) for v in info[:4])

    def spmv_operator_form(self):
        return self.spmv_info_raw()[5]

    def spmv_info_raw(self):
        info = (C.c_int64 * 8)()
        self._ck(self.L.zzz_spmv_info(self.h, info))
        return [int(v) for v in info]

    def spmv_values_info(self):
        info = (C.c_int64 * 10)()
        self._ck(self.L.zzz_spmv_values_info2(self.h, 10, info))
        return dict(form=("doubles", "dictionary in memory", "dictionary in LDS", "slice dictionaries")[int(info[0])], distinct_values=int(info[1]),
                    bytes_per_product=int(info[2]), bytes_per_product_as_doubles=int(info[3]),
                    one_chunk_kernel=bool(info[4]), workgroups_per_cu=int(info[5]), block_rows=int(info[6]) == 1, row_windows=int(info[6]) == 2,
                    special_form=("", "block rows", "block windows")[int(info[6])],
                    block_table_entries=int(info[7]), block_chunks=int(info[8]), block_form=int(info[9]))

    def spmv_x_windows(self):
        info = self.spmv_info_raw()
        return (int(-info[3]), int(info[2])) if info[5] and info[3] < 0 else (0, 0)

    def spmv_lanes_per_row(self):
        info = (C.c_int64 * 8)()
        self._ck(self.L.zzz_spmv_info(self.h, info))
        return int(info[4])

    def internal_order(self):
        perm = np.zeros(self.n_owned, np.int32)
        kind = C.c_int32()
        self._ck(self.L.zzz_internal_order_download(self.h, perm.ctypes.data_as(C.c_void_p), C.byref(kind)))
        return perm, int(kind.value) & 15

    def cells_renumbered(self):
        kind = C.c_int32()
        self._ck(self.L.zzz_internal_order_download(self.h, None, C.byref(kind)))
        return bool(int(kind.value) & 16)

    def cg_reason(self):
        info = (C.c_int64 * 4)()
        self._ck(self.L.zzz_cg_info(self.h, info))
        return int(info[2])

    def cg_info(self):
        info = (C.c_int64 * 4)()
        self._ck(self.L.zzz_cg_info(self.h, info))
        return {"fused": bool(info[0] & 1), "dinv_codes": int(info[0] >> 8) if info[0] & 2 else 0,
                "allreduce_overlapped": bool(info[0] & 4), "xdefer_k": int((info[0] >> 4) & 15) if info[0] & 8 else 1,
                "reason": int(info[2]),
                "pc_spectrum_bound": info[3] * 1.0e-6}

    def profile(self):
        ms, n = C.c_double(), C.c_int64()
        self._ck(self.L.zzz_profile_get(self.h, C.byref(ms), C.byref(n)))
        return ms.value, n.value

    def comm_info(self):
        info = (C.c_int64 * 12)()
        self._ck(self.L.zzz_comm_info(self.h, info))
        keys = ("ranks", "rank", "neighbours", "halo_bytes_sent", "halo_bytes_received", "halo_own_communicator",
                "peer_memory_allreduce", "halo_overlapped", "interior_items", "boundary_items", "local_backend",
                "halo_wait_ns_per_product")
        return {k: int(v) for k, v in zip(keys, info)}

    def comm_init(self, nranks, rank, uid_bytes):
        buf = C.create_string_buffer(bytes(uid_bytes), 128)
        self._ck(self.L.zzz_comm_init(self.h, nranks, rank, buf))

    def comm_init_local(self, group, rank):
        self._ck(self.L.zzz_comm_init_local(self.h, group, rank))

    def comm_init_peer_only(self, nranks, rank):
        self._ck(self.L.zzz_comm_init_peer_only(self.h, nranks, rank))

    def comm_p2p_export(self):
        buf = C.create_string_buffer(P2P_HANDLE_BYTES)
        self._ck(self.L.zzz_comm_p2p_export(self.h, buf))
        return bytes(buf.raw)

    def comm_p2p_attach(self, handles):
        buf = C.create_string_buffer(bytes(handles), len(handles))
        en = C.c_int(0)
        self._ck(self.L.zzz_comm_p2p_attach(self.h, buf, C.byref(en)))
        return bool(en.value)

    def comm_p2p_disable(self):
        self._ck(self.L.zzz_comm_p2p_disable(self.h))

    def comm_p2p_enable(self):
        en = C.c_int(0)
        self._ck(self.L.zzz_comm_p2p_enable(self.h, C.byref(en)))
        return bool(en.value)

    def comm_p2p_halo(self, on=True):
        used = C.c_int(0)
        self._ck(self.L.zzz_comm_p2p_halo(self.h, 1 if on else 0, C.byref(used)))
        return bool(used.value)

    def upload_halo(self, P):
        nn = len(P.neigh)
        z32, z64 = np.zeros(1, np.int32), np.zeros(1, np.int64)
        self._ck(self.L.zzz_halo_upload(self.h, nn, P.neigh if nn else z32, P.send_off if nn else z64,
                                        P.send_idx if P.send_idx.size else z32, P.recv_cnt if nn else z64))


P2P_HANDLE_BYTES = 128


def comm_load():
    rc = hip().zzz_comm_load()
    if rc:
        raise ZzzError(rc, hip().zzz_last_error(None).decode())


def comm_library_path():
    f = hip().zzz_comm_library_path
    f.restype = C.c_char_p
    return f().decode()


def comm_unique_id():
    buf = C.create_string_buffer(128)
    rc = hip().zzz_comm_unique_id(buf)
    if rc:
        raise ZzzError(rc, hip().zzz_last_error(None).decode())
    return buf.raw


class LocalGroup:

    def __init__(self, nranks):
        self.h = C.c_void_p()
        rc = hip().zzz_local_group_create(int(nranks), C.byref(self.h))
        if rc:
            raise ZzzError(rc, hip().zzz_last_error(None).decode())
        self.n = nranks

    def abort(self):
        if self.h:
            hip().zzz_local_group_abort(self.h)

    def close(self):
        if self.h:
            hip().zzz_local_group_destroy(self.h)
            self.h = None
```

Baseline: 54.69 million.

## Add per-slice palette compression of SELL-P value codes in one-chunk SpMV

Adds a build kernel that, for each one-chunk slice, checks whether every column position uses at most 16 distinct dictionary codes. Slices that pass are repacked into a palette with 4-bit indices, shrinking the value stream from 16-bit codes to 8 bytes per lane. The pipelined SpMV kernel gets a PAL variant that loads the packed form, expands the palette into per-wave LDS and gathers values from it, and falls back to reading the full code words for slices that did not pack, including mixed pairs. The aim is to cut HBM bytes per CG SpMV, at the cost of extra LDS traffic, wave barriers, more template variants and an extra build pass. The path is enabled by default (sellp_pal=1) but only applies when the dictionary fits in LDS, the matrix is unsorted and scalar (bs==1), and no x windows are in use.

```diff
diff --git a/performance-test_amd/csrc/zzz_api.hip b/performance-test_amd/csrc/zzz_api.hip
--- a/performance-test_amd/csrc/zzz_api.hip
+++ b/performance-test_amd/csrc/zzz_api.hip
@@ -180,6 +180,8 @@
     ctx->sellp_blk = atoi(e);
   if (const char* e = getenv("ZZZ_SELLP_PIPE"))
     ctx->sellp_pipe = atoi(e);
+  if (const char* e = getenv("ZZZ_SELLP_PAL"))
+    ctx->sellp_pal = atoi(e) != 0;
   if (const char* e = getenv("ZZZ_CG_DINV_CODES"))
     ctx->cg_dinv_codes = atoi(e);
   if (const char* e = getenv("ZZZ_CG_XDEFER"))
@@ -1144,7 +1146,7 @@
   ZZZ_ENTER(ctx);
   if (!out || n < 0 || !ctx->have_pattern)
     return fail(ctx, ZZZ_ERR_ARG, "zzz_spmv_values_info: no pattern");
-  int64_t info[10] = {0, 0, 0, 0, 0, 0, 0, 0, 0, 0};
+  int64_t info[14] = {0, 0, 0, 0, 0, 0, 0, 0, 0, 0, 0, 0, 0, 0};
   if (sellp_active(ctx))
   {
     const bool blk = zzz::sellp_blk_serves(ctx);
@@ -1161,8 +1163,20 @@
     info[9] = blk ? ctx->bk_form : (win ? ctx->bw_nblk : 0);
     if (win)
       info[4] = 0, info[5] = 1;
-  }
-  for (int i = 0; i < std::min(n, 10); ++i)
+    if (info[4] && ctx->sp_pal_on)
+    {
+      info[10] = ctx->sp_pal_packed;
+      info[11] = ctx->nslices - ctx->sp_pal_packed;
+      info[12] = ctx->sp_pal_mixed;
+      info[13] = ctx->sp_pal_maxcount;
+    }
+    else if (info[4])
+    {
+      info[11] = ctx->nslices;
+      info[13] = ctx->sellp_pal ? ctx->sp_pal_maxcount : 0;
+    }
+  }
+  for (int i = 0; i < std::min(n, 14); ++i)
     out[i] = info[i];
   return ZZZ_OK;
 }
diff --git a/performance-test_amd/csrc/zzz_cg.hip b/performance-test_amd/csrc/zzz_cg.hip
--- a/performance-test_amd/csrc/zzz_cg.hip
+++ b/performance-test_amd/csrc/zzz_cg.hip
@@ -819,7 +819,7 @@
 
 bool loop_exceeds_cache(zzz_ctx* ctx, int nvec)
 {
-  const double op = sellp_active(ctx) ? (double)sellp_stream_bytes(ctx) : 10.0 * (double)ctx->nnz;
+  const double op = sellp_active(ctx) ? (double)sellp_stream_bytes(ctx, true) : 10.0 * (double)ctx->nnz;
   return op + 8.0 * nvec * (double)ctx->nloc() > 200.0e6;
 }
 
diff --git a/performance-test_amd/csrc/zzz_internal.h b/performance-test_amd/csrc/zzz_internal.h
--- a/performance-test_amd/csrc/zzz_internal.h
+++ b/performance-test_amd/csrc/zzz_internal.h
@@ -245,6 +245,13 @@
   zzz::DevBuf<uint8_t> sp_pairs;
   bool sp_pairs_ok = false;
   int sellp_pipe = 1;
+  zzz::DevBuf<uint2> sp_pal;
+  zzz::DevBuf<uint8_t> sp_palok;
+  zzz::DevBuf<int32_t> sp_pal_info;
+  bool sp_pal_on = false;
+  int64_t sp_pal_packed = 0, sp_pal_mixed = 0;
+  int sp_pal_maxcount = 0;
+  int sellp_pal = 1;
   int64_t nslices = 0, sp_chunks = 0, sp_kept = 0, sp_bytes = 0;
   zzz::DevBuf<uint8_t> sp_wlast;
   zzz::DevBuf<uint16_t> sp_vcode;
@@ -487,7 +494,7 @@
 int sellp_resolve(zzz_ctx* ctx);
 int sellp_pattern_bounds(zzz_ctx* ctx);
 int sellp_capacity_rows(zzz_ctx* ctx);
-int64_t sellp_stream_bytes(const zzz_ctx* ctx);
+int64_t sellp_stream_bytes(const zzz_ctx* ctx, bool as_codes = false);
 constexpr int SP_DICT_LDS_ENTRIES = 2048;
 int launch_sellp(zzz_ctx* ctx, ProductCall c, int* npartials);
 int launch_sellp_overlapped(zzz_ctx* ctx, double* x, ProductCall c, int* npartials);
diff --git a/performance-test_amd/csrc/zzz_sellp.hip b/performance-test_amd/csrc/zzz_sellp.hip
--- a/performance-test_amd/csrc/zzz_sellp.hip
+++ b/performance-test_amd/csrc/zzz_sellp.hip
@@ -400,7 +400,7 @@
   if (!ctx->sp_dict_done)
   {
     ctx->sp_dict_done = true;
-    ctx->sp_dict_on = ctx->sp_sd_on = ctx->sp_sd_all = false;
+    ctx->sp_dict_on = ctx->sp_sd_on = ctx->sp_sd_all = ctx->sp_pal_on = false;
     ctx->sp_dict_n = 0;
     if (!ctx->sp_special_tried)
     {
@@ -411,7 +411,7 @@
     {
       if (sp_dict_build(ctx) != ZZZ_OK)
       {
-        ctx->sp_dict_on = false;
+        ctx->sp_dict_on = ctx->sp_pal_on = false;
         (void)hipGetLastError();
         ctx->sp_vcode.release();
       }
@@ -432,18 +432,19 @@
   return true;
 }
 
-int64_t sellp_stream_bytes(const zzz_ctx* ctx)
+int64_t sellp_stream_bytes(const zzz_ctx* ctx, bool as_codes)
 {
   if (sellp_blk_serves(ctx))
     return ctx->bk_bytes;
   if (sellp_win_serves(ctx))
     return ctx->bw_bytes;
-  return (ctx->sp_sd_on ? ctx->sp_sd_bytes : (ctx->sp_dict_on ? ctx->sp_dict_bytes : ctx->sp_bytes)) + ctx->nslices * 8;
+  const int64_t packed = !as_codes && ctx->sp_pal_on && sellp_pipe_wgs(ctx, false) ? 512 * ctx->sp_pal_packed : 0;
+  return (ctx->sp_sd_on ? ctx->sp_sd_bytes : (ctx->sp_dict_on ? ctx->sp_dict_bytes : ctx->sp_bytes)) + ctx->nslices * 8 - packed;
 }
 
 static bool sp_stream_nt(const zzz_ctx* ctx)
 {
-  return (double)sellp_stream_bytes(ctx) + 48.0 * (double)(ctx->n_owned + ctx->n_ghost) * ctx->bs > 200.0e6;
+  return (double)sellp_stream_bytes(ctx, true) + 48.0 * (double)(ctx->n_owned + ctx->n_ghost) * ctx->bs > 200.0e6;
 }
 
 static int sp_grid(const zzz_ctx* ctx, int64_t ngroups, bool sr, bool plain)
diff --git a/performance-test_amd/csrc/zzz_sellp_dict.hip b/performance-test_amd/csrc/zzz_sellp_dict.hip
--- a/performance-test_amd/csrc/zzz_sellp_dict.hip
+++ b/performance-test_amd/csrc/zzz_sellp_dict.hip
@@ -115,6 +115,102 @@
   }
   if (lane == 0 && bytes)
     atomicAdd(bytes_out, bytes);
+}
+
+__global__ __launch_bounds__(256) void k_sp_pal_build(const int2* __restrict__ desc, const uint16_t* __restrict__ vcode, int64_t nslices,
+                                                       const int* __restrict__ dict_info, uint2* __restrict__ pal,
+                                                       uint8_t* __restrict__ palok, int32_t* __restrict__ info)
+{
+  __shared__ uint16_t pal_s[4][128];
+  if (dict_info[1])
+    return;
+  const int lane = threadIdx.x & 63, wv = threadIdx.x >> 6;
+  uint16_t* const ps = pal_s[wv];
+  int npacked = 0, maxc = 0;
+  for (int64_t s = blockIdx.x * 4ll + wv; s < nslices; s += gridDim.x * 4ll)
+  {
+    const int2 ds = desc[s];
+    const int nch = ds.y & 0xffffff;
+    if (nch != 1)
+    {
+      if (lane == 0)
+        palok[s] = 0;
+      continue;
+    }
+    const uint4v q = reinterpret_cast<const uint4v*>(vcode + (size_t)ds.x * 512)[lane];
+    const unsigned code[8] = {q.x & 0xffffu, q.x >> 16, q.y & 0xffffu, q.y >> 16, q.z & 0xffffu, q.z >> 16, q.w & 0xffffu, q.w >> 16};
+    ps[2 * lane] = 0;
+    ps[2 * lane + 1] = 0;
+    __builtin_amdgcn_fence(__ATOMIC_ACQ_REL, "wavefront");
+    __builtin_amdgcn_wave_barrier();
+    unsigned idx = 0;
+    bool ok = true;
+#pragma unroll
+    for (int e = 0; e < 8; ++e)
+    {
+      const unsigned cur = code[e];
+      bool rem = true;
+      unsigned myval = 0, mine = 0;
+      int k = 0;
+      for (;;)
+      {
+        const unsigned long long m = __ballot(rem);
+        if (!m)
+          break;
+        const unsigned v = (unsigned)__builtin_amdgcn_readlane((int)cur, __builtin_amdgcn_readfirstlane(__builtin_ctzll(m)));
+        if (cur == v)
+        {
+          mine = (unsigned)k;
+          rem = false;
+        }
+        if (lane == k)
+          myval = v;
+        ++k;
+      }
+      maxc = k > maxc ? k : maxc;
+      if (k > 16)
+      {
+        ok = false;
+        continue;
+      }
+      unsigned rank = 0;
+      for (int j = 0; j < k; ++j)
+        rank += (unsigned)__builtin_amdgcn_readlane((int)myval, j) < myval ? 1u : 0u;
+      if (lane < k)
+        ps[e * 16 + rank] = (uint16_t)myval;
+      idx |= (unsigned)__shfl((int)rank, (int)mine) << (4 * e);
+    }
+    __builtin_amdgcn_fence(__ATOMIC_ACQ_REL, "wavefront");
+    __builtin_amdgcn_wave_barrier();
+    uint2 out = make_uint2(0u, 0u);
+    if (ok)
+      out = make_uint2(idx, (unsigned)ps[2 * lane] | ((unsigned)ps[2 * lane + 1] << 16));
+    pal[(size_t)ds.x * 64 + lane] = out;
+    if (lane == 0)
+      palok[s] = ok ? 1 : 0;
+    npacked += ok ? 1 : 0;
+    __builtin_amdgcn_fence(__ATOMIC_ACQ_REL, "wavefront");
+    __builtin_amdgcn_wave_barrier();
+  }
+  if (lane == 0)
+  {
+    if (npacked)
+      atomicAdd(&info[0], npacked);
+    if (maxc)
+      atomicMax(&info[1], maxc);
+  }
+}
+
+__global__ __launch_bounds__(256) void k_sp_pal_mixed(const uint8_t* __restrict__ palok, int64_t nslices, const int* __restrict__ dict_info,
+                                                       int32_t* __restrict__ info)
+{
+  if (dict_info[1])
+    return;
+  int n = 0;
+  for (int64_t p = blockIdx.x * (int64_t)blockDim.x + threadIdx.x; 2 * p + 1 < nslices; p += (int64_t)gridDim.x * blockDim.x)
+    n += palok[2 * p] != palok[2 * p + 1] ? 1 : 0;
+  if (n)
+    atomicAdd(&info[2], n);
 }
 
 template <bool PERM, bool COUNT>
@@ -278,7 +374,7 @@
 int sp_dict_build(zzz_ctx* ctx)
 {
   ctx->sp_dict_done = true;
-  ctx->sp_dict_on = false;
+  ctx->sp_dict_on = ctx->sp_pal_on = false;
   ctx->sp_dict_n = 0;
   if (!ctx->sellp_dict || ctx->sp_chunks <= 0 || (ctx->sellp_dict == 1 && ctx->sp_bytes < 48ll << 20))
     return ZZZ_OK;
@@ -308,6 +404,20 @@
                        ctx->sp_meta.p, (int)ctx->nrows, nsl, vs.table.p, vs.slot.p, vs.info.p, ctx->sp_vcode.p, bytes);
   unsigned long long hb = 0;
   ZZZ_HIP(ctx, hipMemcpyAsync(&hb, bytes, sizeof(hb), hipMemcpyDeviceToHost, s));
+  const bool pal = ctx->sellp_pal && ctx->sp_one_chunk && !ctx->sp_sorted && ctx->bs == 1 && ctx->sp_win_max == 0;
+  int32_t hp[4] = {0, 0, 0, 0};
+  if (pal)
+  {
+    ZZZ_HIP(ctx, ctx->sp_pal.alloc((size_t)ctx->sp_chunks * 64));
+    ZZZ_HIP(ctx, ctx->sp_palok.alloc((size_t)nsl + 1));
+    ZZZ_HIP(ctx, ctx->sp_pal_info.reserve(4));
+    ZZZ_HIP(ctx, hipMemsetAsync(ctx->sp_pal_info.p, 0, 4 * sizeof(int32_t), s));
+    hipLaunchKernelGGL(k_sp_pal_build, dim3(grid), dim3(256), 0, s, desc, ctx->sp_vcode.p, nsl, vs.info.p, ctx->sp_pal.p, ctx->sp_palok.p,
+                       ctx->sp_pal_info.p);
+    hipLaunchKernelGGL(k_sp_pal_mixed, dim3((unsigned)std::min<int64_t>((nsl / 2 + 255) / 256 + 1, 1024)), dim3(256), 0, s, ctx->sp_palok.p,
+                       nsl, vs.info.p, ctx->sp_pal_info.p);
+    ZZZ_HIP(ctx, hipMemcpyAsync(hp, ctx->sp_pal_info.p, sizeof(hp), hipMemcpyDeviceToHost, s));
+  }
   int n = 0;
   ZZZ_HIP(ctx, vs.finish(s, n));
   if (!n)
@@ -315,6 +425,10 @@
   ctx->sp_dict_n = n;
   ctx->sp_dict_bytes = (int64_t)hb + (int64_t)n * 8;
   ctx->sp_dict_on = true;
+  ctx->sp_pal_packed = hp[0];
+  ctx->sp_pal_maxcount = hp[1];
+  ctx->sp_pal_mixed = hp[2];
+  ctx->sp_pal_on = pal && n <= SP_DICT_LDS_ENTRIES && hp[0] > 0;
   return ZZZ_OK;
 }
 
diff --git a/performance-test_amd/csrc/zzz_sellp_pipe.hip b/performance-test_amd/csrc/zzz_sellp_pipe.hip
--- a/performance-test_amd/csrc/zzz_sellp_pipe.hip
+++ b/performance-test_amd/csrc/zzz_sellp_pipe.hip
@@ -1,4 +1,5 @@
 #include <algorithm>
+#include <array>
 #include <cstdlib>
 #include <type_traits>
 
@@ -54,15 +55,17 @@
   }
 }
 
-template <bool DOT, bool SR, bool NT>
+template <bool DOT, bool SR, bool NT, bool PAL>
 __global__ __launch_bounds__(SP_BLOCK, SR ? SP_ONE_WGS_SR : SP_ONE_WGS) void spmv_one_kernel(
     const int2* __restrict__ p_desc, const unsigned long long* __restrict__ p_smode, const uint8_t* __restrict__ p_pairs,
     const double* __restrict__ p_svals, const uint16_t* __restrict__ p_c16, const int32_t* __restrict__ p_meta,
-    const uint16_t* __restrict__ p_vcode, const double* __restrict__ p_dict, const double* __restrict__ p_x, double* __restrict__ p_y,
+    const uint16_t* __restrict__ p_vcode, const uint2* __restrict__ p_pal, const uint8_t* __restrict__ p_palok,
+    const double* __restrict__ p_dict, const double* __restrict__ p_x, double* __restrict__ p_y,
     const double* __restrict__ p_rvec, const int32_t* __restrict__ p_list, PipeArgs a)
 {
   extern __shared__ __attribute__((aligned(16))) double pp_lds[];
   __shared__ double red[SP_BLOCK / 64];
+  __shared__ __attribute__((aligned(16))) double pal_area[PAL ? (SP_BLOCK / 64) * 256 : 2];
   const int lane = threadIdx.x & 63;
   const int wv = __builtin_amdgcn_readfirstlane((int)(threadIdx.x >> 6));
   const double* dict = pp_lds;
@@ -94,8 +97,10 @@
     };
     r_ia = slice_info(sa);
     r_ib = slice_info(sa + 1);
-    const bool pr = have && sa + 1 < a.nslices && p_pairs[sa >> 1] != 0;
-    r_s = have ? ((int)sa | (pr ? 0x40000000 : 0)) : 0;
+    bool pr = have && sa + 1 < a.nslices && p_pairs[sa >> 1] != 0;
+    const bool pka = PAL && have && sa < a.nslices && p_palok[sa] != 0;
+    const bool pkb = PAL && have && sa + 1 < a.nslices && p_palok[sa + 1] != 0;
+    r_s = have ? ((int)sa | (pr ? 0x40000000 : 0) | (pka ? 0x10000000 : 0) | (pkb ? 0x20000000 : 0)) : 0;
   };
   load_regs(0);
   if (a.stop_flag && *a.stop_flag)
@@ -120,6 +125,7 @@
 
   const int nb8 = a.nrows * 8;
   const __amdgpu_buffer_rsrc_t rs_vq = __builtin_amdgcn_make_buffer_rsrc(const_cast<uint16_t*>(p_vcode), 0, a.nslices * 1024, 0x00020000);
+  const __amdgpu_buffer_rsrc_t rs_pq = __builtin_amdgcn_make_buffer_rsrc(const_cast<uint2*>(p_pal), 0, PAL ? a.nslices * 512 : 0, 0x00020000);
   const __amdgpu_buffer_rsrc_t rs_x = __builtin_amdgcn_make_buffer_rsrc(const_cast<double*>(p_x), 0, nb8, 0x00020000);
   const __amdgpu_buffer_rsrc_t rs_y = __builtin_amdgcn_make_buffer_rsrc(p_y, 0, nb8, 0x00020000);
   const __amdgpu_buffer_rsrc_t rs_r = __builtin_amdgcn_make_buffer_rsrc(const_cast<double*>(SR ? p_rvec : p_x), 0, nb8, 0x00020000);
@@ -131,12 +137,28 @@
     int ba[8];
     uint4v c0, c1;
   };
+  double* const area = pal_area + (PAL ? wv * 256 : 0);
   auto prefetch = [&](Two& S, int ia, int ib, int sw) {
     const int ca = ia & 0x1ffffff, cb = ib & 0x1ffffff;
     const int32_t* __restrict__ ma = p_meta + (int64_t)ca * 8;
 #pragma unroll
     for (int e = 0; e < 8; ++e)
       S.ba[e] = ma[e];
+    if (PAL)
+    {
+      if (sw & 0x40000000)
+      {
+        const auto q = __builtin_amdgcn_raw_buffer_load_b128(rs_pq, ((lane < 32 ? ca : cb) << 9) + ((lane & 31) << 4), 0, aux);
+        S.c0.x = q[0], S.c0.y = q[1], S.c0.z = q[2], S.c0.w = q[3];
+      }
+      else
+      {
+        const auto t0 = __builtin_amdgcn_raw_buffer_load_b64(rs_pq, (ca << 9) + lane8, 0, aux);
+        const auto t1 = __builtin_amdgcn_raw_buffer_load_b64(rs_pq, (cb << 9) + lane8, 0, aux);
+        S.c0.x = t0[0], S.c0.y = t0[1], S.c0.z = t1[0], S.c0.w = t1[1];
+      }
+      return;
+    }
     int off0, off1;
     if (sw & 0x40000000)
     {
@@ -187,10 +209,15 @@
     sw = __builtin_amdgcn_readlane(r_s, i - regs_base);
   };
 
-  auto slice = [&](auto wtag, const int (&b)[8], const uint4v vq, int info, int s, auto&& between) {
+  auto slice = [&](auto wtag, const int (&b)[8], uint4v vq, int info, int s, bool packed, int half, auto&& between) {
     constexpr int W = decltype(wtag)::value;
     const int w = (info >> 25) & 15, cls = (info >> 29) & 3;
     const uint4v cq = load_codes(info);
+    if (PAL && !packed)
+    {
+      const auto q = __builtin_amdgcn_raw_buffer_load_b128(rs_vq, ((info & 0x1ffffff) << 10) + lane16, 0, aux);
+      vq.x = q[0], vq.y = q[1], vq.z = q[2], vq.w = q[3];
+    }
     unsigned cc[8];
     if (cls == SP_CLS_C16)
     {
@@ -227,9 +254,25 @@
         rr = __hiloint2double((int)t[1], (int)t[0]);
       }
     }
-#pragma unroll
-    for (int e = 0; e < W; ++e)
-      v[e] = dict[vc[e]];
+    if (PAL && packed)
+    {
+      double* const ah = area + half * 128;
+      dbl2 t;
+      t.x = dict[vq.y & 0xffffu], t.y = dict[vq.y >> 16];
+      __builtin_amdgcn_fence(__ATOMIC_RELEASE, "wavefront");
+      *reinterpret_cast<dbl2*>(ah + 2 * lane) = t;
+      __builtin_amdgcn_fence(__ATOMIC_ACQ_REL, "wavefront");
+      __builtin_amdgcn_wave_barrier();
+#pragma unroll
+      for (int e = 0; e < W; ++e)
+        v[e] = ah[e * 16 + ((vq.x >> (4 * e)) & 15u)];
+    }
+    else
+    {
+#pragma unroll
+      for (int e = 0; e < W; ++e)
+        v[e] = dict[vc[e]];
+    }
     between();
     double sum = 0.0;
 #pragma unroll
@@ -247,7 +290,7 @@
       }
     }
   };
-  auto slice_w = [&](const int (&b)[8], const uint4v vq, int info, int s, auto&& between) {
+  auto slice_w = [&](const int (&b)[8], const uint4v vq, int info, int s, bool packed, int half, auto&& between) {
     if (info >= 0)
     {
       between();
@@ -255,13 +298,13 @@
     }
     const int w = (info >> 25) & 15;
     if (w == 7)
-      slice(std::integral_constant<int, 7>(), b, vq, info, s, between);
+      slice(std::integral_constant<int, 7>(), b, vq, info, s, packed, half, between);
     else
-      slice(std::integral_constant<int, 8>(), b, vq, info, s, between);
+      slice(std::integral_constant<int, 8>(), b, vq, info, s, packed, half, between);
   };
 
   auto body = [&](Two& S, int ia, int ib, int sw, Two& N, int ia_n, int ib_n, int sw_n) {
-    const int sa = sw & 0x3fffffff;
+    const int sa = sw & 0x0fffffff;
     auto request_next = [&]() {
       __builtin_amdgcn_sched_barrier(0);
       __builtin_amdgcn_s_waitcnt(0xC07F);
@@ -271,8 +314,9 @@
     if (sw & 0x40000000)
     {
       const int w = (ia >> 25) & 15;
-      auto pair = [&](auto wtag, auto dtag) {
+      auto pair = [&](auto wtag, auto dtag, auto mtag) {
         constexpr int W = decltype(wtag)::value;
+        constexpr bool MIX = decltype(mtag)::value;
         constexpr int D = decltype(dtag)::value;
         dbl2u xq[W];
 #pragma unroll
@@ -318,13 +362,50 @@
           return (e & 1) ? wd >> 16 : wd & 0xffffu;
         };
         double s0 = 0.0, s1 = 0.0;
-#pragma unroll
-        for (int e = 0; e < W; ++e)
-          if (W < 8 || e < w)
+        if (PAL)
+        {
+          dbl2 t0, t1;
+          t0.x = dict[c0.y & 0xffffu], t0.y = dict[c0.y >> 16];
+          t1.x = dict[c0.w & 0xffffu], t1.y = dict[c0.w >> 16];
+          __builtin_amdgcn_fence(__ATOMIC_RELEASE, "wavefront");
+          *reinterpret_cast<dbl2*>(area + 4 * lane) = t0;
+          *reinterpret_cast<dbl2*>(area + 4 * lane + 2) = t1;
+          __builtin_amdgcn_fence(__ATOMIC_ACQ_REL, "wavefront");
+          __builtin_amdgcn_wave_barrier();
+          const double* const ah = area + (lane >> 5) * 128;
+          uint4v u0 = {0u, 0u, 0u, 0u}, u1 = {0u, 0u, 0u, 0u};
+          bool coded = false;
+          if (MIX)
           {
-            s0 += dict[code(c0, e)] * xq[e].x;
-            s1 += dict[code(c1, e)] * xq[e].y;
+            coded = ((lane < 32 ? sw & 0x10000000 : sw & 0x20000000)) == 0;
+            if (coded)
+            {
+              const int off = (((lane < 32 ? ia : ib) & 0x1ffffff) << 10) + ((lane & 31) << 5);
+              const auto q0 = __builtin_amdgcn_raw_buffer_load_b128(rs_vq, off, 0, aux);
+              const auto q1 = __builtin_amdgcn_raw_buffer_load_b128(rs_vq, off + 16, 0, aux);
+              u0.x = q0[0], u0.y = q0[1], u0.z = q0[2], u0.w = q0[3];
+              u1.x = q1[0], u1.y = q1[1], u1.z = q1[2], u1.w = q1[3];
+            }
           }
+#pragma unroll
+          for (int e = 0; e < W; ++e)
+            if (W < 8 || e < w)
+            {
+              const double v0 = ah[e * 16 + ((c0.x >> (4 * e)) & 15u)], v1 = ah[e * 16 + ((c0.z >> (4 * e)) & 15u)];
+              s0 += (MIX && coded ? dict[code(u0, e)] : v0) * xq[e].x;
+              s1 += (MIX && coded ? dict[code(u1, e)] : v1) * xq[e].y;
+            }
+        }
+        else
+        {
+#pragma unroll
+          for (int e = 0; e < W; ++e)
+            if (W < 8 || e < w)
+            {
+              s0 += dict[code(c0, e)] * xq[e].x;
+              s1 += dict[code(c1, e)] * xq[e].y;
+            }
+        }
         uint4v out;
         out.x = (unsigned)__double2loint(s0), out.y = (unsigned)__double2hiint(s0);
         out.z = (unsigned)__double2loint(s1), out.w = (unsigned)__double2hiint(s1);
@@ -358,34 +439,46 @@
         return d + 1 < w && (unsigned)S.ba[d] == rb && bl + 1u == rb && (unsigned)S.ba[d + 1] == rb + 1u;
       };
       const int dsel = tri(3) ? 3 : (tri(4) ? 4 : -1);
-      if (w == 7)
+      constexpr std::false_type all_packed;
+      constexpr std::integral_constant<bool, PAL> not_all_packed;
+      if (PAL && (sw & 0x30000000) != 0x30000000)
+      {
+        if (w == 7)
+          pair(std::integral_constant<int, 7>(), std::integral_constant<int, -1>(), not_all_packed);
+        else
+          pair(std::integral_constant<int, 8>(), std::integral_constant<int, -1>(), not_all_packed);
+      }
+      else if (w == 7)
       {
         if (dsel == 3)
-          pair(std::integral_constant<int, 7>(), std::integral_constant<int, 3>());
+          pair(std::integral_constant<int, 7>(), std::integral_constant<int, 3>(), all_packed);
         else if (dsel == 4)
-          pair(std::integral_constant<int, 7>(), std::integral_constant<int, 4>());
+          pair(std::integral_constant<int, 7>(), std::integral_constant<int, 4>(), all_packed);
         else
-          pair(std::integral_constant<int, 7>(), std::integral_constant<int, -1>());
+          pair(std::integral_constant<int, 7>(), std::integral_constant<int, -1>(), all_packed);
       }
       else
       {
         if (dsel == 3)
-          pair(std::integral_constant<int, 8>(), std::integral_constant<int, 3>());
+          pair(std::integral_constant<int, 8>(), std::integral_constant<int, 3>(), all_packed);
         else if (dsel == 4)
-          pair(std::integral_constant<int, 8>(), std::integral_constant<int, 4>());
+          pair(std::integral_constant<int, 8>(), std::integral_constant<int, 4>(), all_packed);
         else
-          pair(std::integral_constant<int, 8>(), std::integral_constant<int, -1>());
+          pair(std::integral_constant<int, 8>(), std::integral_constant<int, -1>(), all_packed);
       }
     }
     else
     {
-      slice_w(S.ba, S.c0, ia, sa, request_next);
+      uint4v qb = S.c1;
+      if (PAL)
+        qb.x = S.c0.z, qb.y = S.c0.w;
+      slice_w(S.ba, S.c0, ia, sa, (sw & 0x10000000) != 0, 0, request_next);
       int bb[8];
       const int32_t* __restrict__ mb = p_meta + (int64_t)(ib & 0x1ffffff) * 8;
 #pragma unroll
       for (int e = 0; e < 8; ++e)
         bb[e] = mb[e];
-      slice_w(bb, S.c1, ib, sa + 1, []() {});
+      slice_w(bb, qb, ib, sa + 1, (sw & 0x20000000) != 0, 1, []() {});
     }
   };
 
@@ -446,10 +539,15 @@
   return sr ? SP_ONE_WGS_SR : SP_ONE_WGS;
 }
 
-using OneKernel = decltype(&spmv_one_kernel<false, false, false>);
-static const OneKernel one_kernels[PM_PLAIN + 1][2] = {{spmv_one_kernel<true, true, true>, spmv_one_kernel<true, true, false>},
-                                                       {spmv_one_kernel<true, false, true>, spmv_one_kernel<true, false, false>},
-                                                       {spmv_one_kernel<false, false, true>, spmv_one_kernel<false, false, false>}};
+using OneKernel = decltype(&spmv_one_kernel<false, false, false, false>);
+template <bool PAL>
+constexpr std::array<std::array<OneKernel, 2>, PM_PLAIN + 1> one_variants()
+{
+  return {{{spmv_one_kernel<true, true, true, PAL>, spmv_one_kernel<true, true, false, PAL>},
+           {spmv_one_kernel<true, false, true, PAL>, spmv_one_kernel<true, false, false, PAL>},
+           {spmv_one_kernel<false, false, true, PAL>, spmv_one_kernel<false, false, false, PAL>}}};
+}
+static const std::array<std::array<OneKernel, 2>, PM_PLAIN + 1> one_kernels[2] = {one_variants<false>(), one_variants<true>()};
 
 bool launch_sellp_pipe(zzz_ctx* ctx, int grid, const ProductCall& c)
 {
@@ -461,9 +559,9 @@
   a.nslices = (int)ctx->nslices;
   product_args_tail(a, c);
   const size_t lds = (size_t)((ctx->sp_dict_n + 1) & ~1) * sizeof(double);
-  hipLaunchKernelGGL(one_kernels[c.mode][c.load], dim3(grid), dim3(SP_BLOCK), lds, ctx->stream,
+  hipLaunchKernelGGL(one_kernels[ctx->sp_pal_on ? 1 : 0][c.mode][c.load], dim3(grid), dim3(SP_BLOCK), lds, ctx->stream,
                      reinterpret_cast<const int2*>(ctx->sp_desc.p), ctx->sp_smode.p, ctx->sp_pairs.p, ctx->sp_vals.p, ctx->sp_codes16.p,
-                     ctx->sp_meta.p, ctx->sp_vcode.p, ctx->sp_dset.dict.p, c.x, c.y, c.rvec, c.list, a);
+                     ctx->sp_meta.p, ctx->sp_vcode.p, ctx->sp_pal.p, ctx->sp_palok.p, ctx->sp_dset.dict.p, c.x, c.y, c.rvec, c.list, a);
   return true;
 }
 ZZZ_PRELOAD_TU(sellp_pipe)
diff --git a/performance-test_amd/zzz/__init__.py b/performance-test_amd/zzz/__init__.py
--- a/performance-test_amd/zzz/__init__.py
+++ b/performance-test_amd/zzz/__init__.py
@@ -613,13 +613,15 @@
         return [int(v) for v in info]
 
     def spmv_values_info(self):
-        info = (C.c_int64 * 10)()
-        self._ck(self.L.zzz_spmv_values_info2(self.h, 10, info))
+        info = (C.c_int64 * 14)()
+        self._ck(self.L.zzz_spmv_values_info2(self.h, 14, info))
         return dict(form=("doubles", "dictionary in memory", "dictionary in LDS", "slice dictionaries")[int(info[0])], distinct_values=int(info[1]),
                     bytes_per_product=int(info[2]), bytes_per_product_as_doubles=int(info[3]),
                     one_chunk_kernel=bool(info[4]), workgroups_per_cu=int(info[5]), block_rows=int(info[6]) == 1, row_windows=int(info[6]) == 2,
                     special_form=("", "block rows", "block windows")[int(info[6])],
-                    block_table_entries=int(info[7]), block_chunks=int(info[8]), block_form=int(info[9]))
+                    block_table_entries=int(info[7]), block_chunks=int(info[8]), block_form=int(info[9]),
+                    packed_slices=int(info[10]), unpacked_slices=int(info[11]), mixed_pairs=int(info[12]),
+                    max_codes_per_slot=int(info[13]))
 
     def spmv_x_windows(self):
         info = self.spmv_info_raw()
```

Result: faster. 59.12 million (median of 6 runs) (+8.1%).
